# mbhall88/drprg

Measured on AMD Instinct MI355X. Metric: reads/sec (+ achieved HBM GB/s) predicting on mtb index, 1/2/4/8 GPUs, higher is better.
Workload: dtype u32

## Files before the change

drprg_amd/_lib.py:

```python
import ctypes as C
import os

_HERE = os.path.dirname(os.path.abspath(__file__))
LIB_PATH = os.environ.get("DRPRG_HIP_LIB") or os.path.join(_HERE, "lib", "libdrprg_hip.so")
PANDORA_EXE = os.path.join(_HERE, "bin", "pandora")


class MapOpts(C.Structure):
    _fields_ = [
        ("max_diff", C.c_int32),
        ("error_rate", C.c_double),
        ("min_cluster_size", C.c_uint32),
        ("illumina", C.c_int32),
        ("genome_size", C.c_uint64),
        ("genotyping_error_rate", C.c_double),
        ("kernel", C.c_int32),
        ("binomial", C.c_int32),
    ]


class AnnotateOpts(C.Structure):
    _fields_ = [
        ("min_covg", C.c_int32), ("max_covg", C.c_int32),
        ("min_strand_bias", C.c_float), ("min_gt_conf", C.c_float), ("min_frs", C.c_float),
        ("max_indel", C.c_int32),
        ("maf", C.c_float), ("max_gaps", C.c_float), ("max_called_gaps", C.c_float), ("max_gaps_diff", C.c_float),
        ("minor_min_covg", C.c_int32), ("minor_min_strand_bias", C.c_float),
        ("ignore_synonymous", C.c_int32), ("id_seed", C.c_uint64),
    ]

    @classmethod
    def cli_defaults(cls, illumina=False):
        return cls(3, 2 ** 31 - 1, 0.01, 0.0, 0.0, -1, 0.1 if illumina else 1.0, 0.5, 0.39, 0.2, 3, 0.01, 0, 0)


SIGNATURES = {
    "drprg_hip_index": (C.c_int, [C.c_char_p, C.c_int, C.c_int, C.c_int]),
    "drprg_hip_open": (C.c_void_p, [C.c_char_p, C.c_int, C.c_int, C.c_int]),
    "drprg_hip_open_prg": (C.c_void_p, [C.c_char_p, C.c_int, C.c_int, C.c_int, C.c_int]),
    "drprg_hip_open_multi": (C.c_void_p, [C.c_char_p, C.c_int, C.c_int, C.POINTER(C.c_int), C.c_int, C.c_int]),
    "drprg_hip_reduce": (C.c_int, [C.c_void_p]),
    "drprg_hip_reduce_info": (C.c_int, [C.c_void_p, C.c_char_p, C.c_size_t]),
    "drprg_hip_comm_unique_id": (C.c_int, [C.c_void_p]),
    "drprg_hip_comm_init_rank": (C.c_int, [C.POINTER(C.c_void_p), C.c_int, C.c_void_p, C.c_int, C.c_int]),
    "drprg_hip_comm_destroy": (C.c_int, [C.c_void_p]),
    "drprg_hip_allreduce": (C.c_int, [C.c_void_p, C.c_void_p, C.c_void_p, C.c_void_p, C.c_void_p]),
    "drprg_hip_close": (None, [C.c_void_p]),
    "drprg_hip_last_error": (C.c_char_p, [C.c_void_p]),
    "drprg_hip_experimental": (C.c_int, []),
    "drprg_hip_set_opts": (C.c_int, [C.c_void_p, C.POINTER(MapOpts)]),
    "drprg_hip_set_opts_sized": (C.c_int, [C.c_void_p, C.POINTER(MapOpts), C.c_size_t]),
    "drprg_hip_map_fastx": (C.c_int, [C.c_void_p, C.c_char_p]),
    "drprg_hip_set_threads": (C.c_int, [C.c_void_p, C.c_int]),
    "drprg_hip_parse_fastx": (C.c_int, [C.c_char_p, C.c_int, C.POINTER(C.c_uint64), C.c_char_p, C.c_size_t]),
    "drprg_hip_parse_fastx_ordered": (C.c_int, [C.c_char_p, C.c_int, C.c_uint64, C.POINTER(C.c_uint64), C.c_char_p, C.c_size_t]),
    "drprg_hip_gunzip_file": (C.c_int, [C.c_char_p, C.c_int, C.c_uint64, C.c_char_p, C.POINTER(C.c_uint64), C.c_char_p, C.c_size_t]),
    "drprg_hip_map_host": (C.c_int, [C.c_void_p, C.c_void_p, C.c_void_p, C.c_uint64]),
    "drprg_hip_map_device": (C.c_int, [C.c_void_p, C.c_void_p, C.c_void_p, C.c_uint64, C.c_uint64, C.c_void_p,
                                       C.c_void_p, C.c_void_p]),
    "drprg_hip_map_device_async": (C.c_int, [C.c_void_p, C.c_void_p, C.c_void_p, C.c_uint64, C.c_uint64, C.c_void_p,
                                             C.c_void_p, C.c_void_p]),
    "drprg_hip_sync": (C.c_int, [C.c_void_p]),
    "drprg_hip_set_input_format": (C.c_int, [C.c_void_p, C.c_int]),
    "drprg_hip_pack_reads": (C.c_int, [C.c_void_p, C.c_uint64, C.c_void_p, C.c_void_p, C.c_uint64, C.POINTER(C.c_uint64)]),
    "drprg_hip_map_host_packed": (C.c_int, [C.c_void_p, C.c_void_p, C.c_void_p, C.c_uint64, C.c_void_p, C.c_uint64]),
    "drprg_hip_map_device_packed": (C.c_int, [C.c_void_p, C.c_void_p, C.c_void_p, C.c_uint64, C.c_uint64, C.c_void_p, C.c_uint64, C.c_void_p,
                                              C.c_void_p, C.c_void_p]),
    "drprg_hip_map_device_packed_async": (C.c_int, [C.c_void_p, C.c_void_p, C.c_void_p, C.c_uint64, C.c_uint64, C.c_void_p, C.c_uint64, C.c_void_p,
                                                    C.c_void_p, C.c_void_p]),
    "drprg_hip_pack_device": (C.c_int, [C.c_void_p, C.c_void_p, C.c_uint64, C.c_void_p, C.c_void_p, C.c_uint64, C.POINTER(C.c_uint64), C.c_void_p]),
    "drprg_hip_coverage_size": (C.c_int, [C.c_void_p, C.POINTER(C.c_uint64), C.POINTER(C.c_uint64)]),
    "drprg_hip_coverage": (C.c_int, [C.c_void_p, C.c_void_p, C.c_uint64, C.c_void_p, C.c_uint64]),
    "drprg_hip_set_coverage": (C.c_int, [C.c_void_p, C.c_void_p, C.c_uint64, C.c_void_p, C.c_uint64, C.c_uint64]),
    "drprg_hip_device_coverage": (C.c_int, [C.c_void_p, C.POINTER(C.c_void_p), C.POINTER(C.c_void_p)]),
    "drprg_hip_reset": (C.c_int, [C.c_void_p]),
    "drprg_hip_set_max_covg": (C.c_int, [C.c_void_p, C.c_uint64]),
    "drprg_hip_max_covg_info": (C.c_int, [C.c_void_p, C.POINTER(C.c_uint64)]),
    "drprg_hip_keep_reads": (C.c_int, [C.c_void_p, C.c_uint64]),
    "drprg_hip_map_resident": (C.c_int, [C.c_void_p, C.c_void_p]),
    "drprg_hip_resident_info": (C.c_int, [C.c_void_p, C.POINTER(C.c_uint64)]),
    "drprg_hip_select_reads": (C.c_int, [C.c_void_p, C.c_void_p, C.c_uint64, C.c_uint32, C.c_uint64, C.c_void_p, C.c_uint64, C.c_void_p, C.c_void_p,
                                         C.c_uint64, C.POINTER(C.c_uint64)]),
    "drprg_hip_counters": (C.c_int, [C.c_void_p, C.POINTER(C.c_uint64)]),
    "drprg_hip_genotype": (C.c_int, [C.c_void_p, C.c_char_p, C.c_char_p, C.c_char_p]),
    "drprg_hip_genotype_info": (C.c_int, [C.c_void_p, C.POINTER(C.c_uint32)]),
    "drprg_hip_discover": (C.c_int, [C.c_void_p, C.c_char_p, C.c_char_p, C.c_char_p, C.POINTER(C.c_uint32)]),
    "drprg_hip_discover_reads": (C.c_int, [C.c_void_p, C.c_char_p, C.c_char_p, C.c_char_p, C.c_char_p, C.c_int, C.POINTER(C.c_uint32)]),
    "drprg_hip_update_prg": (C.c_int, [C.c_void_p, C.c_char_p, C.POINTER(C.c_uint32)]),
    "drprg_hip_update_prg_from_paths": (C.c_int, [C.c_void_p, C.c_char_p, C.c_char_p, C.POINTER(C.c_uint32)]),
    "drprg_hip_save_coverage": (C.c_int, [C.c_void_p, C.c_char_p, C.c_char_p]),
    "drprg_hip_load_coverage": (C.c_int, [C.c_void_p, C.c_char_p, C.c_char_p, C.POINTER(C.c_uint64)]),
    "drprg_hip_allele_stats": (C.c_int, [C.c_void_p, C.c_void_p, C.c_uint32, C.c_uint32, C.c_void_p, C.POINTER(C.c_double)]),
    "drprg_hip_genotype_site": (C.c_int, [C.c_void_p, C.c_void_p, C.c_void_p, C.c_uint32, C.c_double, C.c_double, C.c_void_p,
                                          C.POINTER(C.c_int32), C.POINTER(C.c_double)]),
    "drprg_hip_genotype_alleles": (C.c_int, [C.c_void_p, C.c_char_p]),
    "drprg_hip_estimate_parameters": (C.c_int, [C.c_void_p, C.c_uint64, C.c_uint64, C.c_uint64, C.c_uint32, C.c_int, C.c_double, C.c_int,
                                               C.POINTER(C.c_double)]),
    "drprg_hip_kmer_log_prob": (C.c_int, [C.c_int, C.c_double, C.c_double, C.c_double, C.c_uint32, C.c_uint32, C.c_uint32, C.POINTER(C.c_float)]),
    "drprg_hip_prob_threshold": (C.c_int, [C.c_void_p, C.c_uint64, C.POINTER(C.c_int)]),
    "drprg_hip_max_path": (C.c_int, [C.c_void_p, C.c_uint32, C.c_void_p, C.c_int, C.c_uint32, C.c_void_p, C.c_uint64, C.POINTER(C.c_uint64)]),
    "drprg_hip_path_base_coverage": (C.c_int, [C.c_void_p, C.c_uint32, C.c_void_p, C.c_uint64, C.c_void_p, C.c_void_p, C.c_uint64,
                                              C.POINTER(C.c_uint64)]),
    "drprg_hip_path_coverage_too_low": (C.c_int, [C.c_void_p, C.c_uint64, C.c_uint32]),
    "drprg_hip_coverage_model": (C.c_int, [C.c_void_p, C.POINTER(C.c_double)]),
    "drprg_hip_index_sizes": (C.c_int, [C.c_void_p, C.POINTER(C.c_uint64)]),
    "drprg_hip_filter_selfcheck": (C.c_int, [C.c_void_p, C.POINTER(C.c_uint64)]),
    "drprg_hip_device_tables": (C.c_int, [C.c_void_p, C.POINTER(C.c_uint64)]),
    "drprg_hip_index_export": (C.c_int, [C.c_void_p] + [C.c_void_p] * 7),
    "drprg_hip_prg_nodes": (C.c_int, [C.c_void_p, C.c_uint32, C.c_void_p, C.c_void_p, C.c_uint32, C.POINTER(C.c_uint32),
                                      C.POINTER(C.c_uint32)]),
    "drprg_hip_annotate": (C.c_int, [C.c_char_p, C.c_char_p, C.c_char_p, C.POINTER(AnnotateOpts), C.c_char_p, C.c_size_t]),
    "drprg_hip_vcf_to_bcf": (C.c_int, [C.c_char_p, C.c_char_p, C.c_char_p, C.c_size_t]),
    "drprg_hip_report_json": (C.c_int, [C.c_char_p, C.c_char_p, C.c_char_p, C.c_char_p, C.c_int, C.c_char_p, C.c_char_p,
                                        C.c_size_t]),
    "drprg_hip_kernel_timing": (C.c_int, [C.c_void_p, C.c_int, C.c_int, C.POINTER(C.c_double), C.POINTER(C.c_uint64)]),
    "drprg_hip_filter_schedule": (C.c_int, [C.c_void_p, C.POINTER(C.c_uint64)]),
    "drprg_hip_buffer_info": (C.c_int, [C.c_void_p, C.POINTER(C.c_uint64)]),
}


def load():
    if not os.path.exists(LIB_PATH):
        raise ImportError(
            f"{LIB_PATH} is missing: build the HIP extension first (`make` at the repo root or "
            "`python -c 'import __graft_entry__ as g; g.build()'`). There is no CPU fallback.")
    try:
        import torch
    except Exception:
        pass
    lib = C.CDLL(LIB_PATH)
    for name, (res, args) in SIGNATURES.items():
        fn = getattr(lib, name)
        fn.restype = res
        fn.argtypes = args
    return lib


lib = load()
```

drprg_amd/csrc/capi.cpp:

```cpp
#include <set>
#include <atomic>
#include <mutex>
#include <thread>
#include <fstream>
#include <cstdio>
#include "../../include/drprg_hip.h"
#include "fastx.h"
#include "genotype.h"
#include "ingest.h"
#include "pgunzip.h"
#include "denovo.h"
#include "mapper.h"
#include "rccl_dyn.h"
#include "pack.h"
#include <algorithm>
#include <cstdlib>
#include <cstring>
#include <fcntl.h>
#include <functional>
#include <sys/mman.h>
#include <sys/stat.h>
#include <unistd.h>
#include <memory>

// ... 114 lines not shown
        return DRPRG_EIO;                               \
    }                                                   \
    return DRPRG_OK;

static void apply_defaults(MapParams& p, const drprg_hip_map_opts* o)
{
    p.illumina = o && o->illumina;
    p.error_rate = (o && o->error_rate > 0) ? o->error_rate : (p.illumina ? 0.001 : 0.11);
    p.max_diff = (o && o->max_diff > 0) ? o->max_diff : (p.illumina ? 2 * p.k + 1 : 250);
    p.min_cluster_size = o ? o->min_cluster_size : 10;
    p.genome_size = (o && o->genome_size) ? o->genome_size : 5000000;
    p.genotyping_error_rate = (o && o->genotyping_error_rate > 0) ? o->genotyping_error_rate : 0.01;
    p.kernel_mode = o ? o->kernel : 0;
    p.binomial = o && o->binomial;
}

static void reduce_devices(drprg_hip_ctx* ctx)
{
    if (ctx->extra.empty() || !ctx->mapper) return;
    Mapper& m = *ctx->mapper;
    std::vector<Mapper*> all { &m };
    for (auto& e : ctx->extra) all.push_back(e.get());
    for (Mapper* x : all) x->sync();
    bool distinct = true;
    for (size_t i = 0; i < all.size(); ++i)
        for (size_t j = i + 1; j < all.size(); ++j) distinct &= all[i]->device() != all[j]->device();
    const char* no = std::getenv("DRPRG_HIP_NO_RCCL");
    std::string why;
    const Rccl* r = (distinct && !(no && *no && *no != '0')) ? Rccl::get(&why) : nullptr;
    bool done = false;
    auto chk = [&](int rc, const char* what) {
        if (rc != Rccl::Success) throw Error(DRPRG_EIO, std::string("RCCL ") + what + ": " + (r && r->GetErrorString ? r->GetErrorString(rc) : "error"));
    };
    if (r) {
        if (ctx->comms.empty()) {
            std::vector<int> devs;
            for (Mapper* x : all) devs.push_back(x->device());
            std::vector<Rccl::Comm> comms(all.size(), nullptr);
            const int rc = r->CommInitAll(comms.data(), (int)all.size(), devs.data());
            if (rc == Rccl::Success) ctx->comms = comms;
            else {
                why = std::string("ncclCommInitAll: ") + (r->GetErrorString ? r->GetErrorString(rc) : "error");
                std::fprintf(stderr, "drprg-hip: warning: %s; summing the devices' vectors by peer copies\n", why.c_str());
                r = nullptr;
            }
        }
    }
    if (r) {
        const size_t nv = 2 * (size_t)m.n_knodes() + m.n_prgs();
        chk(r->GroupStart(), "ncclGroupStart");
        int first_rc = Rccl::Success;
        const char* first_what = "";
        for (size_t d = 0; d < all.size() && first_rc == Rccl::Success; ++d) {
            if (hipSetDevice(all[d]->device()) != hipSuccess) {
                first_rc = -1;
                first_what = "hipSetDevice";
                break;
            }
            first_rc = r->Reduce(all[d]->d_covg(), all[d]->d_covg(), nv, Rccl::Uint32, Rccl::Sum, 0, ctx->comms[d], all[d]->stream());
            first_what = "ncclReduce";
        }
        const int end_rc = r->GroupEnd();
        if (first_rc != Rccl::Success || end_rc != Rccl::Success) {
            ctx->needs_reset = true;
            if (first_rc == -1) throw Error(DRPRG_EIO, "hipSetDevice failed inside the reduce (drprg_hip_reset the context)");
            chk(first_rc, first_what);
            chk(end_rc, "ncclGroupEnd");
        }
        for (Mapper* x : all) {
            if (hipSetDevice(x->device()) != hipSuccess || hipStreamSynchronize(x->stream()) != hipSuccess) throw Error(DRPRG_EIO, "stream synchronisation after ncclReduce failed");
        }
        ctx->reduce_how = "rccl: ncclReduce(sum, u32) over " + std::to_string(all.size()) + " devices";
        done = true;
    }
    if (!done) {
        for (auto& e : ctx->extra) m.add_vectors_from(*e);
        ctx->reduce_how = std::string("device add: peer copy + add kernel per device (") + (distinct ? (why.empty() ? "RCCL switched off" : why) : "a device is listed twice") + ")";
    }
    for (auto& e : ctx->extra) {
        const MapCounters k = e->counters();
        ctx->extra_counts.reads += k.reads; ctx->extra_counts.bases += k.bases; ctx->extra_counts.minimizers += k.minimizers;
        ctx->extra_counts.hits += k.hits; ctx->extra_counts.clusters_kept += k.clusters_kept;
        ctx->extra_counts.hits_kept += k.hits_kept; ctx->extra_counts.leftover_reads += k.leftover_reads;
        e->reset_coverage(false);
    }
    ctx->host_coverage_valid = false;
}

extern "C" {

int drprg_hip_index(const char* prg_file, int w, int k, int threads)
{
    if (!prg_file) return DRPRG_EINVAL;
    try {
        PrgIndex::build_and_save(prg_file, w, k, threads > 0 ? threads : 1, read_switches());
    } catch (const Error& e) {
        g_last_error = e.what();
        return e.code;
    } catch (const std::exception& e) {
        g_last_error = e.what();
        return DRPRG_EIO;
    }
    return DRPRG_OK;
}

static drprg_hip_ctx* open_impl(const char* prg_file, int w, int k, int device, bool from_files, int threads, const int* more_devices = nullptr,
    int n_more = 0)
{
    if (!prg_file) {
        g_last_error = "null PRG path";
        return nullptr;
    }
    std::unique_ptr<drprg_hip_ctx> ctx(new (std::nothrow) drprg_hip_ctx);
    if (!ctx) return nullptr;
    std::thread warm;
    if (device >= 0) warm = std::thread(Mapper::warm_device, device);
    struct Join {
        std::thread& t;
        ~Join()
        {
            if (t.joinable()) t.join();
        }
    } join_warm { warm };
    try {
        ctx->prg_file = prg_file;
        const Switches sw = read_switches();
        if (from_files) {
            try {
                ctx->index.load(prg_file, w, k, sw);
            } catch (const Error& e) {
                const char* strict = std::getenv("DRPRG_HIP_STRICT_INDEX");
                if ((e.code != DRPRG_EFORMAT && e.code != DRPRG_ENOENT) || (strict && *strict && *strict != '0')) throw;
                std::fprintf(stderr, "drprg-hip: warning: %s; rebuilding the k-mer graphs from %s\n", e.what(), prg_file);
                ctx->index = PrgIndex();
                ctx->index.build(prg_file, w, k, threads > 0 ? threads : 1, sw);
            }
        } else ctx->index.build(prg_file, w, k, threads > 0 ? threads : 1, sw);
        ctx->params.w = w;
        ctx->params.k = k;
        apply_defaults(ctx->params, nullptr);
        if (warm.joinable()) warm.join();
        if (device >= 0) ctx->mapper.reset(new Mapper(ctx->index.flat, ctx->params, device));
        for (int i = 0; i < n_more; ++i) ctx->extra.emplace_back(new Mapper(ctx->index.flat, ctx->params, more_devices[i]));
    } catch (const std::exception& e) {
        g_last_error = e.what();
        return nullptr;
    }
    return ctx.release();
}

drprg_hip_ctx* drprg_hip_open(const char* prg_file, int w, int k, int device)
{
    return open_impl(prg_file, w, k, device, true, 1);
}

drprg_hip_ctx* drprg_hip_open_prg(const char* prg_file, int w, int k, int device, int threads)
{
    return open_impl(prg_file, w, k, device, false, threads);
}

drprg_hip_ctx* drprg_hip_open_multi(const char* prg_file, int w, int k, const int* devices, int ndev, int from_files)
{
    if (!devices || ndev < 1) {
        g_last_error = "drprg_hip_open_multi needs at least one device";
        return nullptr;
    }
// ... 491 lines not shown
    ctx->extra_counts = MapCounters();
    ctx->covg.clear();
    ctx->prg_reads.clear();
    ctx->host_coverage_valid = false;
    ctx->total_bases = 0;
    ctx->cap_reached = false;
    ctx->accepted_reads = ctx->dropped_reads = 0;
    ctx->bases_without_reads = false;
    ctx->mapped_paths.clear();
    ctx->needs_reset = false;
    API_END(ctx)
}

static std::vector<Mapper*> mappers_of(drprg_hip_ctx* ctx)
{
    std::vector<Mapper*> all;
    if (ctx->mapper) all.push_back(ctx->mapper.get());
    for (auto& e : ctx->extra) all.push_back(e.get());
    return all;
}

static bool reads_resident(drprg_hip_ctx* ctx, const char* path)
{
    const std::vector<Mapper*> all = mappers_of(ctx);
    if (all.empty()) return false;
    for (Mapper* m : all)
        if (!m->kept_complete()) return false;
    if (path && (ctx->mapped_paths.size() != 1 || ctx->mapped_paths[0] != path)) return false;
    return true;
}

int drprg_hip_keep_reads(drprg_hip_ctx* ctx, uint64_t max_bytes)
{
    API_BEGIN(ctx)
    need_mapper(ctx);
    for (Mapper* m : mappers_of(ctx)) m->keep_reads(max_bytes);
    if (ctx->total_bases != 0) ctx->mapped_paths.assign(2, std::string());
    API_END(ctx)
}

int drprg_hip_map_resident(drprg_hip_ctx* ctx, drprg_hip_ctx* from)
{
    API_BEGIN(ctx)
    if (!from || from == ctx) throw Error(DRPRG_EINVAL, "drprg_hip_map_resident needs another open context");
    need_mapper(ctx);
    const std::vector<Mapper*> dst = mappers_of(ctx), src = mappers_of(from);
    if (!reads_resident(from, nullptr)) throw Error(DRPRG_ENODATA, "the other context does not hold all of its reads in device memory");
    if (dst.size() != src.size()) throw Error(DRPRG_EINVAL, "the two contexts span different numbers of devices");
    for (size_t i = 0; i < dst.size(); ++i)
        if (dst[i]->device() != src[i]->device()) throw Error(DRPRG_EINVAL, "the two contexts list different devices");
    ctx->host_coverage_valid = false;
    for (size_t i = 0; i < dst.size(); ++i) ctx->accepted_reads += dst[i]->map_kept_from(*src[i]);
    ctx->total_bases += from->total_bases;
    ctx->mapped_paths.insert(ctx->mapped_paths.end(), from->mapped_paths.begin(), from->mapped_paths.end());
    reduce_devices(ctx);
    API_END(ctx)
}

int drprg_hip_resident_info(drprg_hip_ctx* ctx, uint64_t out[4])
{
    API_BEGIN(ctx)
    if (!out) throw Error(DRPRG_EINVAL, "null output");
    out[0] = reads_resident(ctx, nullptr) ? 1 : 0;
    out[1] = out[2] = 0;
    for (Mapper* m : mappers_of(ctx)) {
        out[1] += m->kept_bytes();
        out[2] += m->kept().size();
    }
    out[3] = ctx->last_discover_resident ? 1 : 0;
    API_END(ctx)
}

int drprg_hip_counters(drprg_hip_ctx* ctx, uint64_t out[8])
{
    API_BEGIN(ctx)
    if (!out) throw Error(DRPRG_EINVAL, "null output");
    std::memset(out, 0, 8 * sizeof(uint64_t));
    if (ctx->mapper) {
        MapCounters c = ctx->mapper->counters();
        const MapCounters& x = ctx->extra_counts;
        out[0] = c.reads + x.reads; out[1] = c.bases + x.bases; out[2] = c.minimizers + x.minimizers; out[3] = c.hits + x.hits;
        out[4] = c.clusters_kept + x.clusters_kept; out[5] = c.hits_kept + x.hits_kept; out[6] = c.kernel; out[7] = c.leftover_reads + x.leftover_reads;
    }
    API_END(ctx)
}

int drprg_hip_genotype(drprg_hip_ctx* ctx, const char* vcf_refs, const char* out_vcf, const char* sample)
{
    API_BEGIN(ctx)
    if (!out_vcf) throw Error(DRPRG_EINVAL, "null output path");
    sync_host_coverage(ctx);
    GenotypeResult r = genotype(ctx->index, ctx->covg, ctx->prg_reads, ctx->total_bases, ctx->params, vcf_refs ? vcf_refs : "");
    write_vcf(out_vcf, r, sample && *sample ? sample : "sample");
    ctx->ginfo[0] = r.exp_depth_covg;
    ctx->ginfo[1] = r.min_kmer_covg;
    ctx->ginfo[2] = (uint32_t)r.present.size();
    ctx->ginfo[3] = (uint32_t)r.records.size();
    ctx->last_model = r.model;
    ctx->last_dropped = r.dropped_low_coverage.size();
    ctx->last_records = std::move(r.records);
    API_END(ctx)
}

int drprg_hip_discover(drprg_hip_ctx* ctx, const char* vcf_refs, const char* out_dir, const char* sample, uint32_t* n_candidates)
{
    API_BEGIN(ctx)
    if (!out_dir) throw Error(DRPRG_EINVAL, "null output directory");
    sync_host_coverage(ctx);
    GenotypeResult r = genotype(ctx->index, ctx->covg, ctx->prg_reads, ctx->total_bases, ctx->params, vcf_refs ? vcf_refs : "");
    const std::string dir = out_dir, smp = sample && *sample ? sample : "sample";
    {
        std::ofstream o(dir + "/candidate_regions.tsv");
        o << "#locus\tstart\tend\tlow_start\tlow_end\tmax_covg\tconsensus\n";
        for (const CandidateRegion& c : r.candidates)
            o << c.chrom << "\t" << c.start << "\t" << c.end << "\t" << c.low_start << "\t" << c.low_end << "\t" << c.max_covg << "\t" << c.seq << "\n";
        if (!o) throw Error(DRPRG_EIO, "cannot write " + dir + "/candidate_regions.tsv");
    }
    {
        std::ofstream o(dir + "/denovo_paths.txt");
        o << "1 samples\nSample " << smp << "\n0 loci with denovo variants\n";
        if (!o) throw Error(DRPRG_EIO, "cannot write " + dir + "/denovo_paths.txt");
        std::ofstream f(dir + "/denovo_sequences.fa");
    }
    if (n_candidates) *n_candidates = (uint32_t)r.candidates.size();
    API_END(ctx)
}

int drprg_hip_discover_reads(drprg_hip_ctx* ctx, const char* reads_path, const char* vcf_refs, const char* out_dir, const char* sample,
    int list_loci, uint32_t out[3])
{
    API_BEGIN(ctx)
    if (!out_dir || !reads_path) throw Error(DRPRG_EINVAL, "null argument");
    sync_host_coverage(ctx);
    const DiscoverParams dp;
    GenotypeResult r = genotype(ctx->index, ctx->covg, ctx->prg_reads, ctx->total_bases, ctx->params, vcf_refs ? vcf_refs : "", dp);
    const std::string dir = out_dir, smp = sample && *sample ? sample : "sample";
    {
        std::ofstream o(dir + "/candidate_regions.tsv");
        o << "#locus\tstart\tend\tlow_start\tlow_end\tmax_covg\tconsensus\n";
        for (const CandidateRegion& c : r.candidates)
            o << c.chrom << "\t" << c.start << "\t" << c.end << "\t" << c.low_start << "\t" << c.low_end << "\t" << c.max_covg << "\t" << c.seq << "\n";
        if (!o) throw Error(DRPRG_EIO, "cannot write " + dir + "/candidate_regions.tsv");
    }
    DiscoverParams adp = dp;
    if (!ctx->params.illumina) {
        adp.min_support = 4;
        adp.min_fraction = 0.6;
    }
    ResidentReads resident;
    ctx->last_discover_resident = reads_resident(ctx, reads_path);
    if (ctx->last_discover_resident)
        resident = [ctx](const std::vector<uint64_t>& anchors, uint32_t A, std::vector<uint8_t>& bases, std::vector<uint64_t>& offsets) {
            for (Mapper* m : mappers_of(ctx)) m->select_reads_with_anchors(anchors, A, bases, offsets);
        };
    const uint64_t max_reads = ctx->cap_reached && !ctx->bases_without_reads ? ctx->accepted_reads : ~0ull;
    std::vector<NovelVariant> variants = assemble_candidate_regions(r, reads_path, ctx->threads, adp, ctx->params.illumina, resident, max_reads);
    write_denovo_paths(dir, smp, r, variants, list_loci != 0);
    if (out) {
        out[0] = (uint32_t)r.candidates.size();
        out[1] = (uint32_t)variants.size();
        std::set<std::string> loci;
        for (const NovelVariant& v : variants) loci.insert(v.chrom);
        out[2] = (uint32_t)loci.size();
    }
    ctx->last_discover = std::move(r);
    ctx->last_variants = std::move(variants);
// ... 523 lines not shown
```

drprg_amd/csrc/common.h:

```cpp
#pragma once
#include <cstdlib>
#include <cstdint>
#include <cstdio>
#include <stdexcept>
#include <string>
#include <vector>

namespace drprg {

struct Error : std::runtime_error {
    int code;
    Error(int c, const std::string& m) : std::runtime_error(m), code(c) {}
};

enum : int {
    DRPRG_OK = 0,
    DRPRG_EINVAL = -22,
    DRPRG_ENOENT = -2,
    DRPRG_EIO = -5,
    DRPRG_ENOMEM = -12,
    DRPRG_ENODEV = -19,
    DRPRG_EOVERFLOW = -75,
    DRPRG_EFORMAT = -84,
    DRPRG_ENODATA = -61,
    DRPRG_EAGAIN_SERIAL = -11,
};

inline uint64_t kmer_mask(int k) { return k >= 32 ? ~0ULL : ((1ULL << (2 * k)) - 1); }

inline uint64_t hash64(uint64_t key, uint64_t mask)
{
    key = (~key + (key << 21)) & mask;
    key = key ^ key >> 24;
    key = ((key + (key << 3)) + (key << 8)) & mask;
    key = key ^ key >> 14;
    key = ((key + (key << 2)) + (key << 4)) & mask;
    key = key ^ key >> 28;
    key = (key + (key << 31)) & mask;
    return key;
}

inline int nt4(unsigned char c)
{
    switch (c) {
    case 'A': case 'a': return 0;
    case 'C': case 'c': return 1;
    case 'G': case 'g': return 2;
    case 'T': case 't': return 3;
    default: return 4;
    }
}

constexpr uint32_t BLOOM_C0 = 0xC2B2AFu;
constexpr uint32_t BLOOM_C1 = 0x9E3779u;
constexpr uint32_t BLOOM_C2 = 0x85EBCA6Bu;
constexpr uint32_t BLOOM_CR = 0xC2B2AE35u;
constexpr uint32_t BLOOMR_WBITS = 14;
constexpr uint32_t MID_BITMAP_WORDS = 1u << 19;
constexpr uint32_t MID_C_MAX_WBITS = 17;
inline uint32_t rc12_code(uint32_t x)
{
    uint32_t r = 0;
    for (int i = 0; i < 12; ++i) r |= (((x >> (2 * i)) & 3u) ^ 2u) << (2 * (11 - i));
    return r;
}
inline uint32_t canon12_code(uint32_t x)
{
    x &= 0xFFFFFFu;
    const uint32_t r = rc12_code(x);
    return x < r ? x : r;
}

inline bool canonical_kmer_hash(const char* s, int k, uint64_t& h, bool& strand)
{
    const uint64_t mask = kmer_mask(k);
    uint64_t f = 0, r = 0;
    for (int i = 0; i < k; ++i) {
        int c = nt4((unsigned char)s[i]);
        if (c > 3) return false;
        f = (f << 2) | (uint64_t)c;
        r = (r >> 2) | ((uint64_t)(3 - c) << (2 * (k - 1)));
    }
    uint64_t hf = hash64(f & mask, mask), hr = hash64(r & mask, mask);
    h = hf < hr ? hf : hr;
    strand = hf <= hr;
    return true;
}

struct MapParams {
    int w = 11;
    int k = 15;
    int max_diff = 250;
    double error_rate = 0.11;
    uint32_t min_cluster_size = 10;
    bool illumina = false;
    uint64_t genome_size = 5000000;
    double genotyping_error_rate = 0.01;
    bool binomial = false;
    int kernel_mode = 0;
    double cluster_fraction() const;
};

}
```

drprg_amd/csrc/index.cpp:

```cpp
#include "index.h"
#include <algorithm>
#include <atomic>
#include <cerrno>
#include <cmath>
#include <cstdlib>
#include <fstream>
#include <sstream>
#include <sys/stat.h>
#include <thread>

namespace drprg {

static std::string dir_of(const std::string& p)
{
    size_t s = p.find_last_of('/');
    return s == std::string::npos ? std::string(".") : p.substr(0, s);
}

std::string PrgIndex::idx_path(const std::string& prg_file, int w, int k)
{
    return prg_file + ".k" + std::to_string(k) + ".w" + std::to_string(w) + ".idx";
}

std::string PrgIndex::gfa_path(const std::string& prg_file, const std::string& name, int w, int k)
// ... 43 lines not shown
    std::vector<Rec> recs;
    for (size_t p = 0; p < prgs.size(); ++p) {
        f.knode_base[p + 1] = f.knode_base[p] + (uint32_t)kgs[p].nodes.size();
        f.min_path_len[p] = kgs[p].shortest_path_length;
        const auto& nodes = kgs[p].nodes;
        for (size_t i = 1; i + 1 < nodes.size(); ++i)
            recs.push_back(Rec { nodes[i].hash, (uint32_t)p, nodes[i].id, (uint8_t)(nodes[i].strand ? 1 : 0) });
    }
    std::sort(recs.begin(), recs.end(), [](const Rec& a, const Rec& b) {
        if (a.key != b.key) return a.key < b.key;
        if (a.prg != b.prg) return a.prg < b.prg;
        return a.knode < b.knode;
    });
    for (size_t i = 0; i < recs.size(); ++i) {
        if (i == 0 || recs[i].key != recs[i - 1].key) {
            f.keys.push_back(recs[i].key);
            f.rec_off.push_back((uint32_t)i);
        }
        f.rec_prg.push_back(recs[i].prg);
        f.rec_knode_global.push_back(f.knode_base[recs[i].prg] + recs[i].knode);
        f.rec_strand.push_back(recs[i].strand);
    }
    f.rec_off.push_back((uint32_t)recs.size());
    uint32_t bits = 4;
    while ((1ULL << bits) < 2 * f.keys.size() + 1) ++bits;
    f.table_bits = bits;
    const size_t nslot = (size_t)1 << bits;
    f.slot_key.assign(nslot, 0);
    f.slot_off.assign(nslot, 0);
    f.slot_cnt.assign(nslot, 0);
    for (size_t i = 0; i < f.keys.size(); ++i) {
        uint32_t s = table_slot(f.keys[i], bits, k <= 15);
        while (f.slot_cnt[s] != 0) s = (s + 1) & (uint32_t)(nslot - 1);
        f.slot_key[s] = f.keys[i];
        f.slot_off[s] = f.rec_off[i];
        f.slot_cnt[s] = f.rec_off[i + 1] - f.rec_off[i];
    }
    constexpr uint32_t MAX_WBITS = 14;
    const size_t entries = 2 * recs.size();
    auto for_each_code = [&](auto&& fn) {
        for (size_t p = 0; p < prgs.size(); ++p) {
            const auto& nodes = kgs[p].nodes;
            for (size_t i = 1; i + 1 < nodes.size(); ++i) {
                const std::string s = kpath_sequence(prgs[p], nodes[i].path);
                uint32_t fw = 0, rc = 0;
                for (int j = 0; j < k; ++j) {
                    const uint32_t c = ((uint32_t)(unsigned char)s[(size_t)j] >> 1) & 3u;
                    fw |= c << (2 * j);
                    rc |= (c ^ 2u) << (2 * (k - 1 - j));
                }
                fn(fw);
                fn(rc);
            }
        }
    };
    constexpr uint32_t L0_WBITS = 15;
    const bool small_tier = k <= 15 && entries > 0 && entries <= 3 * (size_t(1) << MAX_WBITS);
    const bool level0 = small_tier && k == 15 && 4 * entries * 3 <= (size_t(32) << L0_WBITS) / 2;
    const bool force_mid = k == 15 && sw.force_mid_tier;
    if (small_tier && !force_mid && (level0 || k < 15)) {
        const uint32_t max_wbits = level0 ? MAX_WBITS - 1 : MAX_WBITS;
        uint32_t wbits = 8;
        while (wbits < max_wbits && (size_t(1) << wbits) * 5 < entries * 4) ++wbits;
        f.bloom_wbits = wbits;
        f.bloom.assign(size_t(1) << wbits, 0);
        const uint32_t wmask = (1u << wbits) - 1;
        const uint32_t kmask = (1u << (2 * k)) - 1;
        if (level0) {
            f.bloom0_wbits = L0_WBITS;
            f.bloom0.assign(size_t(1) << L0_WBITS, 0);
            f.bloom0f.assign(size_t(1) << L0_WBITS, 0);
            f.bloomr.assign(size_t(1) << BLOOMR_WBITS, 0);
        }
        const uint32_t wmask0 = (1u << L0_WBITS) - 1;
        for_each_code([&](uint32_t code) {
            const uint32_t x = code & kmask & 0xFFFFFFu;
            const uint32_t h = (uint32_t)((uint64_t)x * BLOOM_C1);
            f.bloom[(h >> 18) & wmask] |= (1u << (31 - (h & 31))) | (1u << (31 - ((h >> 8) & 31))) | (1u << (31 - ((x >> 16) & 31)));
            const uint32_t h2 = code * BLOOM_C2;
            f.bloom[h2 >> (32 - wbits)] |= (1u << (h2 & 31)) | (1u << ((h2 >> 5) & 31)) | (1u << ((h2 >> 10) & 31));
            if (level0) {
                const uint32_t hr = code * BLOOM_CR;
                f.bloomr[hr >> (32 - BLOOMR_WBITS)] |= (1u << (hr & 31)) | (1u << ((hr >> 5) & 31)) | (1u << ((hr >> 10) & 31)) | (1u << ((hr >> 15) & 31));
                const uint32_t hs = code * BLOOM_C2;
                f.bloom0f[hr >> (32 - L0_WBITS)] |= (1u << (hr & 31)) | (1u << ((hr >> 5) & 31)) | (1u << ((hr >> 10) & 31)) | (1u << (hs >> 27))
                    | (1u << ((hs >> 22) & 31)) | (1u << ((hs >> 17) & 31));
            }
            if (level0)
                for (int o = 0; o < 4; ++o) {
                    const uint32_t y = (code >> (2 * o)) & 0xFFFFFFu;
                    const uint32_t g = (uint32_t)((uint64_t)y * BLOOM_C0);
                    const uint32_t bits0 = (1u << (31 - (g & 31))) | (1u << (31 - ((g >> 8) & 31))) | (1u << (31 - ((y >> 16) & 31)));
                    f.bloom0[(g >> 17) & wmask0] |= bits0;
                    f.bloom0f[(g >> 17) & wmask0] |= bits0;
                }
        });
        if (level0) {
            uint32_t cw = 10;
            while (cw < MID_C_MAX_WBITS && (size_t(4) << cw) < 4 * entries) ++cw;
            f.blkc_wbits = cw;
            f.blkc.assign(size_t(4) << cw, 0);
            for_each_code([&](uint32_t code) {
                const uint32_t h = code * BLOOM_CR;
                for (int o = 0; o < 4; ++o) {
                    const uint32_t key = (code >> (2 * o)) & 0xFFFFFFu;
                    const uint32_t blk = (uint32_t)((uint64_t)key * BLOOM_C0) >> (32 - cw);
                    uint32_t* b = &f.blkc[(size_t)blk * 4];
                    b[0] |= 1u << (h >> 27);
                    b[1] |= 1u << ((h >> 22) & 31);
                    b[2] |= 1u << ((h >> 17) & 31);
                    b[3] |= 1u << ((h >> 12) & 31);
                }
            });
        }
    } else if (k == 15 && entries > 0 && recs.size() <= sw.mid_max_records) {
        f.mid_bitmap.assign(MID_BITMAP_WORDS, 0);
        for_each_code([&](uint32_t code) {
            for (int o = 0; o < 4; ++o) {
                const uint32_t key = canon12_code(code >> (2 * o));
                f.mid_bitmap[key >> 5] |= 1u << (key & 31);
            }
        });
        uint64_t distinct = 0;
        for (uint32_t wd : f.mid_bitmap) distinct += (uint64_t)__builtin_popcount(wd);
        f.mid0_bits = distinct * 5 <= (size_t(32) << L0_WBITS) * 2 ? 3 : 1;
        f.mid0.assign(size_t(1) << L0_WBITS, 0);
        const uint32_t wmask0 = (1u << L0_WBITS) - 1;
        for (uint32_t wi = 0; wi < MID_BITMAP_WORDS; ++wi)
            for (uint32_t wd = f.mid_bitmap[wi]; wd; wd &= wd - 1) {
                const uint32_t key = (wi << 5) | (uint32_t)__builtin_ctz(wd);
                const uint32_t g = (uint32_t)((uint64_t)key * BLOOM_C0);
                uint32_t bits0 = 1u << (31 - (g & 31));
                if (f.mid0_bits == 3) bits0 |= (1u << (31 - ((g >> 8) & 31))) | (1u << (31 - ((key >> 16) & 31)));
                f.mid0[(g >> 17) & wmask0] |= bits0;
            }
        uint32_t cw = 10;
        while (cw < MID_C_MAX_WBITS && (size_t(8) << cw) < 4 * entries) ++cw;
        f.midc_wbits = cw;
        f.midc.assign(size_t(4) << cw, 0);
        for_each_code([&](uint32_t code) {
            const uint32_t h = code * BLOOM_CR;
            for (int o = 0; o < 4; ++o) {
                const uint32_t key = canon12_code(code >> (2 * o));
                const uint32_t blk = (uint32_t)((uint64_t)key * BLOOM_C0) >> (32 - cw);
                uint32_t* b = &f.midc[(size_t)blk * 4];
                b[0] |= 1u << (h >> 27);
                b[1] |= 1u << ((h >> 22) & 31);
                b[2] |= 1u << ((h >> 17) & 31);
                b[3] |= 1u << ((h >> 12) & 31);
            }
        });
    }
}

void PrgIndex::filter_selfcheck(uint64_t out[8]) const
{
    for (int i = 0; i < 8; ++i) out[i] = 0;
    const FlatIndex& f = flat;
    if (f.midc_wbits) {
        const uint32_t wmask0 = (uint32_t)f.mid0.size() - 1;
        for (size_t p = 0; p < prgs.size(); ++p) {
            const auto& nodes = kgs[p].nodes;
            for (size_t i = 1; i + 1 < nodes.size(); ++i) {
                const std::string s = kpath_sequence(prgs[p], nodes[i].path);
                uint32_t both[2] = { 0, 0 };
                for (int j = 0; j < k; ++j) {
                    const uint32_t c = ((uint32_t)(unsigned char)s[(size_t)j] >> 1) & 3u;
                    both[0] |= c << (2 * j);
                    both[1] |= (c ^ 2u) << (2 * (k - 1 - j));
                }
                for (uint32_t code : both) {
                    ++out[0];
                    bool miss0 = false, missb = false;
                    for (int o = 0; o < 4; ++o) {
                        const uint32_t key = canon12_code(code >> (2 * o));
                        const uint32_t g = (uint32_t)((uint64_t)key * BLOOM_C0), word = f.mid0[(g >> 17) & wmask0];
                        uint32_t t = word << (g & 31);
                        if (f.mid0_bits == 3) t &= (word << ((g >> 8) & 31)) & (word << ((key >> 16) & 31));
                        miss0 |= !(t >> 31);
                        missb |= !((f.mid_bitmap[key >> 5] >> (key & 31)) & 1u);
                    }
                    out[1] += miss0;
                    out[2] += missb;
                    const uint32_t h = code * BLOOM_CR;
                    bool missc = false;
                    for (int o = 0; o < 4; ++o) {
                        const uint32_t key = canon12_code(code >> (2 * o));
                        const uint32_t* b = &f.midc[(size_t)((uint32_t)((uint64_t)key * BLOOM_C0) >> (32 - f.midc_wbits)) * 4];
                        missc |= !((b[0] >> (h >> 27)) & (b[1] >> ((h >> 22) & 31)) & (b[2] >> ((h >> 17) & 31)) & (b[3] >> ((h >> 12) & 31)) & 1u);
                    }
                    out[3] += missc;
                }
            }
        }
        auto fill = [](const std::vector<uint32_t>& v) -> uint64_t {
            uint64_t bits = 0;
            for (uint32_t w : v) bits += (uint64_t)__builtin_popcount(w);
            return v.empty() ? 0 : bits * 1000 / (32 * (uint64_t)v.size());
        };
        out[4] = fill(f.mid0);
        out[5] = fill(f.mid_bitmap);
        out[6] = fill(f.midc);
        return;
    }
    if (!f.bloom_wbits) return;
    const uint32_t wmask = (1u << f.bloom_wbits) - 1, kmask = (1u << (2 * k)) - 1, wmask0 = f.bloom0_wbits ? (1u << f.bloom0_wbits) - 1 : 0;
    auto three = [](uint32_t word, uint32_t h, uint32_t x) {
        return ((word << (h & 31)) & (word << ((h >> 8) & 31)) & (word << ((x >> 16) & 31))) >> 31;
    };
    auto check = [&](uint32_t code) {
        ++out[0];
        if (f.bloom0_wbits) {
            bool any_miss = false;
            for (int o = 0; o < 4; ++o) {
                const uint32_t y = (code >> (2 * o)) & 0xFFFFFFu;
                const uint32_t g = (uint32_t)((uint64_t)y * BLOOM_C0);
                any_miss |= !three(f.bloom0[(g >> 17) & wmask0], g, y);
            }
            out[1] += any_miss;
            const uint32_t hr = code * BLOOM_CR, word = f.bloomr[hr >> (32 - BLOOMR_WBITS)];
            out[3] += !((word >> (hr & 31)) & (word >> ((hr >> 5) & 31)) & (word >> ((hr >> 10) & 31)) & (word >> ((hr >> 15) & 31)) & 1u);
            bool miss_f = false;
            for (int o = 0; o < 4; ++o) {
                const uint32_t y = (code >> (2 * o)) & 0xFFFFFFu;
                const uint32_t g = (uint32_t)((uint64_t)y * BLOOM_C0);
                miss_f |= !three(f.bloom0f[(g >> 17) & wmask0], g, y);
            }
            const uint32_t wf = f.bloom0f[hr >> (32 - f.bloom0_wbits)];
            const uint32_t hs = code * BLOOM_C2;
            miss_f |= !((wf >> (hr & 31)) & (wf >> ((hr >> 5) & 31)) & (wf >> ((hr >> 10) & 31)) & (wf >> (hs >> 27)) & (wf >> ((hs >> 22) & 31))
                & (wf >> ((hs >> 17) & 31)) & 1u);
            bool miss_blk = false;
            if (f.blkc_wbits)
                for (int o = 0; o < 4; ++o) {
                    const uint32_t key = (code >> (2 * o)) & 0xFFFFFFu;
                    const uint32_t* b = &f.blkc[(size_t)((uint32_t)((uint64_t)key * BLOOM_C0) >> (32 - f.blkc_wbits)) * 4];
                    miss_blk |= !((b[0] >> (hr >> 27)) & (b[1] >> ((hr >> 22) & 31)) & (b[2] >> ((hr >> 17) & 31)) & (b[3] >> ((hr >> 12) & 31)) & 1u);
                }
            out[7] += miss_f || miss_blk;
        }
        const uint32_t x = code & kmask & 0xFFFFFFu;
        const uint32_t h = (uint32_t)((uint64_t)x * BLOOM_C1);
        const uint32_t h2 = code * BLOOM_C2, w2 = f.bloom[h2 >> (32 - f.bloom_wbits)];
        const bool l1 = three(f.bloom[(h >> 18) & wmask], h, x);
        const bool l2 = (w2 >> (h2 & 31)) & (w2 >> ((h2 >> 5) & 31)) & (w2 >> ((h2 >> 10) & 31)) & 1u;
        out[2] += !(l1 && l2);
    };
    for (size_t p = 0; p < prgs.size(); ++p) {
        const auto& nodes = kgs[p].nodes;
        for (size_t i = 1; i + 1 < nodes.size(); ++i) {
            const std::string s = kpath_sequence(prgs[p], nodes[i].path);
            uint32_t fw = 0, rc = 0;
            for (int j = 0; j < k; ++j) {
                const uint32_t c = ((uint32_t)(unsigned char)s[(size_t)j] >> 1) & 3u;
                fw |= c << (2 * j);
                rc |= (c ^ 2u) << (2 * (k - 1 - j));
            }
            check(fw);
            check(rc);
        }
    }
    auto fill = [](const std::vector<uint32_t>& v) -> uint64_t {
        uint64_t bits = 0;
        for (uint32_t w : v) bits += (uint64_t)__builtin_popcount(w);
        return v.empty() ? 0 : bits * 1000 / (32 * (uint64_t)v.size());
    };
    out[4] = fill(f.bloom0);
    out[5] = fill(f.bloom);
    out[6] = fill(f.bloomr);
}

void PrgIndex::save(const std::string& prg_file) const
{
    std::string kdir = dir_of(prg_file) + "/kmer_prgs";
    if (mkdir(kdir.c_str(), 0777) != 0 && errno != EEXIST) throw Error(DRPRG_EIO, "cannot create " + kdir);
    for (size_t p = 0; p < prgs.size(); ++p) kgs[p].save_gfa(gfa_path(prg_file, prgs[p].name, w, k), prgs[p]);
    std::ofstream out(idx_path(prg_file, w, k));
    if (!out) throw Error(DRPRG_EIO, "cannot write " + idx_path(prg_file, w, k));
    const FlatIndex& f = flat;
    auto path_string = [&](uint32_t prg, uint32_t node) {
        std::ostringstream os;
        const KPath& kp = kgs[prg].nodes[node].path;
        os << kp.size() << "{";
        for (const PathPiece& pp : kp) {
            const uint32_t base = prgs[prg].nodes[pp.node].start;
            os << "[" << base + pp.off_start << ", " << base + pp.off_end << ")";
        }
        os << "}";
        return os.str();
    };
    out << f.keys.size() << "\n";
    for (size_t i = 0; i < f.keys.size(); ++i) {
        out << f.keys[i] << "\t" << (f.rec_off[i + 1] - f.rec_off[i]);
        for (uint32_t j = f.rec_off[i]; j < f.rec_off[i + 1]; ++j) {
            const uint32_t prg = f.rec_prg[j], node = f.rec_knode_global[j] - f.knode_base[prg];
            out << "\t(" << prg << ", " << path_string(prg, node) << ", " << node << ", " << (int)f.rec_strand[j] << ")";
        }
        out << "\n";
    }
    if (!out) throw Error(DRPRG_EIO, "short write to " + idx_path(prg_file, w, k));
}

void PrgIndex::build_and_save(const std::string& prg_file, int w, int k, int threads, const Switches& sw)
{
    PrgIndex idx;
    idx.build(prg_file, w, k, threads, sw);
    idx.save(prg_file);
}

void PrgIndex::load(const std::string& prg_file, int w_, int k_, const Switches& sw)
{
    w = w_;
    k = k_;
    prgs = load_prg_file(prg_file);
    kgs.assign(prgs.size(), KmerGraph());
    for (size_t p = 0; p < prgs.size(); ++p) kgs[p].load_gfa(gfa_path(prg_file, prgs[p].name, w, k), prgs[p], w, k);
    flatten(sw);
    std::ifstream in(idx_path(prg_file, w, k));
    if (!in) throw Error(DRPRG_ENOENT, "cannot open " + idx_path(prg_file, w, k));
    size_t nkeys = 0, nrec = 0;
    in >> nkeys;
    std::string line;
    std::getline(in, line);
    if (nkeys != flat.keys.size())
        throw Error(DRPRG_EFORMAT, idx_path(prg_file, w, k) + " does not match kmer_prgs/ (key count)");
    for (size_t i = 0; i < nkeys; ++i) {
        if (!std::getline(in, line)) throw Error(DRPRG_EFORMAT, idx_path(prg_file, w, k) + " is truncated");
        std::istringstream is(line);
        uint64_t key;
        uint32_t n;
        is >> key >> n;
        if (key != flat.keys[i] || n != flat.rec_off[i + 1] - flat.rec_off[i])
            throw Error(DRPRG_EFORMAT, idx_path(prg_file, w, k) + " does not match kmer_prgs/ (key " + std::to_string(i) + ")");
        std::string field;
        std::getline(is, field, '\t');
        for (uint32_t j = flat.rec_off[i]; j < flat.rec_off[i + 1]; ++j) {
            if (!std::getline(is, field, '\t')) throw Error(DRPRG_EFORMAT, idx_path(prg_file, w, k) + ": key " + std::to_string(i) + " lists too few records");
            unsigned prg = 0, node = 0;
            int strand = 0;
            bool ok;
            const size_t brace = field.find('}');
            if (!field.empty() && field[0] == '(' && brace != std::string::npos)
                ok = std::sscanf(field.c_str(), "(%u,", &prg) == 1 && std::sscanf(field.c_str() + brace + 1, ", %u, %d)", &node, &strand) == 2;
            else
                ok = std::sscanf(field.c_str(), "%u %u %d", &prg, &node, &strand) == 3;
            if (!ok || prg != flat.rec_prg[j] || node != flat.rec_knode_global[j] - flat.knode_base[flat.rec_prg[j]] || strand != (int)flat.rec_strand[j])
                throw Error(DRPRG_EFORMAT, idx_path(prg_file, w, k) + " does not match kmer_prgs/ (record " + std::to_string(j) + ")");
        }
        nrec += n;
    }
    (void)nrec;
}
// ... 5 lines not shown
```

drprg_amd/csrc/index.h:

```cpp
#pragma once
#include "kmergraph.h"
#include "switches.h"

namespace drprg {

struct MiniRecord {
    uint32_t prg;
    uint32_t knode;
    uint8_t strand;
};

struct FlatIndex {
    std::vector<uint64_t> keys;
    std::vector<uint32_t> rec_off;
    std::vector<uint32_t> rec_prg, rec_knode_global;
    std::vector<uint8_t> rec_strand;
    std::vector<uint32_t> knode_base;
    std::vector<uint32_t> min_path_len;
    uint32_t table_bits = 0;
    std::vector<uint64_t> slot_key;
    std::vector<uint32_t> slot_off, slot_cnt;
    uint32_t bloom_wbits = 0;
    std::vector<uint32_t> bloom;
    uint32_t bloom0_wbits = 0;
    std::vector<uint32_t> bloom0;
    std::vector<uint32_t> bloom0f;
    std::vector<uint32_t> bloomr;
    uint32_t midc_wbits = 0, mid0_bits = 0;
    std::vector<uint32_t> mid0, mid_bitmap, midc;
    uint32_t blkc_wbits = 0;
    std::vector<uint32_t> blkc;
    uint32_t total_knodes() const { return knode_base.empty() ? 0 : knode_base.back(); }
};

struct PrgIndex {
    int w = 0, k = 0;
    std::vector<LocalGraph> prgs;
    std::vector<KmerGraph> kgs;
    FlatIndex flat;
    void filter_selfcheck(uint64_t out[8]) const;

    static void build_and_save(const std::string& prg_file, int w, int k, int threads, const Switches& sw);
    void build(const std::string& prg_file, int w, int k, int threads, const Switches& sw);
    void load(const std::string& prg_file, int w, int k, const Switches& sw);
    void save(const std::string& prg_file) const;

    static std::string idx_path(const std::string& prg_file, int w, int k);
    static std::string gfa_path(const std::string& prg_file, const std::string& name, int w, int k);

private:
    void flatten(const Switches& sw);
};

inline uint32_t table_slot(uint64_t key, uint32_t bits, bool narrow)
{
    if (narrow) return ((uint32_t)key * 0x9E3779B1u) >> (32 - bits);
    return (uint32_t)((key * 0x9E3779B97F4A7C15ULL) >> (64 - bits));
}

}
```

drprg_amd/csrc/kernels.h:

```cpp
#pragma once
#include <cstddef>
#include <cstdint>
#include <hip/hip_runtime_api.h>
#include "switches.h"

#if defined(__HIPCC__)
#define DRPRG_HD __host__ __device__
#else
#define DRPRG_HD
#endif

namespace drprg {
namespace dev {

constexpr int HIT_POS_BITS = 23;
constexpr int HIT_PRG_BITS = 12;
constexpr int HIT_READ_BITS = 28;
constexpr uint64_t HIT_POS_MASK = (1ull << HIT_POS_BITS) - 1;
constexpr uint32_t MAX_BATCH_READS = 1u << HIT_READ_BITS;
constexpr uint32_t MAX_PRGS = 1u << HIT_PRG_BITS;

DRPRG_HD inline uint64_t pack_hit_key(uint32_t read, uint32_t prg, uint32_t rev, uint32_t pos)
{
    return ((uint64_t)read << (HIT_PRG_BITS + 1 + HIT_POS_BITS)) | ((uint64_t)prg << (1 + HIT_POS_BITS))
// ... 91 lines not shown
    const uint32_t* bloom0;
    uint32_t bloom0_wbits;
    const uint32_t* bloomr;
    const uint32_t* bloom0f;
    const uint32_t* mid0 = nullptr;
    const uint32_t* mid_bitmap = nullptr;
    const uint32_t* midc = nullptr;
    uint32_t midc_wbits = 0, mid0_bits = 0;
    const uint32_t* blkc = nullptr;
    uint32_t blkc_wbits = 0;
};
struct FilterBuffers {
    uint64_t* raw_pos;
    uint64_t* cand_info;
    uint32_t* cand_pos1;
    uint4* cand_rec;
    uint64_t raw_capacity;
    uint32_t* small;
    unsigned long long* max_len;
    const uint32_t* wave_share = nullptr;
    unsigned long long* class_clock = nullptr;
};
constexpr int FT_MAX_ROUNDS = 8;
struct FilterSched {
    uint32_t tpw0;
    uint32_t per_wg;
    uint32_t n_tiles;
    uint32_t first_ticket[FT_MAX_ROUNDS], first_tile[FT_MAX_ROUNDS], size[FT_MAX_ROUNDS];
    uint32_t n_rounds;
    uint32_t lds_word;
};
FilterSched make_filter_sched(uint32_t n_tiles, uint32_t n_wg, const uint32_t share[4], const FilterSchedKnobs& knobs);
const uint32_t* filter_builtin_shares(bool mid, bool packed);
struct FilterWork {
    const uint32_t* bloom;
    uint32_t bloom_wbits;
    const uint32_t* bloom0;
    uint32_t bloom0_wbits;
    const uint32_t* mid_bitmap;
    const uint32_t* midc;
    uint32_t midc_wbits;
    uint32_t read_begin, read_end;
    uint32_t n_slices;
    uint32_t slice_budget, slice_cpt, slice_slack;
    uint32_t slice_extra, slice_extra_from;
    uint64_t* raw_pos;
    uint32_t* slice_count;
    uint32_t* slice_base;
    uint32_t* slice_cap;
    uint32_t* super_count;
    FilterSched sched;
    uint32_t* cand_count;
    const uint32_t* cand_total;
    uint64_t* cand_info;
    uint32_t* cand_pos1;
    uint4* cand_rec;
    uint32_t ex_grid;
    uint32_t verify_grid;
    uint32_t *wg_hits, *wg_nmin, *wg_maxlen, *wg_base;
    unsigned long long* max_len;
    unsigned long long* class_clock;
    uint32_t wave_share[4];
};
constexpr uint32_t READ_NONE = 0x7FFFFFFFu;

struct ReadClusterArgs {
    const uint32_t* prg_min_path_len;
    double fraction;
    uint32_t min_cluster_size;
    int max_diff;
    uint32_t n_prgs;
    uint32_t* covg;
    uint32_t* prg_reads;
    unsigned long long* n_clusters_kept;
    unsigned long long* n_hits_kept;
    unsigned long long* n_complex;
    uint32_t* chunk_counter;
    const uint32_t* slice_prefix;
    uint32_t n_slices, mark_epoch;
    const uint32_t* block_first;
    const uint32_t *wg_hits, *wg_nmin, *wg_maxlen;
    uint32_t n_wg;
    unsigned long long *tot_hits, *tot_minimizers, *tot_max_len;
    const uint32_t* overflow_word;
    uint32_t minpath_in_lds;
};
hipError_t launch_counters_home(unsigned long long* from, unsigned long long* to, uint32_t n, hipStream_t stream, uint32_t* zero = nullptr, uint32_t n_zero = 0);
uint32_t* filter_super_counts(uint32_t* small);
uint32_t filter_super_words();
size_t filter_small_words();
void init_candidate_work(FilterWork& fw, const FilterBuffers& b, int n_cus);
hipError_t launch_sketch_filter(const SketchArgs& a, const BloomTables& bt, int n_cus, const FilterBuffers& b, const ReadClusterArgs& rc, FilterWork& fw,
    const Switches& sw, hipStream_t stream, KernelTimer timer = {});
hipError_t launch_filter_recount(const SketchArgs& a, const FilterWork& fw, hipStream_t stream);
hipError_t launch_filter_expand(const SketchArgs& a, const FilterWork& fw, hipStream_t stream);
hipError_t launch_direct_candidates(const SketchArgs& a, bool wide_hash, bool force_lds, uint32_t* tile_prefix, void* temp, size_t temp_bytes,
    uint64_t dense_capacity, const ReadClusterArgs& rc, int n_cus, FilterWork& fw, hipStream_t stream, KernelTimer timer, uint32_t slices_mark);
hipError_t launch_tile_gather_marked(const SketchArgs& a, const FilterWork& fw, const uint32_t* tile_prefix, uint32_t n_tiles, uint64_t dense_capacity,
    uint32_t mark, hipStream_t stream);
hipError_t exclusive_scan_u32(void* temp, size_t temp_bytes, const uint32_t* in, uint32_t* out, uint32_t n, hipStream_t stream);
hipError_t launch_read_sort(uint64_t* key, uint32_t* val, uint32_t n, uint32_t* scratch, uint64_t scratch_words, unsigned long long* count,
    hipStream_t stream);
size_t sort_temp_bytes(uint32_t n);
size_t scan_temp_bytes(uint32_t n);
hipError_t sort_hits(void* temp, size_t temp_bytes, const uint64_t* key_in, uint64_t* key_out, const uint32_t* val_in,
    uint32_t* val_out, uint32_t n, hipStream_t stream);
hipError_t launch_cluster_flags(const uint64_t* key, uint32_t n, int max_diff, uint32_t* head, uint32_t* scan, void* temp,
    size_t temp_bytes, hipStream_t stream);
hipError_t launch_cluster_starts(const uint32_t* head, const uint32_t* scan, uint32_t n, uint32_t* cstart, hipStream_t stream);
hipError_t launch_cluster_pipeline(const ClusterArgs& a, uint32_t n_hits, uint32_t n_prgs, hipStream_t stream);
hipError_t launch_vector_add_u32(uint32_t* dst, const uint32_t* src, uint64_t n, hipStream_t stream);
hipError_t launch_unpack(const uint32_t* words, uint64_t n_bases, const uint64_t* npos, uint64_t n_npos, uint8_t* out, hipStream_t stream);
hipError_t launch_mark_npos(const uint64_t* npos, uint64_t n_npos, uint64_t n_bases, uint16_t* bits, hipStream_t stream);
hipError_t launch_pack(const uint8_t* bases, uint64_t n_bases, uint32_t* words, uint64_t* npos, uint64_t npos_cap, unsigned long long* n_npos,
    hipStream_t stream);

hipError_t launch_covg_cut(const uint64_t* offsets, uint64_t n_reads, uint64_t target, const uint64_t* npos, uint64_t n_npos, unsigned long long* out,
    hipStream_t stream);

struct SelectedRead {
    uint64_t offset;
    uint32_t len, read, batch, pad;
};
hipError_t launch_anchor_scan(const uint8_t* bases, const uint64_t* offsets, uint32_t n_reads, uint64_t n_bases, const uint64_t* anchors,
    uint32_t n_anchors, uint32_t A, const uint32_t* prefilter, uint32_t batch, uint32_t* flags, unsigned long long* count, SelectedRead* list,
    uint64_t list_cap, int n_cus, hipStream_t stream);
struct GatherEntry {
    const uint8_t* src;
    uint64_t dst;
    uint32_t len, pad;
};
hipError_t launch_gather_reads(const GatherEntry* table, uint32_t n, uint8_t* out, hipStream_t stream);

}
}
```

drprg_amd/csrc/mapper.cpp:

```cpp
#include "mapper.h"
#include <algorithm>
#include <cmath>
#include <atomic>
#include <cstdio>
#include <cstdlib>
#include <cstring>
#include <mutex>
#include <set>
#include <hip/hip_runtime.h>
#include <sys/mman.h>

namespace drprg {

#define HIPCHK(x)                                                                                              \
    do {                                                                                                       \
        hipError_t e_ = (x);                                                                                   \
        if (e_ != hipSuccess)                                                                                  \
            throw Error(e_ == hipErrorOutOfMemory ? DRPRG_ENOMEM : DRPRG_EIO,                                  \
                std::string("HIP error: ") + hipGetErrorString(e_) + " at " + __FILE__ + ":" + std::to_string(__LINE__)); \
    } while (0)

template <typename T> static void dmalloc(T*& p, size_t n)
{
    p = nullptr;
// ... 169 lines not shown
void Mapper::zero_now(void* p, int value, size_t bytes)
{
    (void)value;
    HIPCHK(hipMemsetAsync(p, 0, bytes, stream_));
    HIPCHK(hipStreamSynchronize(stream_));
}

static std::mutex g_pinned_mu;
static std::set<void*> g_pinned_by_runtime;

void* Mapper::pinned_alloc(size_t bytes)
{
    constexpr size_t HUGE = 2u << 20;
    const size_t n = (bytes + HUGE - 1) / HUGE * HUGE;
    void* p = std::aligned_alloc(HUGE, n);
    if (!p) return nullptr;
    (void)madvise(p, n, MADV_HUGEPAGE);
    for (size_t i = 0; i < n; i += 4096) static_cast<volatile char*>(p)[i] = 0;
    if (hipHostRegister(p, n, hipHostRegisterPortable) != hipSuccess) {
        (void)hipGetLastError();
        std::free(p);
        p = nullptr;
        if (hipHostMalloc(&p, bytes, hipHostMallocPortable) != hipSuccess) {
            (void)hipGetLastError();
            return nullptr;
        }
        std::lock_guard<std::mutex> g(g_pinned_mu);
        g_pinned_by_runtime.insert(p);
    }
    return p;
}

void Mapper::pinned_free(void* p)
{
    if (!p) return;
    {
        std::lock_guard<std::mutex> g(g_pinned_mu);
        if (g_pinned_by_runtime.erase(p)) {
            (void)hipHostFree(p);
            return;
        }
    }
    (void)hipHostUnregister(p);
    std::free(p);
}

void Mapper::warm_device(int device)
{
    if (hipSetDevice(device) == hipSuccess) (void)hipFree(nullptr);
}

void Mapper::set_params(const MapParams& p)
{
    sync();
    if (p.k < 1 || p.k > 31) throw Error(DRPRG_EINVAL, "k must be in [1,31]");
    if (p.w < 1 || p.w > 1024) throw Error(DRPRG_EINVAL, "w must be in [1,1024]");
    const bool filter_ok = (bloom_wbits_ != 0 || midc_wbits_ != 0) && p.k <= 15 && p.w <= 16;
    if (p.kernel_mode < 0 || p.kernel_mode > 3) throw Error(DRPRG_EINVAL, "kernel must be 0 (auto), 1, 2 or 3");
    if (p.kernel_mode == 2 && !filter_ok)
        throw Error(DRPRG_EINVAL, "the Bloom-prefiltered kernel needs k <= 15, w <= 16 and an index small enough for its filter tiers");
    params_ = p;
    wide_hash_ = p.k > 15;
    halo_ = std::max(16, ((p.w - 1 + 15) / 16) * 16);
    if (d_prg_thr_) {
        std::vector<uint32_t> thr(n_prgs_);
        const double fraction = params_.cluster_fraction();
        for (uint32_t i = 0; i < n_prgs_; ++i) thr[i] = (uint32_t)((double)h_min_path_len_[i] * fraction);
        HIPCHK(hipSetDevice(device_));
        HIPCHK(hipMemcpy(d_prg_thr_, thr.data(), n_prgs_ * sizeof(uint32_t), hipMemcpyHostToDevice));
        HIPCHK(hipStreamSynchronize(nullptr));
    }
    use_filter_ = p.kernel_mode == 2 || (p.kernel_mode == 0 && filter_ok);
    use_mid_ = use_filter_ && bloom_wbits_ == 0;
    use_direct_cands_ = p.kernel_mode == 3 || (p.kernel_mode == 0 && !filter_ok);
}

void Mapper::reset_coverage(bool new_sample)
{
    sync();
    HIPCHK(hipSetDevice(device_));
    HIPCHK(hipMemsetAsync(d_covg_, 0, (2 * (size_t)n_knodes_ + (size_t)n_prgs_) * sizeof(uint32_t), stream_));
    HIPCHK(hipMemsetAsync(d_counters_, 0, C_N * sizeof(unsigned long long), stream_));
    HIPCHK(hipStreamSynchronize(stream_));
    tot_reads_ = tot_bases_ = tot_hits_ = tot_leftover_ = tot_minimizers_ = 0;
    for (auto& sh : ft_share_)
        for (uint32_t& v : sh) v = 0;
    sw_ = read_switches();
    if (new_sample) drop_kept();
}

void Mapper::ensure_workspace(uint64_t cap)
{
    if (cap <= hit_capacity_) return;
    if (cap >= (1ull << 31)) throw Error(DRPRG_EOVERFLOW, "more than 2^31 minimizer hits in one batch; map smaller batches");
    dfree(d_key_a_); dfree(d_key_b_); dfree(d_val_a_); dfree(d_val_b_);
    dfree(d_head_); dfree(d_scan_); dfree(d_cstart_); dfree(d_order_); dfree(d_clusters_);
    if (d_temp_) (void)hipFree(d_temp_);
    d_temp_ = nullptr;
    hit_capacity_ = cap;
    dmalloc(d_key_a_, cap); dmalloc(d_key_b_, cap); dmalloc(d_val_a_, cap); dmalloc(d_val_b_, cap);
    dmalloc(d_head_, cap); dmalloc(d_scan_, cap); dmalloc(d_cstart_, cap + 1); dmalloc(d_order_, cap);
    dmalloc(d_clusters_, cap);
    temp_bytes_ = std::max(dev::sort_temp_bytes((uint32_t)cap), dev::scan_temp_bytes((uint32_t)cap));
    HIPCHK(hipMalloc(&d_temp_, temp_bytes_ ? temp_bytes_ : 1));
}

void Mapper::free_lane(Lane& lane)
{
    dfree(lane.raw_pos); dfree(lane.cand_info); dfree(lane.cand_pos1); dfree(lane.cand_rec); dfree(lane.small);
    dfree(lane.d_scratch);
    if (lane.h_scratch) (void)hipHostFree(lane.h_scratch);
    lane.h_scratch = nullptr;
    lane.h_scratch_dev = nullptr;
    for (hipEvent_t* e : { &lane.done, &lane.t0, &lane.t1 })
        if (*e) (void)hipEventDestroy(*e);
    lane = Lane();
}

void Mapper::grow_lane(Lane& lane, uint64_t cap)
{
    if (cap <= lane.raw_capacity) return;
    if (cap >= (1ull << 31)) throw Error(DRPRG_EOVERFLOW, "more than 2^31 candidate k-mers in one batch; map smaller batches");
    dfree(lane.raw_pos); dfree(lane.cand_info); dfree(lane.cand_pos1); dfree(lane.cand_rec);
    lane.raw_capacity = cap;
    dmalloc(lane.raw_pos, cap); dmalloc(lane.cand_info, cap); dmalloc(lane.cand_pos1, cap); dmalloc(lane.cand_rec, cap);
    zero_now(lane.cand_pos1, 0, cap * sizeof(uint32_t));
}

void Mapper::ensure_lanes()
{
    for (Lane& lane : lanes_) {
        if (lane.h_scratch_dev) continue;
        HIPCHK(hipEventCreateWithFlags(&lane.done, hipEventDisableTiming));
        HIPCHK(hipEventCreate(&lane.t0));
        HIPCHK(hipEventCreate(&lane.t1));
        dmalloc(lane.small, dev::filter_small_words());
        zero_now(lane.small, 0, dev::filter_small_words() * sizeof(uint32_t));
        dmalloc(lane.d_scratch, (size_t)L_N);
        HIPCHK(hipHostMalloc((void**)&lane.h_scratch, L_N * sizeof(unsigned long long), hipHostMallocDefault));
        zero_now(lane.d_scratch, 0, L_N * sizeof(unsigned long long));
        lane.scratch_zero = true;
        HIPCHK(hipHostGetDevicePointer((void**)&lane.h_scratch_dev, lane.h_scratch, 0));
    }
}

Mapper::Batch Mapper::make_batch(int lane, const DeviceBatch& batch, uint32_t* covg, uint32_t* prg_reads, hipStream_t stream) const
{
    Batch b;
    b.batch = batch;
    b.active = true;
    b.direct = !use_filter_;
    b.lane = lane;
    b.covg = covg;
    b.prg_reads = prg_reads;
    b.stream = stream;
    return b;
}

void Mapper::launch(const Batch& b)
{
    ensure_lanes();
    if (b.direct) direct_launch(b);
    else filter_launch(b);
    HIPCHK(hipEventRecord(lanes_[b.lane].done, b.stream));
}

void Mapper::filter_launch(const Batch& b)
{
    Lane& lane = lanes_[b.lane];
    grow_lane(lane, std::max<uint64_t>(min_capacity_, b.batch.n_bases / FILTER_BASES_PER_ENTRY));
    if (!lane.scratch_zero) HIPCHK(hipMemsetAsync(lane.d_scratch, 0, L_N * sizeof(unsigned long long), b.stream));
    lane.scratch_zero = false;
    dev::SketchArgs a = sketch_args(b.batch);
    a.n_hits = &lane.d_scratch[L_HITS];
    a.n_minimizers = &lane.d_scratch[L_MINIMIZERS];
    a.overflow = reinterpret_cast<uint32_t*>(&lane.d_scratch[L_OVERFLOW]);
    dev::FilterBuffers fb { lane.raw_pos, lane.cand_info, lane.cand_pos1, lane.cand_rec, lane.raw_capacity, lane.small, &lane.d_scratch[L_MAXLEN] };
    fb.class_clock = &lane.d_scratch[L_FT_CLOCK];
    if (ft_share_[b.batch.packed ? 1 : 0][0]) fb.wave_share = ft_share_[b.batch.packed ? 1 : 0];
    dev::BloomTables bt { d_bloom_, bloom_wbits_, d_bloom0_, bloom0_wbits_, d_bloomr_, d_bloom0f_ };
    bt.blkc = d_blkc_;
    bt.blkc_wbits = blkc_wbits_;
    if (use_mid_) {
        bt.mid0 = d_mid0_;
        bt.mid_bitmap = d_mid_bitmap_;
        bt.midc = d_midc_;
        bt.midc_wbits = midc_wbits_;
        bt.mid0_bits = mid0_bits_;
    }
    dev::ReadClusterArgs rc {};
    rc.prg_min_path_len = d_min_path_len_;
    rc.fraction = params_.cluster_fraction();
    rc.min_cluster_size = params_.min_cluster_size;
    rc.max_diff = params_.max_diff;
    rc.n_prgs = n_prgs_;
    rc.covg = b.covg;
    rc.prg_reads = b.prg_reads;
    rc.n_clusters_kept = &d_counters_[C_CLUSTERS_KEPT];
    rc.n_hits_kept = &d_counters_[C_HITS_KEPT];
    rc.n_complex = &lane.d_scratch[L_COMPLEX];
    rc.chunk_counter = reinterpret_cast<uint32_t*>(&lane.d_scratch[L_CHUNK]);
    dev::KernelTimer timer;
    if (timing_) {
        timer.begin = lane.t0;
        timer.end = lane.t1;
    }
    HIPCHK(dev::launch_sketch_filter(a, bt, n_cus_, fb, rc, lane.fw, sw_, b.stream, timer));
    HIPCHK(dev::launch_counters_home(lane.d_scratch, lane.h_scratch_dev, L_N, b.stream, dev::filter_super_counts(lane.small), dev::filter_super_words()));
    lane.scratch_zero = true;
}

static void wait_stream(hipStream_t stream, hipEvent_t event = nullptr)
{
    for (int spins = 0; spins < 2048; ++spins) {
        const hipError_t e = event ? hipEventQuery(event) : hipStreamQuery(stream);
        if (e == hipSuccess) return;
        if (e != hipErrorNotReady) HIPCHK(e);
    }
    HIPCHK(event ? hipEventSynchronize(event) : hipStreamSynchronize(stream));
}

void Mapper::cluster_hits(const uint64_t* d_offsets, uint32_t n_hits, bool ordered, unsigned long long* d_unsorted, uint32_t* covg,
    uint32_t* prg_reads, hipStream_t stream)
{
    if (n_hits == 0) return;
    const uint64_t* s_key = d_key_b_;
    const uint32_t* s_val = d_val_b_;
    if (ordered) {
        HIPCHK(dev::launch_read_sort(d_key_a_, d_val_a_, n_hits, d_order_, hit_capacity_, d_unsorted, stream));
        s_key = d_key_a_;
        s_val = d_val_a_;
    } else HIPCHK(dev::sort_hits(d_temp_, temp_bytes_, d_key_a_, d_key_b_, d_val_a_, d_val_b_, n_hits, stream));
    HIPCHK(dev::launch_cluster_flags(s_key, n_hits, params_.max_diff, d_head_, d_scan_, d_temp_, temp_bytes_, stream));
    HIPCHK(dev::launch_cluster_starts(d_head_, d_scan_, n_hits, d_cstart_, stream));
    dev::ClusterArgs c {};
    c.key = s_key;
    c.val = s_val;
    c.scan = d_scan_;
    c.cstart = d_cstart_;
    c.d_n_clusters = d_scan_ + (n_hits - 1);
    c.offsets = d_offsets;
    c.prg_min_path_len = d_min_path_len_;
    c.clusters = d_clusters_;
    c.order = d_order_;
    c.w = params_.w;
    c.fraction = params_.cluster_fraction();
    c.min_cluster_size = params_.min_cluster_size;
    c.covg = covg;
    c.prg_reads = prg_reads;
    c.n_clusters_kept = &d_counters_[C_CLUSTERS_KEPT];
    c.n_hits_kept = &d_counters_[C_HITS_KEPT];
    HIPCHK(dev::launch_cluster_pipeline(c, n_hits, n_prgs_, stream));
}

dev::SketchArgs Mapper::sketch_args(const DeviceBatch& batch) const
{
    dev::SketchArgs a {};
    a.bases = batch.d_bases;
    a.offsets = batch.d_offsets;
    a.n_bases = batch.n_bases;
    a.n_reads = (uint32_t)batch.n_reads;
    a.w = params_.w;
    a.k = params_.k;
    a.halo = halo_;
    a.slot_key = d_slot_key_;
    a.slot_rec = d_slot_rec_;
    a.slot_first = d_slot_first_;
    a.table_bits = table_bits_;
    a.rec_knode = d_rec_knode_;
    a.rec_prg = d_rec_prg_;
    a.tile_first_read = ts_->d_tile_first;
    a.pbloom = d_pbloom_;
    a.pbloom_wbits = pbloom_wbits_;
    a.hit_key = d_key_a_;
    a.hit_val = d_val_a_;
    a.hit_capacity = hit_capacity_;
    a.n_hits = &d_counters_[C_HITS];
    a.n_minimizers = &d_counters_[C_MINIMIZERS];
    a.overflow = reinterpret_cast<uint32_t*>(&d_counters_[C_OVERFLOW]);
    a.packed = batch.packed ? 1 : 0;
    a.npos = batch.d_npos;
    a.n_npos = batch.n_npos;
    return a;
}

Mapper::DeviceBatch Mapper::ascii_view(int slot, const DeviceBatch& batch, hipStream_t stream)
{
    if (!batch.packed) return batch;
    const uint64_t need = (batch.n_bases + 15) / 16 * 16 + 64;
    if (need > unpacked_cap_[slot]) {
        sync();
// ... 126 lines not shown
    a.tile_info = t.d_tile_info;
    a.tile_pos1 = t.d_tile_pos1;
    a.tile_rec = t.d_tile_rec;
    a.tile_count = t.d_tile_count;
    a.tile_hits = t.d_tile_hits;
    a.tile_nmin = t.d_tile_nmin;
    a.prg_min_path_len = d_min_path_len_;
    a.prg_thr = d_prg_thr_;
    a.fraction = params_.cluster_fraction();
    a.min_cluster_size = params_.min_cluster_size;
    dev::FilterBuffers fb { lane.raw_pos, lane.cand_info, lane.cand_pos1, lane.cand_rec, lane.raw_capacity, lane.small, &lane.d_scratch[L_MAXLEN] };
    dev::ReadClusterArgs rc {};
    rc.prg_min_path_len = d_min_path_len_;
    rc.fraction = params_.cluster_fraction();
    rc.min_cluster_size = params_.min_cluster_size;
    rc.max_diff = params_.max_diff;
    rc.n_prgs = n_prgs_;
    rc.covg = b.covg;
    rc.prg_reads = b.prg_reads;
    rc.n_clusters_kept = &d_counters_[C_CLUSTERS_KEPT];
    rc.n_hits_kept = &d_counters_[C_HITS_KEPT];
    rc.n_complex = &lane.d_scratch[L_COMPLEX];
    rc.chunk_counter = reinterpret_cast<uint32_t*>(&lane.d_scratch[L_CHUNK]);
    lane.fw = dev::FilterWork {};
    lane.fw.read_begin = 0;
    lane.fw.read_end = (uint32_t)b.batch.n_reads;
    dev::init_candidate_work(lane.fw, fb, n_cus_);
    dev::KernelTimer timer;
    if (timing_) {
        timer.begin = lane.t0;
        timer.end = lane.t1;
    }
    HIPCHK(dev::launch_direct_candidates(a, wide_hash_, sw_.direct_lds, t.d_tile_prefix, t.d_tile_temp, t.tile_temp_bytes, lane.raw_capacity, rc, n_cus_, lane.fw,
        stream, timer, mark));
    t.a_done = a;
    t.mark = mark;
    t.n_tiles = n_tiles;
    HIPCHK(hipMemcpyAsync(lane.h_scratch, lane.d_scratch, L_N * sizeof(unsigned long long), hipMemcpyDeviceToHost, stream));
    HIPCHK(hipMemsetAsync(lane.d_scratch, 0, L_N * sizeof(unsigned long long), stream));
    lane.scratch_zero = true;
}

bool Mapper::direct_finish(const Batch& b, int attempt)
{
    TileSet& t = tsets_[b.lane];
    ts_ = &t;
    Lane& lane = lanes_[b.lane];
    const uint32_t ovf = (uint32_t)lane.h_scratch[L_OVERFLOW];
    if (ovf & 2u) throw Error(DRPRG_EOVERFLOW, "a read is longer than 2^" + std::to_string(dev::HIT_POS_BITS) + " bases");
    if (ovf & 4u) {
        if (attempt > 6) throw Error(DRPRG_EOVERFLOW, "candidate buffer overflow after regrow");
        HIPCHK(hipStreamSynchronize(b.stream));
        ++reruns_direct_;
        t.slice_cap = std::min<uint32_t>(t.slice_cap * 2, 4096);
        grow_lane(lane, std::min<uint64_t>(lane.raw_capacity * 2, (1ull << 31) - 1));
        return false;
    }
    tot_minimizers_ += lane.h_scratch[L_MINIMIZERS];
    tot_hits_ += lane.h_scratch[L_HITS];
    tot_leftover_ += lane.h_scratch[L_COMPLEX];
    if (lane.h_scratch[L_COMPLEX])
        HIPCHK(dev::launch_tile_gather_marked(t.a_done, lane.fw, t.d_tile_prefix, t.n_tiles, lane.raw_capacity, t.mark, b.stream));
    leftovers(b);
    return true;
}

bool Mapper::filter_finish(const Batch& b, int attempt)
{
    Lane& lane = lanes_[b.lane];
    const uint32_t ovf = (uint32_t)lane.h_scratch[L_OVERFLOW];
    if (ovf & 8u) throw Error(DRPRG_EIO, "sketch_filter_kernel: dynamic LDS does not start at address 0");
    if (ovf & 16u) throw Error(DRPRG_EIO, "sketch_filter_kernel: a chunk of its schedule holds too few whole tiles");
    if (ovf & 32u) throw Error(DRPRG_EINVAL, "the batch's read offsets do not span its bases: offsets[0] must be 0 and offsets[n_reads] must be n_bases");
    if (ovf & 2u) throw Error(DRPRG_EOVERFLOW, "a read is longer than 2^" + std::to_string(dev::HIT_POS_BITS) + " bases");
    if (ovf & 4u) {
        if (attempt > 8) throw Error(DRPRG_EOVERFLOW, "candidate buffer overflow after regrow");
        grow_lane(lane, lane.raw_capacity * 4);
        ++reruns_filter_;
        return false;
    }
    tot_minimizers_ += lane.h_scratch[L_MINIMIZERS];
    tot_hits_ += lane.h_scratch[L_HITS];
    tot_leftover_ += lane.h_scratch[L_COMPLEX];
    tune_filter_shares(lane, b.batch.packed, b.batch.n_bases);
    leftovers(b);
    return true;
}

void Mapper::filter_schedule(uint64_t out[20])
{
    sync();
    for (int i = 0; i < 20; ++i) out[i] = ft_last_[i];
}

void Mapper::buffer_info(uint64_t out[6])
{
    sync();
    uint64_t raw = 0;
    for (const Lane& lane : lanes_) raw = std::max(raw, lane.raw_capacity);
    out[0] = reruns_filter_;
    out[1] = reruns_direct_;
    out[2] = regrows_hits_;
    out[3] = raw;
    out[4] = hit_capacity_;
    out[5] = 0;
}

void Mapper::tune_filter_shares(const Lane& lane, bool packed, uint64_t n_bases)
{
    {
        const dev::FilterSched& sc = lane.fw.sched;
        const unsigned long long* ck = &lane.h_scratch[L_FT_CLOCK];
        ft_last_[0] = sc.n_rounds;
        ft_last_[1] = lane.fw.n_slices;
        ft_last_[2] = sc.tpw0;
        for (int c = 0; c < 4; ++c) {
            ft_last_[3 + c] = lane.fw.wave_share[c];
            ft_last_[7 + c] = ck[0] && ck[1 + c] > ~ck[0] ? ck[1 + c] - ~ck[0] : 0;
        }
        ft_last_[11] = sc.per_wg;
        for (int r = 0; r < dev::FT_MAX_ROUNDS; ++r) ft_last_[12 + r] = r && r < (int)sc.n_rounds ? sc.size[r] : 0;
    }
    if (lane.fw.sched.n_rounds > 1) return;
    if (n_bases < (64ull << 20)) return;
    const unsigned long long* ck = &lane.h_scratch[L_FT_CLOCK];
    if (!ck[0] || !ck[1] || !ck[2] || !ck[3] || !ck[4]) return;
    const unsigned long long t0 = ~ck[0];
    double end[4], mean = 0;
    for (int c = 0; c < 4; ++c) {
        if (ck[1 + c] <= t0) return;
        end[c] = (double)(ck[1 + c] - t0);
        mean += end[c] / 4;
    }
    uint32_t* s = ft_share_[packed ? 1 : 0];
    if (!s[0]) {
        const uint32_t* from = dev::filter_builtin_shares(use_mid_, packed);
        for (int c = 0; c < 4; ++c) s[c] = from[c];
    }
    double v[4], sum = 0;
    for (int c = 0; c < 4; ++c) {
        v[c] = (double)s[c] * std::pow(mean / end[c], 0.6);
        v[c] = std::min(std::max(v[c], 0.35 * 256), 2.2 * 256);
        sum += v[c];
    }
    uint32_t acc = 0;
    for (int c = 0; c < 3; ++c) acc += s[c] = (uint32_t)(1024.0 * v[c] / sum + 0.5);
    s[3] = 1024u - acc;
}

void Mapper::check(const DeviceBatch& b)
{
    if (b.n_npos && !b.d_npos) throw Error(DRPRG_EINVAL, "n_npos > 0 without the positions");
    if (b.n_reads == 0) return;
    if (!b.d_bases || !b.d_offsets) throw Error(DRPRG_EINVAL, "null device pointer");
    if ((reinterpret_cast<uintptr_t>(b.d_bases) & 15u) != 0)
        throw Error(DRPRG_EINVAL, std::string(b.packed ? "d_words" : "d_bases") + " must be 16-byte aligned");
    if (b.n_reads > dev::MAX_BATCH_READS) throw Error(DRPRG_EOVERFLOW, "at most " + std::to_string(dev::MAX_BATCH_READS) + " reads per batch");
}

void Mapper::map(const DeviceBatch& batch, uint32_t* covg, uint32_t* prg_reads, hipStream_t stream, bool deferred)
{
    check(batch);
    if (batch.n_reads == 0) return;
    HIPCHK(hipSetDevice(device_));
    if (kept_cap_ && !in_keep_call_) kept_broken_ = true;
    if (!covg) covg = d_covg_;
// ... 405 lines not shown
    }
    if (!copy_stream_) HIPCHK(hipStreamCreateWithFlags(&copy_stream_, hipStreamNonBlocking));
    Stage& st = stage_[stage_next_];
    stage_next_ ^= 1;
    if (!st.copied) HIPCHK(hipEventCreateWithFlags(&st.copied, hipEventDisableTiming));
    ensure_stage(st, hb.payload_bytes(), n_reads, hb.packed ? hb.n_npos : 0);
    const DeviceBatch b = copy_in(hb, st.d_bases, st.d_offsets, st.d_npos, copy_stream_);
    HIPCHK(hipEventRecord(st.copied, copy_stream_));
    HIPCHK(hipStreamWaitEvent(stream_, st.copied, 0));
    map(b, nullptr, nullptr, stream_, true);
    HIPCHK(hipEventSynchronize(st.copied));
}

void Mapper::add_vectors_from(Mapper& other)
{
    if (other.n_knodes_ != n_knodes_ || other.n_prgs_ != n_prgs_) throw Error(DRPRG_EINVAL, "coverage size mismatch");
    other.sync();
    HIPCHK(hipSetDevice(other.device_));
    HIPCHK(hipStreamSynchronize(other.stream_));
    sync();
    HIPCHK(hipSetDevice(device_));
    const size_t nc = 2 * (size_t)n_knodes_, np = n_prgs_;
    const uint32_t* src = other.d_covg_;
    if (other.device_ != device_) {
        if (!d_peer_tmp_) dmalloc(d_peer_tmp_, nc + np);
        HIPCHK(hipMemcpyPeerAsync(d_peer_tmp_, device_, other.d_covg_, other.device_, (nc + np) * sizeof(uint32_t), stream_));
        src = d_peer_tmp_;
    }
    HIPCHK(dev::launch_vector_add_u32(d_covg_, src, nc + np, stream_));
    HIPCHK(hipStreamSynchronize(stream_));
}

void Mapper::download(std::vector<uint32_t>& covg, std::vector<uint32_t>& prg_reads)
{
    sync();
    HIPCHK(hipSetDevice(device_));
    HIPCHK(hipStreamSynchronize(stream_));
    covg.resize(2 * (size_t)n_knodes_);
    prg_reads.resize(n_prgs_);
    HIPCHK(hipMemcpy(covg.data(), d_covg_, covg.size() * sizeof(uint32_t), hipMemcpyDeviceToHost));
    HIPCHK(hipMemcpy(prg_reads.data(), d_prg_reads_, prg_reads.size() * sizeof(uint32_t), hipMemcpyDeviceToHost));
}

void Mapper::upload(const std::vector<uint32_t>& covg, const std::vector<uint32_t>& prg_reads)
{
    if (kept_cap_) kept_broken_ = true;

    if (covg.size() != 2 * (size_t)n_knodes_ || prg_reads.size() != n_prgs_) throw Error(DRPRG_EINVAL, "coverage size mismatch");
    sync();
    HIPCHK(hipSetDevice(device_));
    HIPCHK(hipMemcpy(d_covg_, covg.data(), covg.size() * sizeof(uint32_t), hipMemcpyHostToDevice));
    HIPCHK(hipMemcpy(d_prg_reads_, prg_reads.data(), prg_reads.size() * sizeof(uint32_t), hipMemcpyHostToDevice));
    HIPCHK(hipStreamSynchronize(nullptr));
}

void Mapper::device_tables(uint64_t out[6]) const
{
    out[4] = use_mid_ ? (uint64_t)MID_BITMAP_WORDS * 4 + ((uint64_t)16 << midc_wbits_) : 0;
    if (!use_mid_ && use_filter_ && d_blkc_) out[4] = (uint64_t)16 << blkc_wbits_;
    out[5] = 0;
    out[0] = d_pbloom_ ? (uint64_t)1 << pbloom_wbits_ : 0;
    out[1] = ((uint64_t)1 << table_bits_) * (wide_hash_ ? 16 : 12);
    out[2] = bloom_wbits_ ? ((uint64_t)4 << bloom_wbits_) + (bloom0_wbits_ ? ((uint64_t)4 << bloom0_wbits_) + ((uint64_t)4 << BLOOMR_WBITS) : 0) : 0;
    if (use_mid_) out[2] = (uint64_t)4 << 15;
    out[3] = use_filter_ ? 2 : (use_direct_cands_ ? 3 : 1);
}

MapCounters Mapper::counters()
{
    sync();
    HIPCHK(hipSetDevice(device_));
    HIPCHK(hipStreamSynchronize(stream_));
    unsigned long long c[C_N];
    HIPCHK(hipMemcpy(c, d_counters_, sizeof(c), hipMemcpyDeviceToHost));
    MapCounters m;
    m.reads = tot_reads_;
    m.bases = tot_bases_;
    m.minimizers = tot_minimizers_;
    m.hits = tot_hits_;
    m.clusters_kept = c[C_CLUSTERS_KEPT];
    m.hits_kept = c[C_HITS_KEPT];
    m.kernel = use_filter_ ? 2 : (use_direct_cands_ ? 3 : 1);
    m.leftover_reads = tot_leftover_;
    return m;
}

}
```

drprg_amd/csrc/mapper.h:

```cpp
#pragma once
#include "index.h"
#include "kernels.h"
#include <vector>

namespace drprg {

struct MapCounters {
    uint64_t reads = 0, bases = 0, minimizers = 0, hits = 0, clusters_kept = 0, hits_kept = 0;
    uint64_t kernel = 0;
    uint64_t leftover_reads = 0;
};

class Mapper {
public:
    Mapper(const FlatIndex& idx, const MapParams& p, int device);
    ~Mapper();
    Mapper(const Mapper&) = delete;
    Mapper& operator=(const Mapper&) = delete;

    int device() const { return device_; }
    uint32_t n_knodes() const { return n_knodes_; }
    uint32_t n_prgs() const { return n_prgs_; }
    hipStream_t stream() const { return stream_; }
    void set_params(const MapParams& p);

    struct DeviceBatch {
        const uint8_t* d_bases = nullptr;
        const uint64_t* d_offsets = nullptr;
        uint64_t n_reads = 0, n_bases = 0;
        bool packed = false;
        const uint64_t* d_npos = nullptr;
        uint64_t n_npos = 0;
    };
    void map(const DeviceBatch& b, uint32_t* d_covg, uint32_t* d_prg_reads, hipStream_t stream, bool deferred);
    void sync();
    static void check(const DeviceBatch& b);

    struct CutPoint {
        uint64_t n_reads, n_bases, n_npos;
    };
    CutPoint find_cut(const DeviceBatch& b, uint64_t target, hipStream_t stream);

    uint64_t pack_on_device(const uint8_t* d_bases, uint64_t n_bases, uint32_t* d_words, uint64_t* d_npos, uint64_t npos_cap, hipStream_t stream);
    struct HostBatch {
        const uint8_t* bases = nullptr;
        const uint64_t* offsets = nullptr;
        uint64_t n_reads = 0;
        bool packed = false;
        const uint64_t* npos = nullptr;
        uint64_t n_npos = 0;
        uint64_t n_bases() const { return offsets[n_reads]; }
        uint64_t payload_bytes() const { return packed ? ((n_bases() + 15) / 16) * 4 : n_bases(); }
    };
    void map_host(const HostBatch& b);
    void map_host_async(const HostBatch& b);
    void keep_reads(uint64_t max_bytes);
    bool kept_complete() const { return kept_cap_ > 0 && !kept_broken_; }
    const std::vector<DeviceBatch>& kept() const { return kept_; }
    uint64_t kept_bytes() const { return kept_bytes_; }
    void drop_kept();
    static constexpr uint64_t SELECT_WINDOW_BYTES = 1ull << 30;
    void select_reads_with_anchors(std::vector<uint64_t> anchors, uint32_t A, std::vector<uint8_t>& bases, std::vector<uint64_t>& offsets,
        std::vector<uint64_t>* ids = nullptr, uint64_t window_bytes = 0);
    uint64_t map_kept_from(const Mapper& other);

    void add_vectors_from(Mapper& other);

    static void* pinned_alloc(size_t bytes);
    static void pinned_free(void* p);
    static void warm_device(int device);

    void reset_coverage(bool new_sample = true);
    uint32_t* d_covg() const { return d_covg_; }
    uint32_t* d_prg_reads() const { return d_prg_reads_; }
    void download(std::vector<uint32_t>& covg, std::vector<uint32_t>& prg_reads);
    void upload(const std::vector<uint32_t>& covg, const std::vector<uint32_t>& prg_reads);
    MapCounters counters();
    void device_tables(uint64_t out[6]) const;

    bool pending_writes_to(const uint32_t* covg, const uint32_t* prg_reads) const
    {
        return pending_.active && ((covg && pending_.covg == covg) || (prg_reads && pending_.prg_reads == prg_reads));
    }
    void filter_schedule(uint64_t out[20]);
    void buffer_info(uint64_t out[6]);
    void enable_kernel_timing(bool on) { timing_ = on; }
    double sketch_ms_total() const { return sketch_ms_; }
    uint64_t sketch_launches() const { return sketch_launches_; }
    void reset_kernel_timing() { sketch_ms_ = 0; sketch_launches_ = 0; }

private:
    void zero_now(void* p, int value, size_t bytes);
    void ensure_workspace(uint64_t hit_capacity);
    struct Lane {
        hipEvent_t done = nullptr, t0 = nullptr, t1 = nullptr;
        uint64_t raw_capacity = 0;
        uint64_t *raw_pos = nullptr, *cand_info = nullptr;
        uint4* cand_rec = nullptr;
        uint32_t *cand_pos1 = nullptr, *small = nullptr;
        unsigned long long* d_scratch = nullptr;
        unsigned long long* h_scratch = nullptr;
        unsigned long long* h_scratch_dev = nullptr;
        bool scratch_zero = false;
        dev::FilterWork fw {};
    };
    enum { L_HITS = 0, L_OVERFLOW = 1, L_MAXLEN = 2, L_UNSORTED = 3, L_COMPLEX = 4, L_CHUNK = 5, L_MINIMIZERS = 6, L_FT_CLOCK = 7 , L_N = 12 };
    struct Batch {
        DeviceBatch batch;
        bool active = false;
        bool direct = false;
        int lane = 0;
        uint32_t *covg = nullptr, *prg_reads = nullptr;
        hipStream_t stream = nullptr;
    };
    Batch make_batch(int lane, const DeviceBatch& batch, uint32_t* covg, uint32_t* prg_reads, hipStream_t stream) const;
    void ensure_lanes();
    void grow_lane(Lane& lane, uint64_t raw_capacity);
    void free_lane(Lane& lane);
    void launch(const Batch& b);
    void filter_launch(const Batch& b);
    bool filter_finish(const Batch& b, int attempt);
    void direct_launch(const Batch& b);
    bool direct_finish(const Batch& b, int attempt);
    void leftovers(const Batch& b);
    void run_batch(const DeviceBatch& batch, uint32_t* d_covg, uint32_t* d_prg_reads, hipStream_t stream);
    void cluster_hits(const uint64_t* d_offsets, uint32_t n_hits, bool ordered, unsigned long long* d_unsorted, uint32_t* d_covg,
        uint32_t* d_prg_reads, hipStream_t stream);
    dev::SketchArgs sketch_args(const DeviceBatch& batch) const;
    DeviceBatch ascii_view(int slot, const DeviceBatch& batch, hipStream_t stream);
    uint8_t* d_unpacked_[3] = { nullptr, nullptr, nullptr };
    unsigned long long* d_pack_count_ = nullptr;
    unsigned long long *h_cut_ = nullptr, *h_cut_dev_ = nullptr;
    uint64_t unpacked_cap_[3] = { 0, 0, 0 };
    void read_counters(hipStream_t stream);
    void note_kernel_time(hipEvent_t t0, hipEvent_t t1);
    void complete_pending();
    void complete_batch(const Batch& b);
    Batch pending_;
    int pipe_next_ = 0;

    int device_ = 0;
    Switches sw_ = read_switches();
    MapParams params_;
    bool wide_hash_ = false;
    int halo_ = 16;
    uint32_t n_knodes_ = 0, n_prgs_ = 0, table_bits_ = 0;
    hipStream_t stream_ = nullptr;
    void* d_slot_key_ = nullptr;
    uint2* d_slot_rec_ = nullptr;
    uint4* d_slot_first_ = nullptr;
    uint32_t* d_rec_knode_ = nullptr;
    uint16_t* d_rec_prg_ = nullptr;
    uint32_t* d_min_path_len_ = nullptr;
    uint32_t* d_prg_thr_ = nullptr;
    std::vector<uint32_t> h_min_path_len_;
    uint32_t* d_bloom_ = nullptr;
    uint32_t bloom_wbits_ = 0;
    uint32_t* d_pbloom_ = nullptr;
    uint32_t pbloom_wbits_ = 0;
    uint32_t* d_bloom0_ = nullptr;
    uint32_t* d_bloom0f_ = nullptr;
    uint32_t bloom0_wbits_ = 0;
    uint32_t* d_bloomr_ = nullptr;
    uint32_t *d_mid0_ = nullptr, *d_mid_bitmap_ = nullptr, *d_midc_ = nullptr;
    uint32_t midc_wbits_ = 0, mid0_bits_ = 0;
    uint32_t* d_blkc_ = nullptr;
    uint32_t blkc_wbits_ = 0;
    bool use_mid_ = false;
    int n_cus_ = 256;
    bool use_filter_ = false;
    bool use_direct_cands_ = false;
    uint32_t* d_covg_ = nullptr;
    uint32_t* d_prg_reads_ = nullptr;
    unsigned long long* d_counters_ = nullptr;
    unsigned long long* h_counters_ = nullptr;
    uint64_t tot_reads_ = 0, tot_bases_ = 0, tot_hits_ = 0, tot_leftover_ = 0, tot_minimizers_ = 0;
    uint64_t hit_capacity_ = 0;
    uint64_t *d_key_a_ = nullptr, *d_key_b_ = nullptr;
    uint32_t *d_val_a_ = nullptr, *d_val_b_ = nullptr;
    uint32_t *d_head_ = nullptr, *d_scan_ = nullptr, *d_cstart_ = nullptr, *d_order_ = nullptr;
    dev::ClusterRec* d_clusters_ = nullptr;
    Lane lanes_[2];
    static constexpr uint64_t MIN_CAPACITY_CLAMP = 4096;
    uint64_t min_capacity_ = 1u << 20;
    uint64_t reruns_filter_ = 0, reruns_direct_ = 0, regrows_hits_ = 0;
    void* d_temp_ = nullptr;
    struct TileSet {
        uint32_t slice_cap = 256, ws_tiles = 0, ws_cap = 0, first_cap = 0;
        uint64_t* d_tile_info = nullptr;
        uint32_t *d_tile_pos1 = nullptr, *d_tile_count = nullptr, *d_tile_hits = nullptr, *d_tile_nmin = nullptr, *d_tile_prefix = nullptr;
        uint4* d_tile_rec = nullptr;
        void* d_tile_temp = nullptr;
        size_t tile_temp_bytes = 0;
        uint32_t* d_tile_first = nullptr;
        uint16_t* d_nbits = nullptr;
        uint64_t nbits_cap = 0;
        bool nbits_dirty = false;
        uint32_t mark = 0, n_tiles = 0;
        dev::SketchArgs a_done {};
    };
    TileSet tsets_[2];
    TileSet* ts_ = &tsets_[0];
    uint32_t slices_epoch_ = 0x80000000u;
    void free_tile_set(TileSet& t);
    void ensure_tile_workspace(TileSet& t, uint32_t n_tiles, uint32_t tile_cap);
    size_t temp_bytes_ = 0;
    struct Stage {
        uint8_t* d_bases = nullptr;
        uint64_t* d_offsets = nullptr;
        uint64_t* d_npos = nullptr;
        uint64_t bases_cap = 0, reads_cap = 0, npos_cap = 0;
        hipEvent_t copied = nullptr;
    };
    void ensure_stage(Stage& st, uint64_t payload_bytes, uint64_t n_reads, uint64_t n_npos);
    Stage stage_[2], stage_sync_;
    DeviceBatch copy_in(const HostBatch& hb, uint8_t* d_bases, uint64_t* d_offsets, uint64_t* d_npos, hipStream_t stream);
    int stage_next_ = 0;
    hipStream_t copy_stream_ = nullptr;
    uint32_t ft_share_[2][4] = { { 0, 0, 0, 0 }, { 0, 0, 0, 0 } };
    uint64_t ft_last_[20] = {};
    void tune_filter_shares(const Lane& lane, bool packed, uint64_t n_bases);
    std::vector<std::pair<void*, size_t>> kept_arenas_;
    uint8_t* arena_at_ = nullptr;
    size_t arena_left_ = 0;
    std::vector<DeviceBatch> kept_;
    uint64_t kept_cap_ = 0, kept_bytes_ = 0;
    bool kept_broken_ = false, in_keep_call_ = false;
    hipEvent_t kept_copied_ = nullptr;
    void* arena_take(size_t bytes);
    uint32_t* d_peer_tmp_ = nullptr;
    bool timing_ = false;
    double sketch_ms_ = 0;
    uint64_t sketch_launches_ = 0;
    hipEvent_t ev0_ = nullptr, ev1_ = nullptr;
};

}
```

drprg_amd/csrc/read_cluster.hip:

```cpp
#include "filter_common.h"
#include <algorithm>
#include <cstdint>

namespace drprg {
namespace dev {

constexpr int RC_THREADS = 1024;
constexpr int RC_WAVES = RC_THREADS / 64;
constexpr int RC_PER = 2;
constexpr int RC_WG_PER_CU = 2;
constexpr int RC_SLOTS = RC_THREADS * RC_PER;
constexpr int RC_HCAP = 3072;
constexpr int RC_POOL = 512;
constexpr uint32_t RC_IRREGULAR = 2u, RC_COMPLEX = 1u;

__device__ __forceinline__ uint32_t pack_max(uint32_t earlier, uint32_t later)
{
    const uint32_t lead = (later >> 16) > (earlier >> 16) ? (later >> 16) : (earlier >> 16);
    const uint32_t seg = (later & 0xFFFFu) > (earlier & 0xFFFFu) ? (later & 0xFFFFu) : (earlier & 0xFFFFu);
    return (lead << 16) | seg;
}
__device__ __forceinline__ void lds_barrier() { asm volatile("s_waitcnt lgkmcnt(0)\n\ts_barrier" ::: "memory"); }
__device__ __forceinline__ void lds_barrier(int& t) { asm volatile("s_waitcnt lgkmcnt(0)\n\ts_barrier" : "+v"(t) : : "memory"); }

template <bool SLICES, int AHEAD>
__global__ __launch_bounds__(RC_THREADS, 4 * RC_WG_PER_CU) void read_cluster_kernel(SketchArgs a, FilterWork fw, ReadClusterArgs rc)
{
    constexpr int RC_AHEAD = AHEAD, RC_OWN = RC_SLOTS - AHEAD;
    static_assert(RC_OWN % 64 == 0, "the slices form locates 64 entries from a multiple of 64 per wave");
    (void)RC_AHEAD;
    extern __shared__ uint32_t s_hist[];
    __shared__ uint32_t s_read[RC_SLOTS + 1], s_hstart[RC_SLOTS + 1];
    __shared__ uint16_t s_pos1[RC_SLOTS];
    __shared__ uint32_t s_gt[RC_SLOTS];
    __shared__ uint16_t s_lead[RC_SLOTS];
    __shared__ uint16_t s_seg[RC_SLOTS];
    __shared__ uint16_t s_end[RC_SLOTS];
    __shared__ uint16_t s_g0[RC_SLOTS];
    __shared__ uint8_t s_dec[RC_SLOTS];
    __shared__ uint8_t s_cplx[RC_SLOTS], s_irrf[RC_SLOTS];
    __shared__ uint16_t s_grp[RC_HCAP];
    __shared__ uint16_t s_hpos[RC_HCAP];
    __shared__ uint32_t s_cov[RC_HCAP];
    __shared__ uint32_t s_w[2][RC_WAVES];
    __shared__ uint32_t s_irr[RC_POOL];
    __shared__ uint32_t s_prev_read, s_n_irr, s_chunk;
    __shared__ unsigned long long s_tot[3];

    int tid = threadIdx.x;
#define lane (tid & 63)
#define wave (tid >> 6)
    if (rc.n_wg && blockIdx.x == 0) {
        uint32_t h = 0, nm = 0, ml = 0;
        for (uint32_t g = (uint32_t)tid; g < rc.n_wg; g += RC_THREADS) {
            h += rc.wg_hits[g];
            nm += rc.wg_nmin[g];
            const uint32_t m = rc.wg_maxlen[g];
            ml = m > ml ? m : ml;
        }
        const uint32_t wh = wave_inclusive_scan(h), wn = wave_inclusive_scan(nm), wm = wave_max(ml);
        if (lane == 63) {
            s_w[0][wave] = wh;
            s_w[1][wave] = wn;
            s_irr[wave] = wm;
        }
        __syncthreads();
        if (tid == 0) {
            unsigned long long th = 0, tn = 0;
            uint32_t tm = 0;
            for (int i = 0; i < RC_WAVES; ++i) {
                th += s_w[0][i];
                tn += s_w[1][i];
                tm = s_irr[i] > tm ? s_irr[i] : tm;
            }
            *rc.tot_hits = th;
            if (tn && !(*reinterpret_cast<volatile const uint32_t*>(rc.overflow_word) & 4u)) atomicAdd(rc.tot_minimizers, tn);
            *rc.tot_max_len = (unsigned long long)tm;
        }
        __syncthreads();
    }
    if (*reinterpret_cast<volatile uint32_t*>(a.overflow) & 4u) return;
    const uint32_t total = SLICES ? rc.slice_prefix[rc.n_slices] : *fw.cand_total;
    const uint32_t handled_mark = SLICES ? rc.mark_epoch : 0u;
    uint16_t* const s_minpath = reinterpret_cast<uint16_t*>(s_hist + rc.n_prgs);
    for (uint32_t i = tid; i < rc.n_prgs; i += RC_THREADS) {
        s_hist[i] = 0;
        if (rc.minpath_in_lds) {
            const uint32_t m = rc.prg_min_path_len[i];
            s_minpath[i] = (uint16_t)(m < 0xFFFFu ? m : 0xFFFFu);
        }
    }
    if (tid < 3) s_tot[tid] = 0;
    unsigned long long my_kept_hits = 0;
    uint32_t my_kept = 0, my_complex = 0;
    const uint32_t w1_magic = w1_reciprocal(a.w);

    struct Staged {
        uint4 rec[RC_PER];
        uint32_t info[RC_PER], pos1[RC_PER], edge_prev, edge_next;
    };
    auto request = [&](uint32_t chunk) {
        Staged st;
        const uint64_t b64 = (uint64_t)chunk * RC_OWN;
        const bool live = b64 < total;
        const uint32_t b = live ? (uint32_t)b64 : 0u;
        const uint32_t n_in = total - b < (uint32_t)RC_SLOTS ? total - b : (uint32_t)RC_SLOTS;
        if constexpr (!SLICES) {
#pragma unroll
            for (int q = 0; q < RC_PER; ++q) {
                const uint32_t i = (uint32_t)tid + (uint32_t)q * RC_THREADS;
                const uint32_t src = b + (i < n_in ? i : 0u);
                st.info[q] = live ? (uint32_t)fw.cand_info[src] : 0u;
                st.pos1[q] = live ? fw.cand_pos1[src] : 0u;
                st.rec[q] = live ? fw.cand_rec[src] : make_uint4(0, 0, 0, 0);
            }
            const bool nxt = n_in == (uint32_t)RC_SLOTS && b + n_in < total;
            st.edge_prev = live ? (uint32_t)fw.cand_info[b ? b - 1 : 0u] : 0u;
            st.edge_next = live ? (uint32_t)fw.cand_info[nxt ? b + n_in : b] : 0u;
        } else {
            const uint32_t* __restrict__ P = rc.slice_prefix;
            uint32_t* const s_mine = s_gt + (wave << 6);
            const uint32_t d_last = b + n_in - 1;
            const bool nxt = n_in == (uint32_t)RC_SLOTS && b + n_in < total;
            uint32_t d0[RC_PER + 1], s0[RC_PER + 1], pj[RC_PER + 1], p0[RC_PER + 1], sn = 0, pn0 = 0;
            bool some[RC_PER + 1];
#pragma unroll
            for (int q = 0; q <= RC_PER; ++q) {
                d0[q] = q < RC_PER ? b + ((uint32_t)(wave << 6) + (uint32_t)q * RC_THREADS) : b - 64u;
                some[q] = q < RC_PER ? live && d0[q] <= d_last : live && b && wave == 0;
                s0[q] = some[q] ? rc.block_first[__builtin_amdgcn_readfirstlane(d0[q] >> 6)] : 0u;
            }
            const bool edge_n = live && nxt && wave == 0;
            if (edge_n) sn = rc.block_first[__builtin_amdgcn_readfirstlane((b + n_in) >> 6)];
#pragma unroll
            for (int q = 0; q <= RC_PER; ++q) {
                s0[q] = __builtin_amdgcn_readfirstlane(s0[q]);
                const uint32_t j1 = s0[q] + 1u + (uint32_t)lane;
                pj[q] = some[q] ? P[j1 < rc.n_slices ? j1 : rc.n_slices] : 0u;
                p0[q] = some[q] ? P[s0[q]] : 0u;
            }
            if (edge_n) pn0 = P[sn];
            auto locate = [&](int q, uint32_t d_hi) -> size_t {
                const uint32_t x = d0[q] + (uint32_t)lane <= d_hi ? (uint32_t)lane : d_hi - d0[q];
                if (__builtin_amdgcn_readlane(pj[q], 63) > d_hi) {
                    s_mine[lane] = 0;
                    const uint32_t pn = __shfl_down(pj[q], 1);
                    const uint32_t rel = pj[q] - d0[q];
                    if ((lane == 63 || pn != pj[q]) && rel < 64u) s_mine[rel] = (uint32_t)lane + 1u;
                    __builtin_amdgcn_wave_barrier();
                    uint32_t c = s_mine[lane];
                    __builtin_amdgcn_wave_barrier();
#pragma unroll
                    for (int off = 1; off < 64; off <<= 1) {
                        const uint32_t n = __shfl_up(c, off);
                        if (lane >= off) c = n > c ? n : c;
                    }
                    c = __shfl(c, (int)x);
                    const uint32_t before = __shfl(pj[q], (int)(c ? c - 1u : 0u));
                    return (size_t)(s0[q] + c) * a.tile_cap + (d0[q] + x - (c ? before : p0[q]));
                }
                const uint32_t d = d0[q] + x;
                uint32_t lo = s0[q], hi = rc.n_slices;
                while (hi - lo > 1) {
                    const uint32_t mid = (lo + hi) >> 1;
// ... 293 lines not shown
                        cl_n = span_n;
                        cl_first = fpos;
                        cl_last = lpos;
                    }
                    nc += n_new;
                }
            }
            if (complex) {
                if (lane == 0) ++my_complex;
                continue;
            }
            const uint64_t expected = expected_minimizers(len, a.w, w1_magic);
            bool kept = false;
            if (lane < nc) {
                uint64_t m = rc.minpath_in_lds ? s_minpath[cl_g >> 1] : 0xFFFFu;
                if (m == 0xFFFFu) m = rc.prg_min_path_len[cl_g >> 1];
                if (expected < m) m = expected;
                const uint32_t length_based = (uint32_t)((double)m * rc.fraction);
                const uint32_t thr = length_based > rc.min_cluster_size ? length_based : rc.min_cluster_size;
                kept = cl_n > thr;
            }
            uint64_t alive = __ballot(kept);
            if (alive & (alive - 1)) {
                uint32_t rank = 0;
                for (uint64_t mm = alive; mm; mm &= mm - 1) {
                    const int o = __ffsll((long long)mm) - 1;
                    const uint32_t of = (uint32_t)__builtin_amdgcn_readlane((int)cl_first, o), on = (uint32_t)__builtin_amdgcn_readlane((int)cl_n, o),
                                   og = (uint32_t)__builtin_amdgcn_readlane((int)cl_g, o);
                    rank += (of < cl_first || (of == cl_first && (on > cl_n || (on == cl_n && og < cl_g)))) ? 1u : 0u;
                }
                const int nk = __popcll(alive);
                int prev = -1;
                uint32_t pg = 0, pn = 0, p_last = 0;
                for (int o = 0; o < nk; ++o) {
                    const int cur = __ffsll((long long)__ballot(kept && rank == (uint32_t)o)) - 1;
                    const uint32_t cg = (uint32_t)__builtin_amdgcn_readlane((int)cl_g, cur), cn = (uint32_t)__builtin_amdgcn_readlane((int)cl_n, cur),
                                   c_last = (uint32_t)__builtin_amdgcn_readlane((int)cl_last, cur);
                    if (prev >= 0) {
                        const bool same_prg_other_strand = (pg >> 1) == (cg >> 1) && (pg & 1u) != (cg & 1u);
                        if (same_prg_other_strand || c_last <= p_last) {
                            if (pn >= cn) {
                                alive &= ~(1ull << cur);
                                continue;
                            }
                            alive &= ~(1ull << prev);
                        }
                    }
                    prev = cur;
                    pg = cg;
                    pn = cn;
                    p_last = c_last;
                }
            }
            if ((alive >> lane) & 1ull) {
                atomicAdd(&s_hist[cl_g >> 1], 1u);
                ++my_kept;
                my_kept_hits += cl_n;
            }
            for (uint32_t b = hb; b < he; b += 64) {
                const uint32_t h = b + lane;
                const uint32_t hg = h < he ? s_grp[h] : 0xFFFFFFFFu, hp = h < he ? s_hpos[h] : 0u;
                for (uint64_t mm = alive; mm; mm &= mm - 1) {
                    const int o = __ffsll((long long)mm) - 1;
                    const uint32_t og = (uint32_t)__builtin_amdgcn_readlane((int)cl_g, o), of = (uint32_t)__builtin_amdgcn_readlane((int)cl_first, o),
                                   ol = (uint32_t)__builtin_amdgcn_readlane((int)cl_last, o);
                    if (hg == og && hp >= of && hp <= ol) atomicAdd(&rc.covg[s_cov[h]], 1u);
                }
            }
            for (uint32_t c = i + lane; c < e; c += 64)
                if (s_pos1[c]) fw.cand_pos1[base + c] = handled_mark;
        }
    }
    if (my_kept) atomicAdd(&s_tot[0], (unsigned long long)my_kept);
    if (my_kept_hits) atomicAdd(&s_tot[1], my_kept_hits);
    if (my_complex) atomicAdd(&s_tot[2], (unsigned long long)my_complex);
    __syncthreads();
    for (uint32_t i = tid; i < rc.n_prgs; i += RC_THREADS)
        if (s_hist[i]) atomicAdd(&rc.prg_reads[i], s_hist[i]);
    if (tid == 0) {
        if (s_tot[0]) atomicAdd(rc.n_clusters_kept, s_tot[0]);
        if (s_tot[1]) atomicAdd(rc.n_hits_kept, s_tot[1]);
        if (s_tot[2]) atomicAdd(rc.n_complex, s_tot[2]);
    }
}
#undef lane
#undef wave

constexpr int CH_THREADS = 256;
__global__ __launch_bounds__(CH_THREADS) void counters_home_kernel(unsigned long long* from, unsigned long long* to, uint32_t n, uint4* zero, uint32_t n_zero4)
{
    const uint32_t i = threadIdx.x;
    if (i < n) {
        to[i] = from[i];
        from[i] = 0;
    }
    for (uint32_t j = i; j < n_zero4; j += CH_THREADS) zero[j] = make_uint4(0, 0, 0, 0);
}
hipError_t launch_counters_home(unsigned long long* from, unsigned long long* to, uint32_t n, hipStream_t stream, uint32_t* zero, uint32_t n_zero)
{
    if (n > CH_THREADS || (n_zero & 3u) || (reinterpret_cast<uintptr_t>(zero) & 15u)) return hipErrorInvalidValue;
    hipLaunchKernelGGL(counters_home_kernel, dim3(1), dim3(CH_THREADS), 0, stream, from, to, n, reinterpret_cast<uint4*>(zero), zero ? n_zero / 4 : 0u);
    return hipGetLastError();
}

__global__ void flag_complex_kernel(const unsigned long long* n_hits, unsigned long long* n_complex)
{
    if (*n_hits) *n_complex = 1;
}

hipError_t launch_read_cluster(const SketchArgs& a, const FilterWork& fw, const ReadClusterArgs& rc, int n_cus, bool skip, hipStream_t stream)
{
    if (skip) {
        hipLaunchKernelGGL(flag_complex_kernel, dim3(1), dim3(1), 0, stream, a.n_hits, rc.n_complex);
        return hipGetLastError();
    }
    ReadClusterArgs rcd = rc;
    size_t dyn = (size_t)rc.n_prgs * sizeof(uint32_t);
    {
        static size_t static_lds = 0;
        if (!static_lds) {
            size_t most = 0;
            for (const void* k : { reinterpret_cast<const void*>(&read_cluster_kernel<false, 128>), reinterpret_cast<const void*>(&read_cluster_kernel<false, 256>),
                     reinterpret_cast<const void*>(&read_cluster_kernel<false, 512>), reinterpret_cast<const void*>(&read_cluster_kernel<true, 128>),
                     reinterpret_cast<const void*>(&read_cluster_kernel<true, 256>), reinterpret_cast<const void*>(&read_cluster_kernel<true, 512>) }) {
                hipFuncAttributes at {};
                HIP_TRY(hipFuncGetAttributes(&at, k));
                most = std::max<size_t>(most, at.sharedSizeBytes);
            }
            static_lds = most;
        }
        const size_t lds_cu = 160 * 1024, with = dyn + (size_t)rc.n_prgs * sizeof(uint16_t);
        const size_t fit_without = std::min<size_t>(lds_cu / (static_lds + dyn), RC_WG_PER_CU), fit_with = std::min<size_t>(lds_cu / (static_lds + with), RC_WG_PER_CU);
        rcd.minpath_in_lds = fit_with == fit_without ? 1u : 0u;
        if (rcd.minpath_in_lds) dyn = with;
    }
    const uint64_t mean_len = a.n_bases / (a.n_reads ? a.n_reads : 1u);
    const int ahead = mean_len <= 300 ? 128 : mean_len <= 600 ? 256 : 512;
    static size_t configured[6][MAX_HIP_DEVICES] = {};
    auto launch = [&](auto kernel, size_t (&conf)[MAX_HIP_DEVICES]) -> hipError_t {
        HIP_TRY(ensure_dynamic_lds(reinterpret_cast<const void*>(kernel), dyn, conf));
        hipLaunchKernelGGL(kernel, dim3((uint32_t)n_cus * RC_WG_PER_CU), dim3(RC_THREADS), dyn, stream, a, fw, rcd);
        return hipGetLastError();
    };
    if (rcd.slice_prefix) {
        if (ahead == 128) HIP_TRY(launch(&read_cluster_kernel<true, 128>, configured[0]));
        else if (ahead == 256) HIP_TRY(launch(&read_cluster_kernel<true, 256>, configured[1]));
        else HIP_TRY(launch(&read_cluster_kernel<true, 512>, configured[2]));
    } else {
        if (ahead == 128) HIP_TRY(launch(&read_cluster_kernel<false, 128>, configured[3]));
        else if (ahead == 256) HIP_TRY(launch(&read_cluster_kernel<false, 256>, configured[4]));
        else HIP_TRY(launch(&read_cluster_kernel<false, 512>, configured[5]));
    }
    return hipGetLastError();
}

}
}
```

drprg_amd/csrc/sketch_filter.hip:

```cpp
#include "filter_common.h"
#include <algorithm>
#include <cstdint>
#include <type_traits>

namespace drprg {
namespace dev {

__device__ inline uint32_t pack16le(const uint4& in)
{
    constexpr uint32_t W = 0x40100401u;
    const uint32_t p0 = __builtin_amdgcn_udot4(in.x & 0x06060606u, W, 0u, false), p1 = __builtin_amdgcn_udot4(in.y & 0x06060606u, W, 0u, false);
    const uint32_t p2 = __builtin_amdgcn_udot4(in.z & 0x06060606u, W, 0u, false), p3 = __builtin_amdgcn_udot4(in.w & 0x06060606u, W, 0u, false);
    return ((p0 | (p1 << 8) | (p2 << 16)) >> 1) | (p3 << 23);
}


typedef __attribute__((address_space(3))) const uint32_t lds_cu32;
__device__ __forceinline__ uint32_t lds_at(uint32_t byte_addr) { return *(lds_cu32*)(uintptr_t)byte_addr; }
__device__ __forceinline__ uint32_t bloom_test(uint32_t word, uint32_t h, uint32_t x)
{
    uint32_t t2;
    asm("v_lshlrev_b32_sdwa %0, %1, %2 dst_sel:DWORD dst_unused:UNUSED_PAD src0_sel:BYTE_1 src1_sel:DWORD" : "=v"(t2) : "v"(h), "v"(word));
    return (word << (h & 31)) & t2 & (word << ((x >> 16) & 0xFF));
}
// ... 124 lines not shown
    using Pair = typename std::conditional<PACKED, typename std::conditional<NW == 4, uint4, uint2>::type, PairAscii>::type;
    const uint32_t* const words = reinterpret_cast<const uint32_t*>(a.bases);
    const int64_t n_pwords = (n_bases + 15) >> 4;
    (void)words; (void)n_pwords;
    const uint32_t n_full = PACKED ? (n_pwords >= NW * 64 ? (uint32_t)((n_pwords - NW * 64) / (WPOS / 16)) + 1 : 0u)
                                   : (n_bases >= 64 * G ? (uint32_t)((n_bases - 64 * G) / WPOS) + 1 : 0u);
    uint32_t c_end = c_all < n_full ? c_all : n_full;
    auto fetch = [&](uint32_t t, Pair& p) {
        if constexpr (PACKED) {
            p = *reinterpret_cast<const Pair*>(words + (int64_t)t * (WPOS / 16) + (int64_t)lane * NW);
        } else {
            const uint8_t* g = a.bases + (int64_t)t * WPOS + (int64_t)lane * G;
            p.a = *reinterpret_cast<const uint4*>(g);
            p.b = *reinterpret_cast<const uint4*>(g + 16);
        }
    };
    uint64_t* out = fw.raw_pos + base_cur;
    uint32_t lane_keep = lane == 63 ? 0u : 0xFFFFFFFFu;
    asm volatile("" : "+v"(lane_keep));
    uint32_t wcur = 0;
    uint4* const stage = FUSED ? reinterpret_cast<uint4*>(s_dyn + STAGE_BASE_WORDS) + (tid >> 6) * STAGE_RECORDS : nullptr;
    uint32_t lcnt = 0;
    (void)stage;
    auto mb_below = [](uint64_t m) { return __builtin_amdgcn_mbcnt_hi((uint32_t)(m >> 32), __builtin_amdgcn_mbcnt_lo((uint32_t)m, 0u)); };
    (void)mb_below;
#define DRPRG_STAGE2_APPEND(r, cand2_in)                                                                                              \
    do {                                                                                                                              \
        uint32_t cand2 = (cand2_in);                                                                                                  \
                                               \
        const uint32_t c2 = (uint32_t)__popc(cand2);                                                                                  \
        const uint64_t e0 = __ballot(c2 & 1u), e1 = __ballot(c2 & 2u), e2 = __ballot(c2 & 4u);                                        \
        if (e0 | e1 | e2) {                                                                                                           \
            uint32_t at2 = wcur + mb_below(e0) + 2u * mb_below(e1) + 4u * mb_below(e2);                                               \
            const uint64_t pos2 = ((uint64_t)(r).y << 32) | (r).x;                                                                    \
            while (cand2) {                                                                                                           \
                const int q2 = __ffs(cand2) - 1;                                                                                      \
                cand2 &= cand2 - 1;                                                                                                   \
                if (at2 < cap_cur) out[at2] = pos2 + (uint64_t)q2;                                                                    \
                ++at2;                                                                                                                \
            }                                                                                                                         \
            wcur += (uint32_t)(__popcll(e0) + 2 * __popcll(e1) + 4 * __popcll(e2));                                                   \
        }                                                                                                                             \
    } while (0)
#define DRPRG_BLOCK_TEST(r, b, dst)                                                                                                   \
    do {                                                                                                                              \
        _Pragma("unroll") for (int q = 0; q < 4; ++q) {                                                                               \
            const uint32_t f = (q ? __funnelshift_r((r).z, (r).w, 2 * q) : (r).z) & kmask;                                            \
            const uint32_t h = f * BLOOM_CR;                                                                                          \
            dst |= (((b).x >> (h >> 27)) & ((b).y >> ((h >> 22) & 31)) & ((b).z >> ((h >> 17) & 31)) & ((b).w >> ((h >> 12) & 31)) & 1u) << q; \
        }                                                                                                                             \
    } while (0)
#define DRPRG_SECOND_STAGE()                                                                                                          \
    do {                                                                                                                              \
        if (lcnt) {                                                                                                                   \
            __builtin_amdgcn_wave_barrier();                  \
            if constexpr (MID != 0) {                                                                                                 \
                                             \
                for (uint32_t c0 = 0; c0 < lcnt; c0 += 128) {                                                                         \
                    const uint32_t ia = c0 + (uint32_t)lane, ib = ia + 64;                                                            \
                    uint4 ra = make_uint4(0, 0, 0, 0), rb = ra, ba = ra, bb = ra;                                                     \
                    if (ia < lcnt) {                                                                                                  \
                        ra = stage[ia];                                                                                               \
                        ba = reinterpret_cast<const uint4*>(fw.midc)[(uint32_t)__umul24(group_key(__funnelshift_r(ra.z, ra.w, 6)), BLOOM_C0) >> sh_c];  \
                    }                                                                                                                 \
                    if (ib < lcnt) {                                                                                                  \
                        rb = stage[ib];                                                                                               \
                        bb = reinterpret_cast<const uint4*>(fw.midc)[(uint32_t)__umul24(group_key(__funnelshift_r(rb.z, rb.w, 6)), BLOOM_C0) >> sh_c]; \
                    }                                                                                                                 \
                    uint32_t ca = 0, cb = 0;                                                                                          \
                    DRPRG_BLOCK_TEST(ra, ba, ca);                            \
                    DRPRG_STAGE2_APPEND(ra, ca);                                                                                      \
                    if (c0 + 64 < lcnt) {                                                                           \
                        DRPRG_BLOCK_TEST(rb, bb, cb);                                                                                 \
                        DRPRG_STAGE2_APPEND(rb, cb);                                                                                  \
                    }                                                                                                                 \
                }                                                                                                                     \
            } else {                                                                                                                  \
                for (uint32_t c0 = 0; c0 < lcnt; c0 += 64) {                                                                          \
                    const uint32_t ri = c0 + (uint32_t)lane;                                                                          \
                    uint32_t cs = 0;                                                                                                  \
                    uint4 r = make_uint4(0, 0, 0, 0);                                                                                 \
                    if (ri < lcnt) {                                                                                                  \
                        r = stage[ri];                                                                                                \
                                                                     \
                        uint32_t hq[4], h2q[4], wq[4];                                                                                \
                        _Pragma("unroll") for (int q = 0; q < 4; ++q) {                                                               \
                            const uint32_t f = (q ? __funnelshift_r(r.z, r.w, 2 * q) : r.z) & kmask;                                  \
                            hq[q] = f * BLOOM_CR;                                                                                     \
                            h2q[q] = f * BLOOM_C2;                                                                                    \
                            wq[q] = lds_at((hq[q] >> 17) << 2);                                                                       \
                        }                                                                                                             \
                        __builtin_amdgcn_sched_barrier(0);      \
                        _Pragma("unroll") for (int q = 0; q < 4; ++q)                                                                 \
                            cs |= ((wq[q] >> (hq[q] & 31)) & (wq[q] >> ((hq[q] >> 5) & 31)) & (wq[q] >> ((hq[q] >> 10) & 31)) & (wq[q] >> (h2q[q] >> 27)) \
                                      & (wq[q] >> ((h2q[q] >> 22) & 31)) & (wq[q] >> ((h2q[q] >> 17) & 31)) & 1u) << q;               \
                    }                                                                                                                 \
                    DRPRG_STAGE2_APPEND(r, cs);                                                                                       \
                }                                                                                                                     \
            }                                                                                                                         \
            __builtin_amdgcn_wave_barrier();                                                                                          \
            lcnt = 0;                                                                                                                 \
        }                                                                                                                             \
    } while (0)
    auto close_slice = [&]() {
        if constexpr (FUSED) DRPRG_SECOND_STAGE();
        if (lane == 0) {
            const uint32_t kept = wcur < cap_cur ? wcur : cap_cur;
            fw.slice_count[slice] = kept;
            fw.slice_base[slice] = base_cur;
            fw.slice_cap[slice] = cap_cur;
            if (wcur > cap_cur) atomicOr(a.overflow, 4u);
            if (kept) atomicAdd(&fw.super_count[slice / FT_SUPER], kept);
        }
    };

    auto process = [&](uint32_t t, const Pair& p) {
        uint32_t wv[NW + 1];
        if constexpr (PACKED) {
            wv[0] = p.x;
            wv[1] = p.y;
            if constexpr (NW == 4) {
                wv[2] = p.z;
                wv[3] = p.w;
            }
        } else {
            wv[0] = pack16le(p.a);
            wv[1] = pack16le(p.b);
        }
        wv[NW] = __builtin_amdgcn_update_dpp(0u, wv[0], 0x130 , 0xF, 0xF, true);
        const uint32_t wa = wv[0], wb = wv[1], wc = wv[2];
        (void)wa; (void)wb; (void)wc;
        if constexpr (LEVEL0) {
            uint32_t grp = 0, xs[NG], hs[NG], ws[NG];
#pragma unroll
            for (int g = 0; g < NG; ++g) {
                const int j = 4 * g + 3;
                const uint32_t lo = wv[j >> 4], hi = wv[(j >> 4) + 1];
                xs[g] = __builtin_amdgcn_alignbit(hi, lo, 2 * (j & 15));
                if constexpr (CANON) xs[g] = canon12_dev(xs[g]);
                hs[g] = __umul24(xs[g], BLOOM_C0);
                ws[g] = lds_at((hs[g] >> 15) & amask0);
            }
#pragma unroll
            for (int g = NG - 1; g >= 0; --g)
                grp = __builtin_amdgcn_alignbit(grp, MID == 1 ? ws[g] << (hs[g] & 31) : bloom_test(ws[g], hs[g], xs[g]), 31);
            grp &= lane_keep;
            if constexpr (CANON) {
                uint32_t bw[NG];
#pragma unroll
                for (int g = 0; g < NG; ++g) {
                    bw[g] = 0;
                    if (grp & (1u << g)) bw[g] = fw.mid_bitmap[xs[g] >> 5];
                }
                uint32_t keep = 0;
#pragma unroll
                for (int g = 0; g < NG; ++g) keep |= ((bw[g] >> (xs[g] & 31)) & 1u) << g;
                grp &= keep;
            }
            const uint32_t cnt = (uint32_t)__popc(grp);
            const uint64_t b0 = __ballot(cnt & 1u), b1 = __ballot(cnt & 2u), b2 = __ballot(cnt & 4u), b3 = __ballot(cnt & 8u);
            const uint64_t b4 = NG > 8 ? __ballot(cnt & 16u) : 0ull;
            if (b0 | b1 | b2 | b3 | b4) {
                auto below = [&](uint64_t m) { return __builtin_amdgcn_mbcnt_hi((uint32_t)(m >> 32), __builtin_amdgcn_mbcnt_lo((uint32_t)m, 0u)); };
                auto lanes_below = [&]() { return below(b0) + 2u * below(b1) + 4u * below(b2) + 8u * below(b3) + (NG > 8 ? 16u * below(b4) : 0u); };
                const uint32_t total = (uint32_t)(__popcll(b0) + 2 * __popcll(b1) + 4 * __popcll(b2) + 8 * __popcll(b3) + (NG > 8 ? 16 * __popcll(b4) : 0));
                const uint64_t base = (uint64_t)t * WPOS + (uint64_t)lane * G;
                auto record = [&](int g) {
                    const int q = g >> 2;
                    uint32_t lo = wv[0], hi = wv[1];
#pragma unroll
                    for (int u = 1; u < NW; ++u) {
                        lo = q == u ? wv[u] : lo;
                        hi = q == u ? wv[u + 1] : hi;
                    }
                    const uint32_t sh = (8u * (uint32_t)g) & 31u;
                    const uint64_t pos = base + 4u * (uint32_t)g;
                    return make_uint4((uint32_t)pos, (uint32_t)(pos >> 32), __funnelshift_r(lo, hi, sh), hi >> sh);
                };
// ... 155 lines not shown

uint32_t filter_n_tiles(uint64_t n_bases, int positions_per_lane)
{
    const uint64_t wpos = 63ull * (uint64_t)positions_per_lane;
    return (uint32_t)((n_bases + wpos - 1) / wpos);
}

uint32_t filter_grid(bool level0, int n_cus, uint32_t n_tiles, uint32_t cap)
{
    uint32_t grid = (uint32_t)n_cus * (level0 ? 1 : 2);
    const uint32_t need = (n_tiles + FT_WAVES - 1) / FT_WAVES;
    if (grid > need) grid = need;
    if (grid > (uint32_t)(MAX_SLICES / FT_WAVES)) grid = MAX_SLICES / FT_WAVES;
    if (cap && grid > cap) grid = cap;
    return grid ? grid : 1;
}

constexpr size_t FT_SMALL_HEAD = (size_t)MAX_CHUNKS * 3 + MAX_SLICES;
size_t filter_small_words() { return FT_SMALL_HEAD + 4 + 4 * (size_t)MAX_EX_WG; }
uint32_t* filter_super_counts(uint32_t* small) { return small + MAX_CHUNKS; }
uint32_t filter_super_words() { return (uint32_t)MAX_SLICES; }

FilterSched make_filter_sched(uint32_t n_tiles, uint32_t n_wg, const uint32_t share[4], const FilterSchedKnobs& knobs)
{
    FilterSched s {};
    for (int r = 0; r < FT_MAX_ROUNDS; ++r) s.first_ticket[r] = 0xFFFFFFFFu;
    s.n_rounds = 1;
    s.per_wg = FT_WAVES;
    s.n_tiles = n_tiles;
    s.tpw0 = (n_tiles + n_wg * FT_WAVES - 1) / (n_wg * FT_WAVES);
    uint32_t min_share = share[0];
    for (int c = 1; c < 4; ++c) min_share = std::min(min_share, share[c]);
    const uint64_t wg_tiles = n_tiles / n_wg, avg = wg_tiles / FT_WAVES;
    const uint32_t tpw0 = (uint32_t)(avg * knobs.f / 256);
    if (knobs.is_static || avg < knobs.min_avg || (uint64_t)tpw0 * min_share / 256 < FT_DEPTH + 2) return s;
    const uint32_t max_per_wg = (uint32_t)MAX_CHUNKS / n_wg;
    uint64_t done = (uint64_t)FT_WAVES * tpw0, rest = wg_tiles - done;
    if (rest < FT_DEPTH + 2) return s;
    uint32_t tk = FT_WAVES;
    int r = 1;
    for (; r < FT_MAX_ROUNDS - 1 && tk + 2 * FT_WAVES <= max_per_wg; ++r) {
        const uint32_t sz = (uint32_t)(rest * 16 / ((uint64_t)FT_WAVES * knobs.d));
        if (sz < 2 * knobs.m) break;
        s.first_ticket[r] = tk;
        s.first_tile[r] = (uint32_t)done;
        s.size[r] = sz;
        done += (uint64_t)FT_WAVES * sz;
        rest -= (uint64_t)FT_WAVES * sz;
        tk += FT_WAVES;
    }
    const uint32_t left = max_per_wg - tk;
    const uint32_t sz = (uint32_t)std::max<uint64_t>(knobs.m, (rest + left - 1) / left);
    const uint32_t cnt = (uint32_t)std::max<uint64_t>(1, (rest - (FT_DEPTH - 2)) / sz);
    s.first_ticket[r] = tk;
    s.first_tile[r] = (uint32_t)done;
    s.size[r] = sz;
    s.n_rounds = (uint32_t)r + 1;
    s.per_wg = tk + cnt;
    s.tpw0 = tpw0;
    return s;
}

void init_candidate_work(FilterWork& fw, const FilterBuffers& b, int n_cus)
{
    fw.cand_info = b.cand_info;
    fw.cand_pos1 = b.cand_pos1;
    fw.cand_rec = b.cand_rec;
    fw.wg_hits = b.small + FT_SMALL_HEAD + 4;
    fw.wg_nmin = fw.wg_hits + MAX_EX_WG;
    fw.wg_maxlen = fw.wg_nmin + MAX_EX_WG;
    fw.wg_base = fw.wg_maxlen + MAX_EX_WG;
    fw.ex_grid = std::min<uint32_t>((uint32_t)n_cus * 8, MAX_EX_WG);
    fw.verify_grid = fw.ex_grid;
    fw.max_len = b.max_len;
}

const uint32_t* filter_builtin_shares(bool mid, bool packed)
{
    static const uint32_t ascii_l0[4] = { 397, 294, 200, 133 }, packed_l0[4] = { 422, 292, 184, 126 }, mid_l0[4] = { 356, 292, 220, 156 };
    return mid ? mid_l0 : packed ? packed_l0 : ascii_l0;
}

hipError_t launch_sketch_filter(const SketchArgs& a, const BloomTables& bt, int n_cus, const FilterBuffers& b, const ReadClusterArgs& rc, FilterWork& fw,
    const Switches& sw, hipStream_t stream, KernelTimer timer)
{
    fw = FilterWork {};
    fw.read_begin = 0;
    fw.read_end = a.n_reads;
    if (a.n_bases == 0) return hipSuccess;
    const bool mid = bt.mid_bitmap != nullptr;
    if (mid && (a.k != 15 || !bt.mid0 || !bt.midc || bt.midc_wbits < 1 || bt.midc_wbits > MID_C_MAX_WBITS || (bt.mid0_bits != 1 && bt.mid0_bits != 3)))
        return hipErrorInvalidValue;
    if (!mid && (1u << bt.bloom_wbits) > (uint32_t)FT_BLOOM_WORDS) return hipErrorInvalidValue;
    if (!mid && bt.bloom0 && (1u << bt.bloom0_wbits) != (uint32_t)FT_L0_WORDS) return hipErrorInvalidValue;
    if (!mid && bt.bloom0 && (!bt.bloomr || !bt.bloom0f)) return hipErrorInvalidValue;
    const bool level0 = mid || (bt.bloom0 != nullptr && a.k == 15 && ((size_t)4 << bt.bloom_wbits) + (size_t)FT_L0_WORDS * 4 <= 160 * 1024);
    const bool want_l2 = sw.stage2 == Stage2::by_format ? a.packed != 0 : sw.stage2 == Stage2::l2;
    const bool blk = !mid && level0 && want_l2 && bt.blkc != nullptr && bt.blkc_wbits >= 1 && bt.blkc_wbits <= MID_C_MAX_WBITS;
    fw.bloom = bt.bloom;
    fw.bloom_wbits = bt.bloom_wbits;
    fw.bloom0 = mid ? bt.mid0 : (level0 ? (blk ? bt.bloom0 : bt.bloom0f) : nullptr);
    fw.bloom0_wbits = mid ? 15 : (level0 ? bt.bloom0_wbits : 0);
    fw.mid_bitmap = bt.mid_bitmap;
    fw.midc = blk ? bt.blkc : bt.midc;
    fw.midc_wbits = blk ? bt.blkc_wbits : bt.midc_wbits;
    const uint32_t grid = filter_grid(level0, n_cus, filter_n_tiles(a.n_bases, filter_positions_per_lane(level0, a.packed != 0)), sw.ft_grid);
    {
        static const uint32_t even[4] = { 256, 256, 256, 256 };
        const uint32_t* share = sw.ft_share_pinned ? sw.ft_share : !level0 ? even : b.wave_share ? b.wave_share : filter_builtin_shares(mid, a.packed != 0);
        fw.class_clock = level0 && !sw.ft_share_pinned ? b.class_clock : nullptr;
        for (int c = 0; c < 4; ++c) fw.wave_share[c] = share[c];
    }
    fw.sched = make_filter_sched(filter_n_tiles(a.n_bases, filter_positions_per_lane(level0, a.packed != 0)), grid, fw.wave_share, sw.ft_sched);
    fw.n_slices = grid * fw.sched.per_wg;
    {
        const uint32_t n_tiles = filter_n_tiles(a.n_bases, filter_positions_per_lane(level0, a.packed != 0));
        const uint64_t budget = std::min<uint64_t>(b.raw_capacity, 0x7FFFFFFFull) / grid;
        const uint64_t wg_tiles = fw.sched.per_wg > (uint32_t)FT_WAVES ? (n_tiles + grid - 1) / grid : (uint64_t)FT_WAVES * ((n_tiles + grid * FT_WAVES - 1) / (grid * FT_WAVES));
        fw.slice_budget = (uint32_t)budget;
        fw.slice_extra = 0;
        fw.slice_extra_from = 0xFFFFFFFFu;
        const bool last_round = fw.sched.n_rounds > 1;
        const uint64_t reserve = last_round ? budget / 4 : 0, main = budget - reserve;
        fw.slice_slack = (uint32_t)std::min<uint64_t>(256, main / (4ull * fw.sched.per_wg));
        const uint64_t tiles = std::max<uint64_t>(wg_tiles, 1);
        fw.slice_cpt = (uint32_t)((main - (uint64_t)fw.slice_slack * fw.sched.per_wg) / tiles);
        if (last_round) {
            const uint32_t last = fw.sched.n_rounds - 1, from = fw.sched.first_ticket[last], n_last = fw.sched.per_wg - from;
            const uint64_t tile_pos = 63ull * (uint64_t)filter_positions_per_lane(level0, a.packed != 0);
            const uint64_t sz = fw.sched.size[last], want = sz * tile_pos * 2 / (uint64_t)(a.w + 1);
            const uint64_t have = sz * fw.slice_cpt + fw.slice_slack;
            if (n_last && want > have) {
                fw.slice_extra = (uint32_t)std::min<uint64_t>(want - have, reserve / n_last);
                fw.slice_extra_from = from;
            }
        }
    }
    fw.raw_pos = b.raw_pos;
    fw.cand_info = b.cand_info;
    fw.cand_pos1 = b.cand_pos1;
    fw.cand_rec = b.cand_rec;
    init_candidate_work(fw, b, n_cus);
    fw.slice_count = b.small;
    fw.super_count = filter_super_counts(b.small);
    fw.slice_base = b.small + MAX_CHUNKS + MAX_SLICES;
    fw.slice_cap = fw.slice_base + MAX_CHUNKS;
    fw.cand_count = b.small + FT_SMALL_HEAD;
    fw.cand_total = fw.cand_count;
    {
        using Kernel = void (*)(SketchArgs, FilterWork);
        const int which = mid ? (bt.mid0_bits == 3 ? 3 : 4) : blk ? 5 : level0 ? 2 : (a.k < 12 ? 1 : 0);
        const Kernel ascii = which == 5 ? &sketch_filter_kernel<false, true, true, 2>
            : which == 4                ? &sketch_filter_kernel<false, true, true, 1>
            : which == 3                ? &sketch_filter_kernel<false, true, true, 3>
            : which == 2                ? &sketch_filter_kernel<false, true, true>
            : which == 1                ? &sketch_filter_kernel<true, false>
                                        : &sketch_filter_kernel<false, false>;
        const Kernel packed = which == 5 ? &sketch_filter_kernel<false, true, true, 2, true>
            : which == 4                 ? &sketch_filter_kernel<false, true, true, 1, true>
            : which == 3                 ? &sketch_filter_kernel<false, true, true, 3, true>
            : which == 2                 ? &sketch_filter_kernel<false, true, true, 0, true>
            : which == 1                 ? &sketch_filter_kernel<true, false, false, 0, true>
                                         : &sketch_filter_kernel<false, false, false, 0, true>;
        const Kernel kernel = a.packed ? packed : ascii;
        const size_t dyn = level0 ? (size_t)FT_L0_WORDS * 4 + (size_t)FT_WAVES * 2048 : ((size_t)4 << bt.bloom_wbits) + 16;
        fw.sched.lds_word = (uint32_t)(dyn / 4 - 4);
        static size_t configured[12][MAX_HIP_DEVICES] = {};
        HIP_TRY(ensure_dynamic_lds(reinterpret_cast<const void*>(kernel), dyn, configured[which + (a.packed ? 6 : 0)]));
        launch_timed(timer, kernel, dim3(grid), dim3(FT_THREADS), dyn, stream, a, fw);
    }
    HIP_TRY(hipGetLastError());
    const bool skip_rc = sw.skip_read_cluster;
    HIP_TRY(launch_candidate_stage(a, fw, rc, n_cus, stream, skip_rc));
    ReadClusterArgs rct = rc;
    if (!skip_rc) {
        rct.wg_hits = fw.wg_hits;
        rct.wg_nmin = fw.wg_nmin;
        rct.wg_maxlen = fw.wg_maxlen;
        rct.n_wg = fw.verify_grid;
        rct.tot_hits = a.n_hits;
        rct.tot_minimizers = a.n_minimizers;
        rct.tot_max_len = fw.max_len;
        rct.overflow_word = a.overflow;
    }
    return launch_read_cluster(a, fw, rct, n_cus, skip_rc, stream);
}

}
}
```

drprg_amd/pandora.py:

```python
import ctypes as C
import os
import re

import numpy as np

from ._lib import MapOpts, lib

MTB_GENOME_SIZE = 4411532


class DependencyError(RuntimeError):

    def __init__(self, kind, message, code=0):
        super().__init__(f"{kind}: {message}")
        self.kind = kind
        self.code = code


def _check(rc, ctx=None):
    if rc != 0:
        msg = lib.drprg_hip_last_error(ctx)
        raise DependencyError("ProcessError", (msg or b"").decode() or f"error {rc}", code=-rc)


# ... 59 lines not shown
        _check(lib.drprg_hip_map_host_packed(self._h, _ptr(words), _ptr(offsets), len(offsets) - 1, _ptr(npos) if npos.size else None, npos.size), self._h)

    def map_device_packed(self, d_words, d_offsets, n_reads, n_bases, d_npos=None, n_npos=0, d_covg=None, d_prg_reads=None, stream=None, deferred=False):
        fn = lib.drprg_hip_map_device_packed_async if deferred else lib.drprg_hip_map_device_packed
        _check(fn(self._h, d_words, d_offsets, n_reads, n_bases, d_npos, n_npos, d_covg, d_prg_reads, stream), self._h)

    def pack_device(self, d_bases, n_bases, d_words, d_npos=None, npos_cap=0, stream=None):
        n = C.c_uint64()
        _check(lib.drprg_hip_pack_device(self._h, d_bases, n_bases, d_words, d_npos, npos_cap, C.byref(n), stream), self._h)
        return int(n.value)

    def map_device(self, d_bases, d_offsets, n_reads, n_bases, d_covg=None, d_prg_reads=None, stream=None):
        _check(lib.drprg_hip_map_device(self._h, d_bases, d_offsets, n_reads, n_bases, d_covg, d_prg_reads, stream), self._h)

    def map_device_async(self, d_bases, d_offsets, n_reads, n_bases, d_covg=None, d_prg_reads=None, stream=None):
        _check(lib.drprg_hip_map_device_async(self._h, d_bases, d_offsets, n_reads, n_bases, d_covg, d_prg_reads, stream), self._h)

    def sync(self):
        _check(lib.drprg_hip_sync(self._h), self._h)

    def reduce(self):
        _check(lib.drprg_hip_reduce(self._h), self._h)
        buf = C.create_string_buffer(256)
        lib.drprg_hip_reduce_info(self._h, buf, len(buf))
        return buf.value.decode()

    def coverage(self):
        covg = np.zeros(2 * self.n_knodes, dtype=np.uint32)
        prg_reads = np.zeros(self.n_prgs, dtype=np.uint32)
        _check(lib.drprg_hip_coverage(self._h, _ptr(covg), covg.size, _ptr(prg_reads), prg_reads.size), self._h)
        return covg, prg_reads

    def set_coverage(self, covg, prg_reads, total_bases):
        covg = np.ascontiguousarray(covg, dtype=np.uint32)
        prg_reads = np.ascontiguousarray(prg_reads, dtype=np.uint32)
        _check(lib.drprg_hip_set_coverage(self._h, _ptr(covg), covg.size, _ptr(prg_reads), prg_reads.size, total_bases), self._h)

    def device_coverage(self):
        a, b = C.c_void_p(), C.c_void_p()
        _check(lib.drprg_hip_device_coverage(self._h, C.byref(a), C.byref(b)), self._h)
        return a.value, b.value

    def reset(self):
        _check(lib.drprg_hip_reset(self._h), self._h)

    def set_max_covg(self, max_covg):
        _check(lib.drprg_hip_set_max_covg(self._h, 2 ** 64 - 1 if max_covg is None else int(max_covg)), self._h)

    def max_covg_info(self):
        out = (C.c_uint64 * 4)()
        _check(lib.drprg_hip_max_covg_info(self._h, out), self._h)
        return dict(reached=bool(out[0]), reads=int(out[1]), bases=int(out[2]), dropped=int(out[3]))

    def keep_reads(self, max_bytes):
        _check(lib.drprg_hip_keep_reads(self._h, int(max_bytes)), self._h)

    def map_resident(self, other):
        _check(lib.drprg_hip_map_resident(self._h, other._h), self._h)

    def resident_info(self):
        out = (C.c_uint64 * 4)()
        _check(lib.drprg_hip_resident_info(self._h, out), self._h)
        return dict(complete=bool(out[0]), bytes=int(out[1]), blocks=int(out[2]), last_discover_from_hbm=bool(out[3]))

    def select_reads(self, anchors, A, window_bytes=0):
        anchors = np.ascontiguousarray(anchors, dtype=np.uint64)
        out = (C.c_uint64 * 2)()
        offsets = np.zeros(1, np.uint64)
        rc = lib.drprg_hip_select_reads(self._h, _ptr(anchors), anchors.size, int(A), int(window_bytes), None, 0, _ptr(offsets), None, 0, out)
        if rc == 0:
            return np.zeros(0, np.uint8), offsets, np.zeros(0, np.uint64)
        if rc != -75:
            _check(rc, self._h)
        n_reads, n_bases = int(out[0]), int(out[1])
        bases, offsets, ids = np.zeros(n_bases, np.uint8), np.zeros(n_reads + 1, np.uint64), np.zeros(n_reads, np.uint64)
        _check(lib.drprg_hip_select_reads(self._h, _ptr(anchors), anchors.size, int(A), int(window_bytes), _ptr(bases), n_bases, _ptr(offsets),
                                          _ptr(ids), n_reads, out), self._h)
        return bases, offsets, ids

    def counters(self):
        out = (C.c_uint64 * 8)()
        _check(lib.drprg_hip_counters(self._h, out), self._h)
        names = ("reads", "bases", "minimizers", "hits", "clusters_kept", "hits_kept", "kernel", "leftover_reads")
        return dict(zip(names, (int(x) for x in out)))

    def genotype(self, vcf_refs, out_vcf, sample="sample"):
        _check(lib.drprg_hip_genotype(self._h, os.fsencode(vcf_refs) if vcf_refs else None, os.fsencode(out_vcf),
                                      sample.encode()), self._h)
        gi = (C.c_uint32 * 4)()
        lib.drprg_hip_genotype_info(self._h, gi)
        return dict(exp_depth_covg=int(gi[0]), min_kmer_covg=int(gi[1]), loci_present=int(gi[2]), records=int(gi[3]))

    def coverage_model(self):
        out = (C.c_double * 12)()
        _check(lib.drprg_hip_coverage_model(self._h, out), self._h)
        names = ("exp_depth_covg", "binomial", "e_rate", "nb_p", "nb_r", "branch", "mean", "var", "reads_per_locus", "bin_p", "thresh",
                 "dropped_low_coverage")
        d = dict(zip(names, (float(x) for x in out)))
        for key in ("exp_depth_covg", "binomial", "branch", "reads_per_locus", "thresh", "dropped_low_coverage"):
            d[key] = int(d[key])
        return d

    def discover(self, vcf_refs, out_dir, sample="sample"):
        n = C.c_uint32()
        _check(lib.drprg_hip_discover(self._h, os.fsencode(vcf_refs) if vcf_refs else None, os.fsencode(out_dir), sample.encode(),
                                      C.byref(n)), self._h)
        regions = []
        for line in open(os.path.join(out_dir, "candidate_regions.tsv")):
            if not line.startswith("#"):
                f = line.rstrip("\n").split("\t")
                regions.append(dict(locus=f[0], start=int(f[1]), end=int(f[2]), low_start=int(f[3]), low_end=int(f[4]),
                                    max_covg=int(f[5]), seq=f[6]))
        assert len(regions) == n.value
        return regions

    def discover_reads(self, reads, vcf_refs, out_dir, sample="sample", list_loci=True):
        out = (C.c_uint32 * 3)()
        _check(lib.drprg_hip_discover_reads(self._h, os.fsencode(reads), os.fsencode(vcf_refs) if vcf_refs else None, os.fsencode(out_dir),
                                            sample.encode(), 1 if list_loci else 0, out), self._h)
        variants = []
        for line in open(os.path.join(out_dir, "denovo_variants.tsv")):
            if not line.startswith("#"):
                f = line.rstrip("\n").split("\t")
                variants.append((f[0], int(f[1]), "" if f[2] == "." else f[2], "" if f[3] == "." else f[3], int(f[4]), int(f[5])))
        assert len(variants) == out[1]
        return variants

    def update_prg(self, out_prg):
        n = C.c_uint32()
        _check(lib.drprg_hip_update_prg(self._h, os.fsencode(out_prg), C.byref(n)), self._h)
        return int(n.value)

    def update_prg_from_paths(self, denovo_paths, out_prg):
        n = C.c_uint32()
        _check(lib.drprg_hip_update_prg_from_paths(self._h, os.fsencode(denovo_paths), os.fsencode(out_prg), C.byref(n)), self._h)
        return int(n.value)

    def save_coverage(self, path, tag):
        _check(lib.drprg_hip_save_coverage(self._h, os.fsencode(path), tag.encode()), self._h)

    def load_coverage(self, path, tag):
        rc = lib.drprg_hip_load_coverage(self._h, os.fsencode(path), tag.encode(), None)
        if rc == -2:
            return False
        _check(rc, self._h)
        return True

    def genotype_alleles(self, out_tsv):
        _check(lib.drprg_hip_genotype_alleles(self._h, os.fsencode(out_tsv)), self._h)
        out = {}
        for line in open(out_tsv):
            if line.startswith("#"):
                continue
            chrom, pos, a, n, nodes = line.rstrip("\n").split("\t")
            out[(chrom, int(pos), int(a))] = np.array([int(x) for x in nodes.split(",") if x], dtype=np.int64)
        return out

    def filter_selfcheck(self):
        out = (C.c_uint64 * 8)()
        _check(lib.drprg_hip_filter_selfcheck(self._h, out), self._h)
        names = ("codes", "level0_false_negatives", "level12_false_negatives", "stage2_false_negatives", "level0_fill_permille",
                 "level12_fill_permille", "stage2_fill_permille", "shared_array_false_negatives")
        return dict(zip(names, (int(x) for x in out)))

    def table_tier(self):
        out = (C.c_uint64 * 6)()
        _check(lib.drprg_hip_device_tables(self._h, out), self._h)
        return dict(pbloom_words=int(out[0]), table_bytes=int(out[1]), lds_filter_bytes=int(out[2]), kernel=int(out[3]),
                    l2_filter_bytes=int(out[4]))

    def export_index(self):
        keys = np.zeros(self.n_keys, dtype=np.uint64)
        rec_off = np.zeros(self.n_keys + 1, dtype=np.uint32)
        rec_prg = np.zeros(self.n_records, dtype=np.uint32)
        rec_knode = np.zeros(self.n_records, dtype=np.uint32)
        rec_strand = np.zeros(self.n_records, dtype=np.uint8)
        min_path_len = np.zeros(self.n_prgs, dtype=np.uint32)
        knode_base = np.zeros(self.n_prgs + 1, dtype=np.uint32)
        _check(lib.drprg_hip_index_export(self._h, _ptr(keys), _ptr(rec_off), _ptr(rec_prg), _ptr(rec_knode), _ptr(rec_strand),
                                          _ptr(min_path_len), _ptr(knode_base)), self._h)
        return dict(keys=keys, rec_off=rec_off, rec_prg=rec_prg, rec_knode=rec_knode, rec_strand=rec_strand,
                    min_path_len=min_path_len, knode_base=knode_base)

    def prg_nodes(self, prg):
        n, ns = C.c_uint32(), C.c_uint32()
        _check(lib.drprg_hip_prg_nodes(self._h, prg, None, None, 0, C.byref(n), C.byref(ns)), self._h)
        starts = np.zeros(n.value, dtype=np.uint32)
        ends = np.zeros(n.value, dtype=np.uint32)
        _check(lib.drprg_hip_prg_nodes(self._h, prg, _ptr(starts), _ptr(ends), n.value, C.byref(n), C.byref(ns)), self._h)
        return starts, ends, int(ns.value)

    def filter_schedule(self):
        out = (C.c_uint64 * 20)()
        _check(lib.drprg_hip_filter_schedule(self._h, out), self._h)
        v = [int(x) for x in out]
        return {"form": "dynamic" if v[0] > 1 else "static", "rounds": v[0], "slices": v[1], "slices_per_workgroup": v[11], "round0_tiles_per_wave": v[2],
                "round0_class_shares_per_256": v[3:7], "chunk_tiles_per_round": [x for x in v[13:20] if x],
                "class_end_us": [round(x / 100.0, 1) for x in v[7:11]]}

    def buffer_info(self):
        out = (C.c_uint64 * 6)()
        _check(lib.drprg_hip_buffer_info(self._h, out), self._h)
        return dict(filter_reruns=int(out[0]), direct_reruns=int(out[1]), hit_regrows=int(out[2]), lane_capacity=int(out[3]),
                    hit_capacity=int(out[4]))

    def kernel_timing(self, enable=True, reset=False):
        ms, n = C.c_double(), C.c_uint64()
        _check(lib.drprg_hip_kernel_timing(self._h, 1 if enable else 0, 1 if reset else 0, C.byref(ms), C.byref(n)), self._h)
        return ms.value, int(n.value)


def allele_stats(fwd, rev, min_kmer_covg):
    fwd = np.ascontiguousarray(fwd, dtype=np.uint32)
    rev = np.ascontiguousarray(rev, dtype=np.uint32)
    out = np.zeros(6, np.uint32)
    gaps = C.c_double()
    _check(lib.drprg_hip_allele_stats(_ptr(fwd), _ptr(rev), len(fwd), min_kmer_covg, _ptr(out), C.byref(gaps)))
    return [int(x) for x in out], gaps.value


def genotype_site(mean_fwd, mean_rev, gaps, e, eps=0.01):
    mf = np.ascontiguousarray(mean_fwd, dtype=np.uint32)
    mr = np.ascontiguousarray(mean_rev, dtype=np.uint32)
    g = np.ascontiguousarray(gaps, dtype=np.float64)
    lik = np.zeros(len(mf), np.float64)
    gt, conf = C.c_int32(), C.c_double()
    _check(lib.drprg_hip_genotype_site(_ptr(mf), _ptr(mr), _ptr(g), len(mf), e, eps, _ptr(lik), C.byref(gt), C.byref(conf)))
    return lik, gt.value, conf.value


class Pandora:

    def __init__(self, device=0):
        self.device = device

    @staticmethod
    def _parse_args(args):
        o = dict(threads=1, w=14, k=15, c=10, illumina=False, max_covg=300)
        it = iter([str(a) for a in args])
        for a in it:
            if a == "-t":
                o["threads"] = int(next(it))
            elif a == "-w":
                o["w"] = int(next(it))
            elif a == "-k":
                o["k"] = int(next(it))
# ... 114 lines not shown
```

include/drprg_hip.h:

```cpp
#ifndef DRPRG_HIP_H
#define DRPRG_HIP_H

#include <stddef.h>
#include <stdint.h>

#ifdef __cplusplus
extern "C" {
#endif

typedef struct drprg_hip_ctx drprg_hip_ctx;

#define DRPRG_HIP_MAP_OPTS_SIZE 48
typedef struct drprg_hip_map_opts {
    int32_t max_diff;
    double error_rate;
    uint32_t min_cluster_size;
    int32_t illumina;
    uint64_t genome_size;
    double genotyping_error_rate;
    int32_t kernel;
    int32_t binomial;
} drprg_hip_map_opts;

int drprg_hip_index(const char* prg_file, int w, int k, int threads);

drprg_hip_ctx* drprg_hip_open(const char* prg_file, int w, int k, int device);

drprg_hip_ctx* drprg_hip_open_prg(const char* prg_file, int w, int k, int device, int threads);

drprg_hip_ctx* drprg_hip_open_multi(const char* prg_file, int w, int k, const int* devices, int ndev, int from_files);

int drprg_hip_reduce(drprg_hip_ctx* ctx);
int drprg_hip_reduce_info(const drprg_hip_ctx* ctx, char* out, size_t cap);
int drprg_hip_comm_unique_id(uint8_t id[128]);
int drprg_hip_comm_init_rank(void** comm, int nranks, const uint8_t id[128], int rank, int device);
int drprg_hip_comm_destroy(void* comm);
int drprg_hip_allreduce(drprg_hip_ctx* ctx, void* comm, void* d_covg, void* d_prg_reads, void* hip_stream);

void drprg_hip_close(drprg_hip_ctx* ctx);
const char* drprg_hip_last_error(const drprg_hip_ctx* ctx);
int drprg_hip_experimental(void);

int drprg_hip_set_opts(drprg_hip_ctx* ctx, const drprg_hip_map_opts* opts);
int drprg_hip_set_opts_sized(drprg_hip_ctx* ctx, const drprg_hip_map_opts* opts, size_t opts_size);

int drprg_hip_map_fastx(drprg_hip_ctx* ctx, const char* reads_path);
int drprg_hip_set_threads(drprg_hip_ctx* ctx, int threads);

int drprg_hip_set_max_covg(drprg_hip_ctx* ctx, uint64_t max_covg);
int drprg_hip_max_covg_info(drprg_hip_ctx* ctx, uint64_t out[4]);
int drprg_hip_parse_fastx(const char* reads_path, int threads, uint64_t out[5], char* err, size_t err_len);
int drprg_hip_parse_fastx_ordered(const char* reads_path, int threads, uint64_t max_reads, uint64_t out[6], char* err, size_t err_len);
int drprg_hip_gunzip_file(const char* gz_path, int threads, uint64_t chunk_bytes, const char* out_path, uint64_t out[3], char* err, size_t err_len);
int drprg_hip_map_host(drprg_hip_ctx* ctx, const uint8_t* bases, const uint64_t* offsets, uint64_t n_reads);
int drprg_hip_map_device(drprg_hip_ctx* ctx, const void* d_bases, const void* d_offsets, uint64_t n_reads,
    uint64_t n_bases, void* d_covg, void* d_prg_reads, void* hip_stream);
int drprg_hip_map_device_async(drprg_hip_ctx* ctx, const void* d_bases, const void* d_offsets, uint64_t n_reads,
    uint64_t n_bases, void* d_covg, void* d_prg_reads, void* hip_stream);
int drprg_hip_sync(drprg_hip_ctx* ctx);

int drprg_hip_set_input_format(drprg_hip_ctx* ctx, int packed);
int drprg_hip_pack_reads(const uint8_t* bases, uint64_t n_bases, uint32_t* words, uint64_t* npos, uint64_t npos_cap, uint64_t* n_npos);
int drprg_hip_map_host_packed(drprg_hip_ctx* ctx, const uint32_t* words, const uint64_t* offsets, uint64_t n_reads, const uint64_t* npos, uint64_t n_npos);
int drprg_hip_map_device_packed(drprg_hip_ctx* ctx, const void* d_words, const void* d_offsets, uint64_t n_reads, uint64_t n_bases, const void* d_npos,
    uint64_t n_npos, void* d_covg, void* d_prg_reads, void* hip_stream);
int drprg_hip_map_device_packed_async(drprg_hip_ctx* ctx, const void* d_words, const void* d_offsets, uint64_t n_reads, uint64_t n_bases, const void* d_npos,
    uint64_t n_npos, void* d_covg, void* d_prg_reads, void* hip_stream);
int drprg_hip_pack_device(drprg_hip_ctx* ctx, const void* d_bases, uint64_t n_bases, void* d_words, void* d_npos, uint64_t npos_cap, uint64_t* n_npos,
    void* hip_stream);

int drprg_hip_coverage_size(const drprg_hip_ctx* ctx, uint64_t* n_covg, uint64_t* n_prgs);
int drprg_hip_coverage(drprg_hip_ctx* ctx, uint32_t* covg, uint64_t n_covg, uint32_t* prg_reads, uint64_t n_prgs);
int drprg_hip_set_coverage(drprg_hip_ctx* ctx, const uint32_t* covg, uint64_t n_covg, const uint32_t* prg_reads,
    uint64_t n_prgs, uint64_t total_bases);
int drprg_hip_device_coverage(drprg_hip_ctx* ctx, void** d_covg, void** d_prg_reads);
int drprg_hip_reset(drprg_hip_ctx* ctx);
int drprg_hip_counters(drprg_hip_ctx* ctx, uint64_t out[8]);

int drprg_hip_genotype(drprg_hip_ctx* ctx, const char* vcf_refs, const char* out_vcf, const char* sample);
int drprg_hip_genotype_info(const drprg_hip_ctx* ctx, uint32_t out[4]);

int drprg_hip_discover(drprg_hip_ctx* ctx, const char* vcf_refs, const char* out_dir, const char* sample, uint32_t* n_candidates);
int drprg_hip_discover_reads(drprg_hip_ctx* ctx, const char* reads_path, const char* vcf_refs, const char* out_dir, const char* sample,
    int list_loci, uint32_t out[3]);
int drprg_hip_keep_reads(drprg_hip_ctx* ctx, uint64_t max_bytes);
int drprg_hip_map_resident(drprg_hip_ctx* ctx, drprg_hip_ctx* from);
int drprg_hip_resident_info(drprg_hip_ctx* ctx, uint64_t out[4]);
int drprg_hip_select_reads(drprg_hip_ctx* ctx, const uint64_t* anchors, uint64_t n_anchors, uint32_t A, uint64_t window_bytes, uint8_t* bases,
    uint64_t bases_cap, uint64_t* offsets, uint64_t* ids, uint64_t reads_cap, uint64_t out[2]);

int drprg_hip_update_prg(drprg_hip_ctx* ctx, const char* out_prg, uint32_t* n_applied);
int drprg_hip_update_prg_from_paths(drprg_hip_ctx* ctx, const char* denovo_paths, const char* out_prg, uint32_t* n_applied);

int drprg_hip_save_coverage(drprg_hip_ctx* ctx, const char* path, const char* tag);
int drprg_hip_load_coverage(drprg_hip_ctx* ctx, const char* path, const char* tag, uint64_t counters[8]);

int drprg_hip_allele_stats(const uint32_t* fwd, const uint32_t* rev, uint32_t n, uint32_t min_kmer_covg, uint32_t out[6], double* gaps);
int drprg_hip_genotype_site(const uint32_t* mean_fwd, const uint32_t* mean_rev, const double* gaps, uint32_t n_alleles, double e,
    double eps, double* likelihood, int32_t* gt, double* gt_conf);
int drprg_hip_genotype_alleles(drprg_hip_ctx* ctx, const char* out_tsv);

int drprg_hip_filter_selfcheck(const drprg_hip_ctx* ctx, uint64_t out[8]);
int drprg_hip_estimate_parameters(const uint32_t* kmer_covg, uint64_t n, uint64_t clusters, uint64_t loci, uint32_t global_covg, int k,
    double e_rate, int bin, double out[10]);
int drprg_hip_kmer_log_prob(int use_bin, double nb_p, double nb_r, double bin_p, uint32_t fwd, uint32_t rev, uint32_t locus_reads, float* out);
int drprg_hip_prob_threshold(const float* logp, uint64_t n, int* out);
int drprg_hip_max_path(const drprg_hip_ctx* ctx, uint32_t prg, const float* logp, int thresh, uint32_t max_kmers_to_average, uint32_t* path,
    uint64_t cap, uint64_t* n_path);
int drprg_hip_path_base_coverage(const drprg_hip_ctx* ctx, uint32_t prg, const uint32_t* path, uint64_t n_path, const uint32_t* covg2,
    uint32_t* out, uint64_t cap, uint64_t* n_out);
int drprg_hip_path_coverage_too_low(const uint32_t* base_covg, uint64_t n, uint32_t global_covg);
int drprg_hip_coverage_model(const drprg_hip_ctx* ctx, double out[12]);

int drprg_hip_index_sizes(const drprg_hip_ctx* ctx, uint64_t sizes[5]);
int drprg_hip_index_export(const drprg_hip_ctx* ctx, uint64_t* keys, uint32_t* rec_off, uint32_t* rec_prg,
    uint32_t* rec_knode, uint8_t* rec_strand, uint32_t* prg_min_path_len, uint32_t* prg_knode_base);

int drprg_hip_device_tables(drprg_hip_ctx* ctx, uint64_t out[6]);

int drprg_hip_prg_nodes(const drprg_hip_ctx* ctx, uint32_t prg, uint32_t* starts, uint32_t* ends, uint32_t cap,
    uint32_t* n_nodes, uint32_t* n_sites);

typedef struct drprg_hip_annotate_opts {
    int32_t min_covg, max_covg;
    float min_strand_bias, min_gt_conf, min_frs;
    int32_t max_indel;
    float maf, max_gaps, max_called_gaps, max_gaps_diff;
    int32_t minor_min_covg;
    float minor_min_strand_bias;
    int32_t ignore_synonymous;
    uint64_t id_seed;
} drprg_hip_annotate_opts;

int drprg_hip_annotate(const char* index_dir, const char* pandora_vcf, const char* out_vcf,
    const drprg_hip_annotate_opts* opts, char* err, size_t err_len);
int drprg_hip_vcf_to_bcf(const char* vcf_path, const char* bcf_path, char* err, size_t err_len);
int drprg_hip_report_json(const char* index_dir, const char* annotated_vcf, const char* out_json, const char* sample,
    int padding, const char* index_version, char* err, size_t err_len);

int drprg_hip_kernel_timing(drprg_hip_ctx* ctx, int enable, int reset, double* ms_total, uint64_t* launches);
int drprg_hip_filter_schedule(drprg_hip_ctx* ctx, uint64_t out[20]);
int drprg_hip_buffer_info(drprg_hip_ctx* ctx, uint64_t out[6]);

#ifdef __cplusplus
}
#endif
#endif
```

Measured before the change: 21.04 billion.

## Split stage-2 bloom into two words and fold counter copy into last workgroup

The stage-2 bloom filter now draws its six probe bits from two independently hashed words (three bits each) rather than one word, which lowers the false-positive rate and so the number of candidates reaching the cluster stage. The cost is a second LDS load per k-mer. Separately, the counters-home copy and the zeroing of the super-count array move into the last finishing workgroup of the read-cluster kernel, using an atomic done-counter, which removes one kernel launch per batch. Diagnostic candidate counts and filter stats APIs are also added.

```diff
diff --git a/drprg_amd/_lib.py b/drprg_amd/_lib.py
--- a/drprg_amd/_lib.py
+++ b/drprg_amd/_lib.py
@@ -82,6 +82,7 @@
     "drprg_hip_select_reads": (C.c_int, [C.c_void_p, C.c_void_p, C.c_uint64, C.c_uint32, C.c_uint64, C.c_void_p, C.c_uint64, C.c_void_p, C.c_void_p,
                                          C.c_uint64, C.POINTER(C.c_uint64)]),
     "drprg_hip_counters": (C.c_int, [C.c_void_p, C.POINTER(C.c_uint64)]),
+    "drprg_hip_filter_candidates": (C.c_int, [C.c_void_p, C.POINTER(C.c_uint64)]),
     "drprg_hip_genotype": (C.c_int, [C.c_void_p, C.c_char_p, C.c_char_p, C.c_char_p]),
     "drprg_hip_genotype_info": (C.c_int, [C.c_void_p, C.POINTER(C.c_uint32)]),
     "drprg_hip_discover": (C.c_int, [C.c_void_p, C.c_char_p, C.c_char_p, C.c_char_p, C.POINTER(C.c_uint32)]),
@@ -105,6 +106,7 @@
     "drprg_hip_coverage_model": (C.c_int, [C.c_void_p, C.POINTER(C.c_double)]),
     "drprg_hip_index_sizes": (C.c_int, [C.c_void_p, C.POINTER(C.c_uint64)]),
     "drprg_hip_filter_selfcheck": (C.c_int, [C.c_void_p, C.POINTER(C.c_uint64)]),
+    "drprg_hip_filter_stats": (C.c_int, [C.c_void_p, C.POINTER(C.c_uint64)]),
     "drprg_hip_device_tables": (C.c_int, [C.c_void_p, C.POINTER(C.c_uint64)]),
     "drprg_hip_index_export": (C.c_int, [C.c_void_p] + [C.c_void_p] * 7),
     "drprg_hip_prg_nodes": (C.c_int, [C.c_void_p, C.c_uint32, C.c_void_p, C.c_void_p, C.c_uint32, C.POINTER(C.c_uint32),
diff --git a/drprg_amd/csrc/capi.cpp b/drprg_amd/csrc/capi.cpp
--- a/drprg_amd/csrc/capi.cpp
+++ b/drprg_amd/csrc/capi.cpp
@@ -220,6 +220,7 @@
         ctx->extra_counts.reads += k.reads; ctx->extra_counts.bases += k.bases; ctx->extra_counts.minimizers += k.minimizers;
         ctx->extra_counts.hits += k.hits; ctx->extra_counts.clusters_kept += k.clusters_kept;
         ctx->extra_counts.hits_kept += k.hits_kept; ctx->extra_counts.leftover_reads += k.leftover_reads;
+        ctx->extra_counts.candidates += k.candidates;
         e->reset_coverage(false);
     }
     ctx->host_coverage_valid = false;
@@ -877,6 +878,21 @@
         out[0] = c.reads + x.reads; out[1] = c.bases + x.bases; out[2] = c.minimizers + x.minimizers; out[3] = c.hits + x.hits;
         out[4] = c.clusters_kept + x.clusters_kept; out[5] = c.hits_kept + x.hits_kept; out[6] = c.kernel; out[7] = c.leftover_reads + x.leftover_reads;
     }
+    API_END(ctx)
+}
+
+int drprg_hip_filter_stats(const drprg_hip_ctx* ctx, uint64_t out[4])
+{
+    if (!ctx || !out) return DRPRG_EINVAL;
+    ctx->index.filter_stats(out);
+    return DRPRG_OK;
+}
+
+int drprg_hip_filter_candidates(drprg_hip_ctx* ctx, uint64_t* out)
+{
+    API_BEGIN(ctx)
+    if (!out) throw Error(DRPRG_EINVAL, "null output");
+    *out = ctx->mapper ? ctx->mapper->counters().candidates + ctx->extra_counts.candidates : 0;
     API_END(ctx)
 }
 
diff --git a/drprg_amd/csrc/common.h b/drprg_amd/csrc/common.h
--- a/drprg_amd/csrc/common.h
+++ b/drprg_amd/csrc/common.h
@@ -56,6 +56,7 @@
 constexpr uint32_t BLOOM_C2 = 0x85EBCA6Bu;
 constexpr uint32_t BLOOM_CR = 0xC2B2AE35u;
 constexpr uint32_t BLOOMR_WBITS = 14;
+inline uint32_t bloom0f_bits(uint32_t h, int lo) { return (1u << ((h >> lo) & 31)) | (1u << ((h >> (lo + 5)) & 31)) | (1u << ((h >> (lo + 10)) & 31)); }
 constexpr uint32_t MID_BITMAP_WORDS = 1u << 19;
 constexpr uint32_t MID_C_MAX_WBITS = 17;
 inline uint32_t rc12_code(uint32_t x)
diff --git a/drprg_amd/csrc/index.cpp b/drprg_amd/csrc/index.cpp
--- a/drprg_amd/csrc/index.cpp
+++ b/drprg_amd/csrc/index.cpp
@@ -149,9 +149,9 @@
             if (level0) {
                 const uint32_t hr = code * BLOOM_CR;
                 f.bloomr[hr >> (32 - BLOOMR_WBITS)] |= (1u << (hr & 31)) | (1u << ((hr >> 5) & 31)) | (1u << ((hr >> 10) & 31)) | (1u << ((hr >> 15) & 31));
+                f.bloom0f[hr >> (32 - L0_WBITS)] |= bloom0f_bits(hr, 0);
                 const uint32_t hs = code * BLOOM_C2;
-                f.bloom0f[hr >> (32 - L0_WBITS)] |= (1u << (hr & 31)) | (1u << ((hr >> 5) & 31)) | (1u << ((hr >> 10) & 31)) | (1u << (hs >> 27))
-                    | (1u << ((hs >> 22) & 31)) | (1u << ((hs >> 17) & 31));
+                f.bloom0f[hs >> (32 - L0_WBITS)] |= bloom0f_bits(hs, 2);
             }
             if (level0)
                 for (int o = 0; o < 4; ++o) {
@@ -293,10 +293,9 @@
                 const uint32_t g = (uint32_t)((uint64_t)y * BLOOM_C0);
                 miss_f |= !three(f.bloom0f[(g >> 17) & wmask0], g, y);
             }
-            const uint32_t wf = f.bloom0f[hr >> (32 - f.bloom0_wbits)];
             const uint32_t hs = code * BLOOM_C2;
-            miss_f |= !((wf >> (hr & 31)) & (wf >> ((hr >> 5) & 31)) & (wf >> ((hr >> 10) & 31)) & (wf >> (hs >> 27)) & (wf >> ((hs >> 22) & 31))
-                & (wf >> ((hs >> 17) & 31)) & 1u);
+            const uint32_t wf = f.bloom0f[hr >> (32 - f.bloom0_wbits)], ws = f.bloom0f[hs >> (32 - f.bloom0_wbits)];
+            miss_f |= (wf & bloom0f_bits(hr, 0)) != bloom0f_bits(hr, 0) || (ws & bloom0f_bits(hs, 2)) != bloom0f_bits(hs, 2);
             bool miss_blk = false;
             if (f.blkc_wbits)
                 for (int o = 0; o < 4; ++o) {
@@ -335,6 +334,33 @@
     out[4] = fill(f.bloom0);
     out[5] = fill(f.bloom);
     out[6] = fill(f.bloomr);
+}
+
+void PrgIndex::filter_stats(uint64_t out[4]) const
+{
+    for (int i = 0; i < 4; ++i) out[i] = 0;
+    const FlatIndex& f = flat;
+    if (!f.bloom0_wbits || f.bloom0f.empty()) return;
+    auto fill_ppm = [](const std::vector<uint32_t>& v) {
+        uint64_t bits = 0;
+        for (uint32_t w : v) bits += (uint64_t)__builtin_popcount(w);
+        return bits * 1000000 / (32 * (uint64_t)v.size());
+    };
+    out[0] = fill_ppm(f.bloom0f);
+    out[1] = fill_ppm(f.bloom0);
+    const uint32_t wmask0 = (1u << f.bloom0_wbits) - 1, n = 1u << 20;
+    uint64_t s = 0x9E3779B97F4A7C15ull, pass0 = 0, pass2 = 0;
+    for (uint32_t i = 0; i < n; ++i) {
+        s = s * 6364136223846793005ull + 1442695040888963407ull;
+        const uint32_t y = (uint32_t)(s >> 40) & 0xFFFFFFu, code = (uint32_t)(s >> 34) & 0x3FFFFFFFu;
+        const uint32_t g = (uint32_t)((uint64_t)y * BLOOM_C0), w0 = f.bloom0f[(g >> 17) & wmask0];
+        pass0 += ((w0 << (g & 31)) & (w0 << ((g >> 8) & 31)) & (w0 << ((y >> 16) & 31))) >> 31;
+        const uint32_t hr = code * BLOOM_CR, hs = code * BLOOM_C2;
+        pass2 += (f.bloom0f[hr >> (32 - f.bloom0_wbits)] & bloom0f_bits(hr, 0)) == bloom0f_bits(hr, 0)
+            && (f.bloom0f[hs >> (32 - f.bloom0_wbits)] & bloom0f_bits(hs, 2)) == bloom0f_bits(hs, 2);
+    }
+    out[2] = pass0 * 1000000 / n;
+    out[3] = pass2 * 1000000 / n;
 }
 
 void PrgIndex::save(const std::string& prg_file) const
diff --git a/drprg_amd/csrc/index.h b/drprg_amd/csrc/index.h
--- a/drprg_amd/csrc/index.h
+++ b/drprg_amd/csrc/index.h
@@ -39,6 +39,7 @@
     std::vector<KmerGraph> kgs;
     FlatIndex flat;
     void filter_selfcheck(uint64_t out[8]) const;
+    void filter_stats(uint64_t out[4]) const;
 
     static void build_and_save(const std::string& prg_file, int w, int k, int threads, const Switches& sw);
     void build(const std::string& prg_file, int w, int k, int threads, const Switches& sw);
diff --git a/drprg_amd/csrc/kernels.h b/drprg_amd/csrc/kernels.h
--- a/drprg_amd/csrc/kernels.h
+++ b/drprg_amd/csrc/kernels.h
@@ -197,7 +197,13 @@
     const uint32_t *wg_hits, *wg_nmin, *wg_maxlen;
     uint32_t n_wg;
     unsigned long long *tot_hits, *tot_minimizers, *tot_max_len;
+    unsigned long long* tot_candidates;
     const uint32_t* overflow_word;
+    unsigned long long *home_from, *home_to;
+    uint32_t home_n;
+    uint32_t* home_zero;
+    uint32_t home_zero_words;
+    uint32_t* wg_done;
     uint32_t minpath_in_lds;
 };
 hipError_t launch_counters_home(unsigned long long* from, unsigned long long* to, uint32_t n, hipStream_t stream, uint32_t* zero = nullptr, uint32_t n_zero = 0);
@@ -205,8 +211,12 @@
 uint32_t filter_super_words();
 size_t filter_small_words();
 void init_candidate_work(FilterWork& fw, const FilterBuffers& b, int n_cus);
+struct CountersHome {
+    unsigned long long *from = nullptr, *to = nullptr;
+    uint32_t n = 0;
+};
 hipError_t launch_sketch_filter(const SketchArgs& a, const BloomTables& bt, int n_cus, const FilterBuffers& b, const ReadClusterArgs& rc, FilterWork& fw,
-    const Switches& sw, hipStream_t stream, KernelTimer timer = {});
+    const Switches& sw, hipStream_t stream, KernelTimer timer = {}, const CountersHome& home = {}, bool* home_done = nullptr);
 hipError_t launch_filter_recount(const SketchArgs& a, const FilterWork& fw, hipStream_t stream);
 hipError_t launch_filter_expand(const SketchArgs& a, const FilterWork& fw, hipStream_t stream);
 hipError_t launch_direct_candidates(const SketchArgs& a, bool wide_hash, bool force_lds, uint32_t* tile_prefix, void* temp, size_t temp_bytes,
diff --git a/drprg_amd/csrc/mapper.cpp b/drprg_amd/csrc/mapper.cpp
--- a/drprg_amd/csrc/mapper.cpp
+++ b/drprg_amd/csrc/mapper.cpp
@@ -275,7 +275,7 @@
     HIPCHK(hipMemsetAsync(d_covg_, 0, (2 * (size_t)n_knodes_ + (size_t)n_prgs_) * sizeof(uint32_t), stream_));
     HIPCHK(hipMemsetAsync(d_counters_, 0, C_N * sizeof(unsigned long long), stream_));
     HIPCHK(hipStreamSynchronize(stream_));
-    tot_reads_ = tot_bases_ = tot_hits_ = tot_leftover_ = tot_minimizers_ = 0;
+    tot_reads_ = tot_bases_ = tot_hits_ = tot_leftover_ = tot_minimizers_ = tot_candidates_ = 0;
     for (auto& sh : ft_share_)
         for (uint32_t& v : sh) v = 0;
     sw_ = read_switches();
@@ -362,7 +362,10 @@
 {
     Lane& lane = lanes_[b.lane];
     grow_lane(lane, std::max<uint64_t>(min_capacity_, b.batch.n_bases / FILTER_BASES_PER_ENTRY));
-    if (!lane.scratch_zero) HIPCHK(hipMemsetAsync(lane.d_scratch, 0, L_N * sizeof(unsigned long long), b.stream));
+    if (!lane.scratch_zero) {
+        HIPCHK(hipMemsetAsync(lane.d_scratch, 0, L_N * sizeof(unsigned long long), b.stream));
+        HIPCHK(hipMemsetAsync(dev::filter_super_counts(lane.small), 0, dev::filter_super_words() * sizeof(uint32_t), b.stream));
+    }
     lane.scratch_zero = false;
     dev::SketchArgs a = sketch_args(b.batch);
     a.n_hits = &lane.d_scratch[L_HITS];
@@ -393,13 +396,16 @@
     rc.n_hits_kept = &d_counters_[C_HITS_KEPT];
     rc.n_complex = &lane.d_scratch[L_COMPLEX];
     rc.chunk_counter = reinterpret_cast<uint32_t*>(&lane.d_scratch[L_CHUNK]);
+    rc.tot_candidates = &lane.d_scratch[L_CANDS];
     dev::KernelTimer timer;
     if (timing_) {
         timer.begin = lane.t0;
         timer.end = lane.t1;
     }
-    HIPCHK(dev::launch_sketch_filter(a, bt, n_cus_, fb, rc, lane.fw, sw_, b.stream, timer));
-    HIPCHK(dev::launch_counters_home(lane.d_scratch, lane.h_scratch_dev, L_N, b.stream, dev::filter_super_counts(lane.small), dev::filter_super_words()));
+    bool home_done = false;
+    HIPCHK(dev::launch_sketch_filter(a, bt, n_cus_, fb, rc, lane.fw, sw_, b.stream, timer, dev::CountersHome { lane.d_scratch, lane.h_scratch_dev, (uint32_t)L_N }, &home_done));
+    if (!home_done)
+        HIPCHK(dev::launch_counters_home(lane.d_scratch, lane.h_scratch_dev, L_N, b.stream, dev::filter_super_counts(lane.small), dev::filter_super_words()));
     lane.scratch_zero = true;
 }
 
@@ -692,6 +698,7 @@
     tot_minimizers_ += lane.h_scratch[L_MINIMIZERS];
     tot_hits_ += lane.h_scratch[L_HITS];
     tot_leftover_ += lane.h_scratch[L_COMPLEX];
+    tot_candidates_ += lane.h_scratch[L_CANDS];
     tune_filter_shares(lane, b.batch.packed, b.batch.n_bases);
     leftovers(b);
     return true;
@@ -1263,6 +1270,7 @@
     m.hits_kept = c[C_HITS_KEPT];
     m.kernel = use_filter_ ? 2 : (use_direct_cands_ ? 3 : 1);
     m.leftover_reads = tot_leftover_;
+    m.candidates = tot_candidates_;
     return m;
 }
 
diff --git a/drprg_amd/csrc/mapper.h b/drprg_amd/csrc/mapper.h
--- a/drprg_amd/csrc/mapper.h
+++ b/drprg_amd/csrc/mapper.h
@@ -9,6 +9,7 @@
     uint64_t reads = 0, bases = 0, minimizers = 0, hits = 0, clusters_kept = 0, hits_kept = 0;
     uint64_t kernel = 0;
     uint64_t leftover_reads = 0;
+    uint64_t candidates = 0;
 };
 
 class Mapper {
@@ -104,7 +105,7 @@
         bool scratch_zero = false;
         dev::FilterWork fw {};
     };
-    enum { L_HITS = 0, L_OVERFLOW = 1, L_MAXLEN = 2, L_UNSORTED = 3, L_COMPLEX = 4, L_CHUNK = 5, L_MINIMIZERS = 6, L_FT_CLOCK = 7 , L_N = 12 };
+    enum { L_HITS = 0, L_OVERFLOW = 1, L_MAXLEN = 2, L_UNSORTED = 3, L_COMPLEX = 4, L_CHUNK = 5, L_MINIMIZERS = 6, L_FT_CLOCK = 7 , L_CANDS = 12, L_N = 13 };
     struct Batch {
         DeviceBatch batch;
         bool active = false;
@@ -174,7 +175,7 @@
     uint32_t* d_prg_reads_ = nullptr;
     unsigned long long* d_counters_ = nullptr;
     unsigned long long* h_counters_ = nullptr;
-    uint64_t tot_reads_ = 0, tot_bases_ = 0, tot_hits_ = 0, tot_leftover_ = 0, tot_minimizers_ = 0;
+    uint64_t tot_reads_ = 0, tot_bases_ = 0, tot_hits_ = 0, tot_leftover_ = 0, tot_minimizers_ = 0, tot_candidates_ = 0;
     uint64_t hit_capacity_ = 0;
     uint64_t *d_key_a_ = nullptr, *d_key_b_ = nullptr;
     uint32_t *d_val_a_ = nullptr, *d_val_b_ = nullptr;
diff --git a/drprg_amd/csrc/read_cluster.hip b/drprg_amd/csrc/read_cluster.hip
--- a/drprg_amd/csrc/read_cluster.hip
+++ b/drprg_amd/csrc/read_cluster.hip
@@ -76,10 +76,34 @@
             *rc.tot_hits = th;
             if (tn && !(*reinterpret_cast<volatile const uint32_t*>(rc.overflow_word) & 4u)) atomicAdd(rc.tot_minimizers, tn);
             *rc.tot_max_len = (unsigned long long)tm;
+            if (rc.tot_candidates) *rc.tot_candidates = (unsigned long long)*fw.cand_total;
         }
         __syncthreads();
     }
-    if (*reinterpret_cast<volatile uint32_t*>(a.overflow) & 4u) return;
+    auto counters_home = [&]() {
+        if (!rc.home_to) return;
+        __threadfence();
+        __syncthreads();
+        if (tid == 0) s_chunk = atomicAdd(rc.wg_done, 1u);
+        __syncthreads();
+        if (s_chunk != gridDim.x - 1) return;
+        __threadfence();
+        const uint32_t done_word = (uint32_t)(reinterpret_cast<unsigned long long*>(rc.wg_done - 1) - rc.home_from);
+        if ((uint32_t)tid < rc.home_n) {
+            rc.home_to[tid] = __hip_atomic_load(&rc.home_from[tid], __ATOMIC_RELAXED, __HIP_MEMORY_SCOPE_AGENT);
+            if ((uint32_t)tid != done_word) rc.home_from[tid] = 0;
+        }
+        uint4* const z = reinterpret_cast<uint4*>(rc.home_zero);
+        for (uint32_t j = (uint32_t)tid; j < rc.home_zero_words / 4; j += RC_THREADS) z[j] = make_uint4(0, 0, 0, 0);
+        const uint32_t tail = fw.n_slices + (uint32_t)tid;
+        if (tail < ((fw.n_slices + FT_SUPER - 1) & ~(uint32_t)(FT_SUPER - 1))) fw.slice_count[tail] = 0;
+        __syncthreads();
+        if (tid == 0) rc.home_from[done_word] = 0;
+    };
+    if (*reinterpret_cast<volatile uint32_t*>(a.overflow) & 4u) {
+        counters_home();
+        return;
+    }
     const uint32_t total = SLICES ? rc.slice_prefix[rc.n_slices] : *fw.cand_total;
     const uint32_t handled_mark = SLICES ? rc.mark_epoch : 0u;
     uint16_t* const s_minpath = reinterpret_cast<uint16_t*>(s_hist + rc.n_prgs);
@@ -539,6 +563,7 @@
         if (s_tot[1]) atomicAdd(rc.n_hits_kept, s_tot[1]);
         if (s_tot[2]) atomicAdd(rc.n_complex, s_tot[2]);
     }
+    counters_home();
 }
 #undef lane
 #undef wave
diff --git a/drprg_amd/csrc/sketch_filter.hip b/drprg_amd/csrc/sketch_filter.hip
--- a/drprg_amd/csrc/sketch_filter.hip
+++ b/drprg_amd/csrc/sketch_filter.hip
@@ -230,18 +230,19 @@
                     uint4 r = make_uint4(0, 0, 0, 0);                                                                                 \
                     if (ri < lcnt) {                                                                                                  \
                         r = stage[ri];                                                                                                \
-                                                                     \
-                        uint32_t hq[4], h2q[4], wq[4];                                                                                \
+                                    \
+                        uint32_t hq[4], h2q[4], wq[4], w2q[4];                                                                        \
                         _Pragma("unroll") for (int q = 0; q < 4; ++q) {                                                               \
                             const uint32_t f = (q ? __funnelshift_r(r.z, r.w, 2 * q) : r.z) & kmask;                                  \
                             hq[q] = f * BLOOM_CR;                                                                                     \
                             h2q[q] = f * BLOOM_C2;                                                                                    \
                             wq[q] = lds_at((hq[q] >> 17) << 2);                                                                       \
+                            w2q[q] = lds_at((h2q[q] >> 17) << 2);                                                                     \
                         }                                                                                                             \
                         __builtin_amdgcn_sched_barrier(0);      \
                         _Pragma("unroll") for (int q = 0; q < 4; ++q)                                                                 \
-                            cs |= ((wq[q] >> (hq[q] & 31)) & (wq[q] >> ((hq[q] >> 5) & 31)) & (wq[q] >> ((hq[q] >> 10) & 31)) & (wq[q] >> (h2q[q] >> 27)) \
-                                      & (wq[q] >> ((h2q[q] >> 22) & 31)) & (wq[q] >> ((h2q[q] >> 17) & 31)) & 1u) << q;               \
+                            cs |= ((wq[q] >> (hq[q] & 31)) & (wq[q] >> ((hq[q] >> 5) & 31)) & (wq[q] >> ((hq[q] >> 10) & 31))         \
+                                      & (w2q[q] >> ((h2q[q] >> 2) & 31)) & (w2q[q] >> ((h2q[q] >> 7) & 31)) & (w2q[q] >> ((h2q[q] >> 12) & 31)) & 1u) << q; \
                     }                                                                                                                 \
                     DRPRG_STAGE2_APPEND(r, cs);                                                                                       \
                 }                                                                                                                     \
@@ -563,11 +564,12 @@
 }
 
 hipError_t launch_sketch_filter(const SketchArgs& a, const BloomTables& bt, int n_cus, const FilterBuffers& b, const ReadClusterArgs& rc, FilterWork& fw,
-    const Switches& sw, hipStream_t stream, KernelTimer timer)
+    const Switches& sw, hipStream_t stream, KernelTimer timer, const CountersHome& home, bool* home_done)
 {
     fw = FilterWork {};
     fw.read_begin = 0;
     fw.read_end = a.n_reads;
+    if (home_done) *home_done = false;
     if (a.n_bases == 0) return hipSuccess;
     const bool mid = bt.mid_bitmap != nullptr;
     if (mid && (a.k != 15 || !bt.mid0 || !bt.midc || bt.midc_wbits < 1 || bt.midc_wbits > MID_C_MAX_WBITS || (bt.mid0_bits != 1 && bt.mid0_bits != 3)))
@@ -663,6 +665,17 @@
         rct.tot_minimizers = a.n_minimizers;
         rct.tot_max_len = fw.max_len;
         rct.overflow_word = a.overflow;
+        if (home.to && home_done) {
+            const size_t chunk_word = (size_t)(reinterpret_cast<unsigned long long*>(rc.chunk_counter) - home.from);
+            if (chunk_word >= home.n || home.n > 64) return hipErrorInvalidValue;
+            rct.home_from = home.from;
+            rct.home_to = home.to;
+            rct.home_n = home.n;
+            rct.home_zero = fw.super_count;
+            rct.home_zero_words = filter_super_words();
+            rct.wg_done = rc.chunk_counter + 1;
+            *home_done = true;
+        }
     }
     return launch_read_cluster(a, fw, rct, n_cus, skip_rc, stream);
 }
diff --git a/drprg_amd/pandora.py b/drprg_amd/pandora.py
--- a/drprg_amd/pandora.py
+++ b/drprg_amd/pandora.py
@@ -165,7 +165,9 @@
         out = (C.c_uint64 * 8)()
         _check(lib.drprg_hip_counters(self._h, out), self._h)
         names = ("reads", "bases", "minimizers", "hits", "clusters_kept", "hits_kept", "kernel", "leftover_reads")
-        return dict(zip(names, (int(x) for x in out)))
+        cand = C.c_uint64()
+        _check(lib.drprg_hip_filter_candidates(self._h, C.byref(cand)), self._h)
+        return dict(zip(names, (int(x) for x in out)), candidates=int(cand.value))
 
     def genotype(self, vcf_refs, out_vcf, sample="sample"):
         _check(lib.drprg_hip_genotype(self._h, os.fsencode(vcf_refs) if vcf_refs else None, os.fsencode(out_vcf),
@@ -245,6 +247,12 @@
         names = ("codes", "level0_false_negatives", "level12_false_negatives", "stage2_false_negatives", "level0_fill_permille",
                  "level12_fill_permille", "stage2_fill_permille", "shared_array_false_negatives")
         return dict(zip(names, (int(x) for x in out)))
+
+    def filter_stats(self):
+        out = (C.c_uint64 * 4)()
+        _check(lib.drprg_hip_filter_stats(self._h, out), self._h)
+        names = ("shared_array_fill", "level0_fill", "random_12mer_pass", "random_code_stage2_pass")
+        return dict(zip(names, (int(x) / 1e6 for x in out)))
 
     def table_tier(self):
         out = (C.c_uint64 * 6)()
diff --git a/include/drprg_hip.h b/include/drprg_hip.h
--- a/include/drprg_hip.h
+++ b/include/drprg_hip.h
@@ -76,6 +76,7 @@
 int drprg_hip_device_coverage(drprg_hip_ctx* ctx, void** d_covg, void** d_prg_reads);
 int drprg_hip_reset(drprg_hip_ctx* ctx);
 int drprg_hip_counters(drprg_hip_ctx* ctx, uint64_t out[8]);
+int drprg_hip_filter_candidates(drprg_hip_ctx* ctx, uint64_t* out);
 
 int drprg_hip_genotype(drprg_hip_ctx* ctx, const char* vcf_refs, const char* out_vcf, const char* sample);
 int drprg_hip_genotype_info(const drprg_hip_ctx* ctx, uint32_t out[4]);
@@ -101,6 +102,7 @@
 int drprg_hip_genotype_alleles(drprg_hip_ctx* ctx, const char* out_tsv);
 
 int drprg_hip_filter_selfcheck(const drprg_hip_ctx* ctx, uint64_t out[8]);
+int drprg_hip_filter_stats(const drprg_hip_ctx* ctx, uint64_t out[4]);
 int drprg_hip_estimate_parameters(const uint32_t* kmer_covg, uint64_t n, uint64_t clusters, uint64_t loci, uint32_t global_covg, int k,
     double e_rate, int bin, double out[10]);
 int drprg_hip_kmer_log_prob(int use_bin, double nb_p, double nb_r, double bin_p, uint32_t fwd, uint32_t rev, uint32_t locus_reads, float* out);
```

After: 17.25 billion. 18.0% lower.
